# zicodasilva/cheetah_pose_estimation

Measured on AMD Instinct MI355X. Metric: frames/sec residual+Jacobian eval + full-traj solves/sec, 200-frame 6-cam seq, higher is better.
Workload: dtype f64; 1 GPU; cfg2: synthetic 200-frame x 6-cam x 25-marker sequences, phantom skeleton, const-accel model; frames=200, cams=6, markers=25, sequences_per_gpu=2048, parallelism=shard1 (independent sequences, no collective)

## Files before the change

cheetah_pose_estimation_amd/csrc/cpe_api.hip:

```cpp
#include <hip/hip_runtime.h>

#include <cmath>
#include <cstdio>
#include <cstdlib>
#include <cstring>
#include <functional>
#include <string>
#include <vector>
#include <algorithm>
#include <type_traits>

#include "cpe_kernels.hip"

static thread_local std::string g_err;
static cpe_status fail(cpe_status s, const std::string& m) { g_err = m; return s; }
#define HIPCHK(x)                                                                                         \
    do {                                                                                                  \
        hipError_t e_ = (x);                                                                              \
        if (e_ != hipSuccess) return fail(CPE_HIP_ERROR, std::string(#x) + ": " + hipGetErrorString(e_)); \
    } while (0)

struct cpe_handle {
    int device = 0;
    int n_cu = 256;
    hipStream_t stream = nullptr;
    DevModel hm;
    DevModel* dm = nullptr;
    std::vector<DevModel> models;
    cpe_options opts;
    size_t ws_frames = 0; int ws_B = 0;
    std::vector<void**> ws_bufs;
    double *qbuf = nullptr, *gbuf = nullptr, *Bbuf = nullptr, *costbuf = nullptr, *Lbuf = nullptr, *zbuf = nullptr,
           *gtbuf = nullptr, *dgbuf = nullptr, *cmax = nullptr, *mu = nullptr, *gambuf = nullptr;
    SeqState* st = nullptr;
    int* flag = nullptr;
    int* act = nullptr;
    int2* rseq = nullptr;
    int* n_act = nullptr;
    int* poll_host = nullptr;
    hipEvent_t poll_ev[2] = {nullptr, nullptr};
    hipEvent_t order_ev = nullptr;
    bool prof = false;
    double prof_ms[CPE_PROFILE_SLOTS] = {0};
    int64_t prof_n[CPE_PROFILE_SLOTS] = {0};
    std::vector<std::pair<int, std::pair<hipEvent_t, hipEvent_t>>> prof_spans;
    cpe_eom_options* eom = nullptr;
    cpe_dyn_options* dyn = nullptr;
    DevPriors* pri = nullptr;
    int gmm_k = 0, gmm_dim = 0, lr_window = 0;
    double* Hlr = nullptr;
    DevKin* dk = nullptr; DevKin hk;
    std::vector<DevKin> hks;
    size_t kws_frames = 0;
    std::vector<void**> kws_bufs;
    double *kmut = nullptr;
    double *kmus = nullptr;
    double *fbuf = nullptr, *kmu = nullptr, *Jbuf = nullptr, *Abuf = nullptr, *pieces = nullptr, *gTb = nullptr, *dstat = nullptr, *slackb = nullptr,
           *Tbuf = nullptr, *gk = nullptr, *Bk = nullptr, *Hk = nullptr;
    int* pmeta = nullptr;
    DevTrack* dtrack = nullptr; std::vector<DevTrack> htrack;
    double* xtgt = nullptr; size_t xtgt_frames = 0;
    double* covG = nullptr; size_t covG_n = 0;
    int pb = 3;
};

struct DevBuf {
    double* p = nullptr;
    ~DevBuf() { if (p) (void)hipFree(p); }
    hipError_t alloc(size_t n) { return hipMalloc(&p, sizeof(double) * (n ? n : 1)); }
};

template <class T>
static hipError_t ws_alloc(std::vector<void**>& rec, T*& p, size_t n) {
    rec.push_back(reinterpret_cast<void**>(&p));
    return hipMalloc(&p, sizeof(T) * n);
}
static void ws_free(std::vector<void**>& rec) {
    for (void** p : rec) { (void)hipFree(*p); *p = nullptr; }
    rec.clear();
}

static double host_rho0(double a, double b, double c) {
    auto sg = [](double t) { return 1.0 / (1.0 + std::exp(t)); };
    const double sa = sg(a), sb = sg(b), sc = sg(c);
    const double cb = c - b, w = c / cb;
    return (sa - sb) * (-0.5 * a * a) + (sb - sc) * (a * b - 0.5 * a * a + 0.5 * a * cb * (1.0 - w * w)) +
           sc * (a * b - 0.5 * a * a + 0.5 * a * cb);
}

static cpe_status build_model(const cpe_skeleton* s, const cpe_camera* cams, int C, const cpe_options* o, DevModel& m) {
    memset(&m, 0, sizeof(m));
    if (s->n_links < 1 || s->n_links > CPE_MAX_LINKS || s->n_markers < 1 || s->n_markers > CPE_MAX_MARKERS ||
        s->n_joints < 0 || s->n_joints > CPE_MAX_JOINTS || s->n_bounds < 0 || s->n_bounds > CPE_MAX_BOUNDS ||
        C < 1 || C > CPE_MAX_CAMS)
        return fail(CPE_BAD_ARG, "skeleton / camera counts out of range");
    const int nl = s->n_links, nq = 3 + 3 * nl, L = s->n_markers;
    m.nl = nl; m.L = L; m.C = C; m.nq = nq; m.nj = s->n_joints; m.nb = s->n_bounds;
    m.h = o->h; m.ih2 = 1.0 / (o->h * o->h);
    m.loss_a = o->loss_a; m.loss_b = o->loss_b; m.loss_c = o->loss_c;
    m.bound_penalty = o->bound_penalty; m.curvature = o->curvature;
    m.rho0 = host_rho0(o->loss_a, o->loss_b, o->loss_c);
    if (!(o->h > 0)) return fail(CPE_BAD_ARG, "options.h must be > 0");
    double mt = 0;
    for (int i = 0; i < nl; i++) {
        if (s->parent[i] >= i) return fail(CPE_BAD_ARG, "links must be ordered parents first");
        m.parent[i] = s->parent[i];
        for (int d = 0; d < 3; d++) { m.attach[i][d] = s->attach[i][d]; m.com[i][d] = s->com[i][d]; }
        m.mass[i] = s->mass[i]; mt += s->mass[i];
    }
    m.inv_total_mass = mt > 0 ? 1.0 / mt : 0.0;
    for (int c = 0; c < C; c++) m.cam[c] = cams[c];

    for (int p = 0; p < nq; p++) { m.u_of_q[p] = -1; m.dep_of_q[p] = -1; }
    int ndep = 0;
    std::vector<int> joint_of_child(nl, -1);
    for (int j = 0; j < s->n_joints; j++) {
        const int p = s->joint_parent[j], c = s->joint_child[j], k = s->joint_kind[j];
        if (p < 0 || p >= nl || c <= p || c >= nl || joint_of_child[c] >= 0) return fail(CPE_BAD_ARG, "bad joint");
        m.joint_parent[j] = p; m.joint_child[j] = c; m.joint_kind[j] = k;
        joint_of_child[c] = j;
        m.joint_dep0[j] = ndep;
        m.dep_joint[ndep] = j;
        m.dep_of_q[3 + 3 * c] = ndep++;
        if (k == CPE_JOINT_REVOLUTE_Y) { m.dep_joint[ndep] = j; m.dep_of_q[3 + 3 * c + 2] = ndep++; }
        else if (k != CPE_JOINT_HOOKE_YZ) return fail(CPE_BAD_ARG, "unknown joint kind");
        if (ndep > CPE_MAX_DEP) return fail(CPE_BAD_ARG, "too many dependent angles");
    }
    m.ndep = ndep;
    int nu = 0;
    for (int p = 0; p < nq; p++)
        if (m.dep_of_q[p] < 0) { if (nu >= CPE_NX) return fail(CPE_BAD_ARG, "more than 28 independent dofs"); m.indep[nu] = p; m.u_of_q[p] = nu++; }
    m.nu = nu;
    if (nu != CPE_NX) return fail(CPE_BAD_ARG, "the solver is built for exactly 28 independent dofs");
    for (int p = 0; p < nq; p++)
        if (m.dep_of_q[p] >= 0 && s->motion_w[p] != 0.0) return fail(CPE_BAD_ARG, "motion weight on a dependent angle");
    for (int k = 0; k < nu; k++) {
        const int p = m.indep[k];
        m.motion_w_u[k] = s->motion_w[p];
        m.rel_sign_u[k] = s->rel_ref[p] < 0 ? 1.0 : s->rel_sign[p];
        m.rel_ref_u[k] = s->rel_ref[p] < 0 ? -1 : m.u_of_q[s->rel_ref[p]];
        if (s->rel_ref[p] >= 0 && m.rel_ref_u[k] < 0) return fail(CPE_BAD_ARG, "relative angle references a dependent dof");
    }
// ... 21 lines not shown
            m.joint_body[j] = p;
            m.srow[r] = m.n_srow++;
            int n = 0;
            auto add = [&](int col, int kind, int ang, int chain) -> bool {
                for (int e = 0; e < n; e++)
                    if (m.scol[r][e] == col) { if (chain >= 0) m.hk_chain[r][e] = (int16_t)chain; else { m.hk_kind[r][e] = (int8_t)kind; m.hk_ang[r][e] = (int8_t)ang; } return true; }
                if (n >= CPE_MAX_SCOL) return false;
                m.scol[r][n] = col; m.hk_kind[r][n] = (int8_t)kind; m.hk_ang[r][n] = (int8_t)ang; m.hk_chain[r][n] = (int16_t)chain; n++;
                return true;
            };
            if (m.u_of_q[3 + 3 * c + 1] < 0 || m.u_of_q[3 + 3 * c + 2] < 0) return fail(CPE_BAD_ARG, "theta/psi of a hooke child must be independent");
            bool ok = add(m.u_of_q[3 + 3 * c + 1], 0, 1, -1) && add(m.u_of_q[3 + 3 * c + 2], 0, 2, -1);
            m.dep_level[r] = 0;
            for (int a = 0; a < 3 && ok; a++) {
                const int pq = 3 + 3 * p + a;
                if (m.u_of_q[pq] >= 0) ok = add(m.u_of_q[pq], 1, a, -1);
                else {
                    if (a != 0) return fail(CPE_BAD_ARG, "hooke parent with dependent theta/psi is not supported");
                    const int pr = m.dep_of_q[pq];
                    if (m.dep_level[pr] != 0 || m.joint_kind[m.dep_joint[pr]] != CPE_JOINT_HOOKE_YZ)
                        return fail(CPE_BAD_ARG, "hooke chains deeper than two are not supported");
                    m.dep_level[r] = 1;
                    for (int e = 0; e < m.scol_n[pr] && ok; e++) ok = add(m.scol[pr][e], 2, 0, m.srow[pr] * CPE_MAX_SCOL + e);
                }
            }
            if (!ok) return fail(CPE_BAD_ARG, "too many columns in a hooke row");
            m.scol_n[r] = n;
        }
    }
    std::vector<int> rev_of_link(nl, -1);
    m.nrev = 0;
    for (int p = 0; p < nq; p++) m.euler_rev[p] = -1;
    for (int k = 0; k < nu; k++) { m.rev_of_u[k] = -1; m.ucoord_src[k] = m.indep[k]; m.bodyang_j[k] = -1; m.bodyang_legs_n[k] = 0; }
    for (int j = 0; j < s->n_joints; j++)
        if (m.joint_kind[j] == CPE_JOINT_REVOLUTE_Y) {
            const int r = m.nrev++, c = m.joint_child[j], Bk = m.joint_body[j];
            rev_of_link[c] = r;
            m.rev_child[r] = c; m.rev_body[r] = Bk; m.rev_u[r] = m.u_of_q[3 + 3 * c + 1];
            m.rev_of_u[m.rev_u[r]] = r; m.euler_rev[3 + 3 * c + 1] = r;
            for (int a = 0; a < 3; a++) {
                const int kb = m.u_of_q[3 + 3 * Bk + a];
                m.rev_body_u[r][a] = kb; m.bodyang_j[kb] = a;
                m.bodyang_legs[kb][m.bodyang_legs_n[kb]++] = r;
            }
        }
    m.ns = nq + m.nrev;
    for (int k = 0; k < nu; k++) {
        const int r = m.rev_of_u[k];
        m.ucost[k] = r < 0 ? m.indep[k] : ((3 + 3 * m.rev_body[r] + 1) | (nq + r + 1) << 8);
    }
    if (m.nrev > LM_MAX_REV) return fail(CPE_BAD_ARG, "more than 12 leg links");
    for (int k = 0; k < nu; k++) if (m.bodyang_legs_n[k] > LM_MAX_LEGS) return fail(CPE_BAD_ARG, "more than 6 leg links on one body");
    for (int r = 0; r < m.nrev; r++) m.ucoord_src[m.rev_u[r]] = nq + r;
    m.n_trunk = 0;
    for (int i = 0; i < nl; i++) { m.trunk_slot[i] = -1; if (rev_of_link[i] < 0) { m.trunk_slot[i] = m.n_trunk; m.trunk_link[m.n_trunk++] = i; } }
    int S = 0, mct = 0, ss = 0, sv = 0;
    for (int l = 0; l < L; l++) {
        int chain[CPE_MAX_LINKS], n = 0, k = s->marker_link[l];
        if (k < 0 || k >= nl) return fail(CPE_BAD_ARG, "bad marker link");
        while (k >= 0) { chain[n++] = k; k = s->parent[k]; }
        if (n > CPE_MAX_CHAIN) return fail(CPE_BAD_ARG, "marker chain too long");
        m.chain_len[l] = n;
        for (int i = 0; i < n; i++) {
            const int link = chain[n - 1 - i];
            m.chain_link[l][i] = link;
            const double* v = i == n - 1 ? s->marker_off[l] : s->attach[chain[n - 2 - i]];
            for (int d = 0; d < 3; d++) m.chain_vec[l][i][d] = v[d];
        }
        m.slot_off[l] = S;
        if (S + 3 + 3 * n > CPE_MAX_SLOTS) return fail(CPE_BAD_ARG, "too many Jacobian slots");
        for (int d = 0; d < 3; d++) { m.slot_marker[S] = l; m.slot_dof[S] = d; m.slot_cpos[S] = -1; m.slot_ang[S] = 0; S++; }
        for (int i = 0; i < n; i++)
            for (int a = 0; a < 3; a++) { m.slot_marker[S] = l; m.slot_dof[S] = 3 + 3 * m.chain_link[l][i] + a; m.slot_cpos[S] = i; m.slot_ang[S] = a; S++; }
        int nc = 0;
        auto col_index = [&](int col) -> int {
            for (int e = 0; e < nc; e++) if (m.mcol[l][e] == col) return e;
            if (nc >= CPE_MAX_MCOL) return -1;
            m.mcol[l][nc] = col; m.term_n[l][nc] = 0; return nc++;
        };
        auto add_term = [&](int col, int slot, int sidx) -> bool {
            const int e = col_index(col);
            if (e < 0 || m.term_n[l][e] >= CPE_MAX_TERMS) return false;
            m.term_slot[l][e][m.term_n[l][e]] = (int16_t)slot; m.term_s[l][e][m.term_n[l][e]] = (int16_t)sidx; m.term_n[l][e]++;
            return true;
        };
        auto new_slot = [&](int moff, int vdyn, const double* v) -> int {
            if (ss >= CPE_MAX_SLOTS) return -1;
            m.ss_moff[ss] = moff; m.ss_vdyn[ss] = vdyn;
            for (int d = 0; d < 3; d++) m.ss_vec[ss][d] = v ? v[d] : 0.0;
            return ss++;
        };
        bool ok = true;
        const double ex[3][3] = {{1, 0, 0}, {0, 1, 0}, {0, 0, 1}};
        for (int d = 0; d < 3 && ok; d++) { const int sl = new_slot(-1, -1, ex[d]); ok = sl >= 0 && add_term(m.u_of_q[d], sl, -1); }
        int n_trunk_chain = 0;
        while (n_trunk_chain < n && rev_of_link[m.chain_link[l][n_trunk_chain]] < 0) n_trunk_chain++;
        m.pc_len[l] = n_trunk_chain; m.pw_id[l] = -1; m.pw_body[l] = 0;
        for (int i = 0; i < n_trunk_chain && ok; i++) {
            const int link = m.chain_link[l][i];
            m.pc_link[l][i] = link;
            for (int d = 0; d < 3; d++) m.pc_vec[l][i][d] = m.chain_vec[l][i][d];
            for (int a = 0; a < 3 && ok; a++) {
                const int sl = new_slot(9 * (4 * m.trunk_slot[link] + 1 + a), -1, m.chain_vec[l][i]);
                const int p = 3 + 3 * link + a;
                if (sl < 0) { ok = false; break; }
                if (m.u_of_q[p] >= 0) ok = add_term(m.u_of_q[p], sl, -1);
// ... 86 lines not shown
                const int a = m.mcol[l][i];
                if (m.gg_cnt[a] >= CPE_MAX_GG) return fail(CPE_BAD_ARG, "gradient gather list too long");
                m.gg_code[m.gg_cnt[a]++][a] = (uint16_t)((m.mcol_off[l] + i) | (l << 8));
            }
    }
    {
        m.hk_n = 0;
        for (int r = 0; r < m.ndep; r++) {
            const int j = m.dep_joint[r];
            if (m.joint_kind[j] != CPE_JOINT_HOOKE_YZ || m.srow[r] < 0) continue;
            for (int jc = 0; jc < m.scol_n[r]; jc++) {
                if (m.hk_n >= 64) return fail(CPE_BAD_ARG, "more than 64 entries in the hooke rows of S");
                const int ps = m.trunk_slot[m.joint_parent[j]], cs = m.trunk_slot[m.joint_child[j]];
                if (ps < 0 || cs < 0 || ps >= 64 || cs >= 64) return fail(CPE_BAD_ARG, "hooke joint between leg links");
                m.hk_w[m.hk_n][0] = ps | (cs << 6) | ((m.hk_kind[r][jc] & 3) << 12) | ((m.hk_ang[r][jc] & 3) << 14) | ((m.dep_level[r] & 1) << 16);
                m.hk_w[m.hk_n][1] = (m.hk_chain[r][jc] + 1) | ((m.srow[r] * CPE_MAX_SCOL + jc) << 16);
                m.hk_n++;
            }
        }
        m.hj_n = 0;
        for (int j = 0; j < s->n_joints; j++)
            if (m.joint_kind[j] == CPE_JOINT_HOOKE_YZ) {
                if (m.hj_n >= 64) return fail(CPE_BAD_ARG, "more than 64 hooke joints");
                m.fn_lane[m.hj_n++][0] = m.joint_parent[j] | (m.joint_child[j] << 8) | ((m.dep_of_q[3 + 3 * m.joint_parent[j]] >= 0 ? 1 : 0) << 16);
            }
        for (int t = 0; t < 4 * m.n_trunk && t < 64; t++) m.fn_lane[t][1] = m.trunk_link[t >> 2];
        for (int r = 0; r < m.nrev; r++) m.fn_lane[r][2] = m.rev_body[r] | (m.rev_child[r] << 8) | (m.trunk_slot[m.rev_body[r]] << 16);
        for (int t = 0; t < m.sv_n; t++) m.fn_lane[t][3] = m.sv_kind[t] | (m.sv_cnt[t] << 2) | (m.sv_rev[t][0] << 4) | (m.sv_rev[t][1] << 10) | (m.sv_rev[t][2] << 16);
        for (int l = 0; l < L; l++) {
            for (int i = 0; i < m.pc_len[l]; i++) m.pc_off[l][i] = 36 * m.trunk_slot[m.pc_link[l][i]];
            m.pw_off[l] = m.pw_id[l] >= 0 ? 36 * m.trunk_slot[m.pw_body[l]] : 0;
        }
    }
    for (int bnd = 0; bnd < s->n_bounds; bnd++) {
        const int a = s->bound_a[bnd], bb = s->bound_b[bnd];
        if (a < 0 || a >= nq || bb >= nq || m.u_of_q[a] < 0 || (bb >= 0 && m.u_of_q[bb] < 0))
            return fail(CPE_BAD_ARG, "bounds must act on independent dofs");
        m.bound_ua[bnd] = m.u_of_q[a]; m.bound_ub[bnd] = bb < 0 ? -1 : m.u_of_q[bb];
        m.bound_lo[bnd] = s->bound_lo[bnd]; m.bound_up[bnd] = s->bound_up[bnd];
        const int ca = m.ucost[m.u_of_q[a]], cb = bb < 0 ? 0 : m.ucost[m.u_of_q[bb]];
        m.bnd_q[bnd] = (ca & 255) | (bb < 0 ? 0 : ((cb & 255) + 1) << 8) | ((ca >> 8) & 255) << 16 | (bb < 0 ? 0 : ((cb >> 8) & 255)) << 24;
    }
    return CPE_OK;
}

#define FRAME_NORMAL(plain) ((plain) ? k_frame_normal<true> : k_frame_normal<false>)
#define FRAME_NORMAL_RAGGED(plain) ((plain) ? k_frame_normal<true, true> : k_frame_normal<false, true>)
static size_t lds_fk(const DevModel& m) { return sizeof(double) * (m.nq + 6 * m.nl + 36 * m.nl + 3 * m.L + 23 * m.C); }
static size_t lds_normal(const DevModel& m, int gmm_k = 0, int gmm_dim = 0, bool shutter = false) {
    const bool plain = gmm_k == 0 && !shutter;
    size_t ov = CPE_MAX_SCOL * m.n_srow, hg = plain ? m.nu : m.nu * m.nu + m.nu;
    size_t camov = 6 * m.nl + 2 * m.nrev + 36 * m.n_trunk;
    if (camov < (size_t)22 * m.C) camov = (size_t)22 * m.C;
    size_t n = m.ns + camov + 3 * m.L + 3 * m.sv_n + GAM_STRIDE * m.nrev + (ov > hg ? ov : hg) +
               9 * m.L + 3 * m.mc_total;
    if (gmm_k > 0) n += CPE_NX + gmm_k * gmm_dim + CPE_MAX_GMM + CPE_NX;
    if (shutter) n += 15 * m.C + 6 * m.L + 6;
    return sizeof(double) * n;
}
static size_t lds_fk_all(const cpe_handle* h) {
    size_t n = lds_fk(h->hm);
    for (const DevModel& m : h->models) n = std::max(n, lds_fk(m));
    return n;
}
static size_t lds_normal_all(const cpe_handle* h) {
    size_t n = lds_normal(h->hm, h->gmm_k, h->gmm_dim);
    for (const DevModel& m : h->models) n = std::max(n, lds_normal(m, h->gmm_k, h->gmm_dim));
    return n;
}
#define FRAME_TRACKED(gmm) ((gmm) ? k_frame_tracked<true> : k_frame_tracked<false>)
#define FRAME_TRACKED_RAGGED(gmm) ((gmm) ? k_frame_tracked<true, true> : k_frame_tracked<false, true>)
static size_t lds_tracked(const DevModel& m, int gmm_k, int gmm_dim) {
    size_t n = m.ns + 6 * m.nl + 2 * m.nrev + 36 * m.n_trunk + GAM_STRIDE * m.nrev + m.nu + m.nu * m.nu + m.nu;
    if (gmm_k > 0) n += CPE_NX + gmm_k * gmm_dim + CPE_MAX_GMM + CPE_NX;
    return sizeof(double) * n;
}
static size_t lds_tracked_all(const cpe_handle* h) {
    size_t n = lds_tracked(h->hm, h->gmm_k, h->gmm_dim);
    for (const DevModel& m : h->models) n = std::max(n, lds_tracked(m, h->gmm_k, h->gmm_dim));
    return n;
}
static int n_models(const cpe_handle* h) { return h->models.empty() ? 1 : (int)h->models.size(); }
static int cams_max(const cpe_handle* h) {
    int c = h->hm.C;
    for (const DevModel& m : h->models) c = std::max(c, m.C);
    return c;
}

extern "C" {

const char* cpe_last_error(void) { return g_err.c_str(); }

void cpe_default_options(cpe_options* o) {
    o->h = 1.0 / 120.0; o->loss_a = 3.0; o->loss_b = 10.0; o->loss_c = 20.0; o->cost_scale = 1e-3;
    o->bound_penalty = 1e4; o->bound_tol = 1e-6; o->lambda0 = 1e-4; o->tol_step = 1e-8; o->tol_cost = 1e-9; o->max_iter = 200;
    o->curvature = 0; o->max_outer = 8; o->_pad = 0;
}

void cpe_destroy(cpe_handle* h);
static cpe_status create_impl(cpe_handle* h, const cpe_skeleton* skel, const cpe_camera* cams, int32_t n_cams, const cpe_options* opts,
                              const cpe_priors* priors, bool use_pri, const std::vector<DevModel>* models = nullptr) {
    const int device = h->device;
    if (models) { h->models = *models; h->hm = h->models[0]; }
    else if (cpe_status s = build_model(skel, cams, n_cams, opts, h->hm); s != CPE_OK) return s;
    HIPCHK(hipSetDevice(device));
    {
        hipDeviceProp_t prop;
        HIPCHK(hipGetDeviceProperties(&prop, device));
        h->n_cu = prop.multiProcessorCount > 0 ? prop.multiProcessorCount : 256;
        const void* ks[] = {(const void*)&k_resjac<true, 4, 3, 2>, (const void*)&k_resjac<false, 4, 3, 2>,
                            (const void*)&k_resjac<true, 4, 4, 2>, (const void*)&k_resjac<false, 4, 4, 2>,
                            (const void*)&k_dyn_eval<>, (const void*)&k_dyn_assemble<>, (const void*)&k_dyn_schur<>, (const void*)&k_dyn_jac<>,
                            (const void*)&k_dyn_eval<true>, (const void*)&k_dyn_assemble<true>, (const void*)&k_dyn_schur<true>, (const void*)&k_dyn_jac<true>};
        for (const void* k : ks) {
            hipFuncAttributes fa;
            HIPCHK(hipFuncGetAttributes(&fa, k));
            HIPCHK(hipFuncSetAttribute(k, hipFuncAttributeMaxDynamicSharedMemorySize, 160 * 1024 - (int)fa.sharedSizeBytes));
        }
    }
    HIPCHK(hipStreamCreateWithFlags(&h->stream, hipStreamNonBlocking));
    HIPCHK(hipEventCreateWithFlags(&h->order_ev, hipEventDisableTiming));
    for (int i = 0; i < 2; i++) HIPCHK(hipEventCreateWithFlags(&h->poll_ev[i], hipEventDisableTiming));
    HIPCHK(hipHostMalloc(reinterpret_cast<void**>(&h->poll_host), 2 * sizeof(int), hipHostMallocDefault));
    HIPCHK(hipMalloc(&h->n_act, sizeof(int)));
    HIPCHK(hipMalloc(&h->dm, sizeof(DevModel) * n_models(h)));
    HIPCHK(hipMemcpy(h->dm, h->models.empty() ? &h->hm : h->models.data(), sizeof(DevModel) * n_models(h), hipMemcpyHostToDevice));
// ... 374 lines not shown
    if (!h) return fail(CPE_BAD_ARG, "null argument");
    size_t F;
    if (cpe_status s = frames(B, N, &F); s != CPE_OK) return s;
    if (F == 0) return CPE_OK;
    if (!positions || !uv) return fail(CPE_BAD_ARG, "null argument");
    HIPCHK(hipSetDevice(h->device));
    hipLaunchKernelGGL(k_reproject, dim3((unsigned)F), dim3(WAVE), 0, h->stream, h->dm, positions, uv);
    HIPCHK(hipGetLastError());
    return CPE_OK;
}

cpe_status cpe_triangulate(cpe_handle* h, int32_t n, const int32_t* cam_a, const int32_t* cam_b, const double* uv_a, const double* uv_b,
                           double depth, double* xyz) {
    if (!h) return fail(CPE_BAD_ARG, "null argument");
    if (n < 0) return fail(CPE_BAD_ARG, "negative size");
    if (n == 0) return CPE_OK;
    if (!cam_a || !cam_b || !uv_a || !uv_b || !xyz) return fail(CPE_BAD_ARG, "null argument");
    HIPCHK(hipSetDevice(h->device));
    std::vector<int32_t> ia(n), ib(n);
    HIPCHK(hipMemcpyAsync(ia.data(), cam_a, sizeof(int32_t) * n, hipMemcpyDeviceToHost, h->stream));
    HIPCHK(hipMemcpyAsync(ib.data(), cam_b, sizeof(int32_t) * n, hipMemcpyDeviceToHost, h->stream));
    HIPCHK(hipStreamSynchronize(h->stream));
    for (int i = 0; i < n; i++)
        if (ia[i] < 0 || ia[i] >= h->hm.C || ib[i] >= h->hm.C) return fail(CPE_BAD_ARG, "camera index out of range");
    hipLaunchKernelGGL(k_triangulate, dim3((unsigned)((n + 255) / 256)), dim3(256), 0, h->stream, h->dm, n, cam_a, cam_b, uv_a, uv_b, depth, xyz);
    HIPCHK(hipGetLastError());
    return CPE_OK;
}

cpe_status cpe_tensorise_dlc(cpe_handle* h, int32_t N, int32_t n_slots, int32_t slot, const double* table, int32_t rows, int32_t parts,
                             int32_t first_row, const int32_t* part_of_marker, const double* inv_sigma, double thresh, double* meas, double* weight) {
    if (!h) return fail(CPE_BAD_ARG, "null argument");
    if (N < 0 || rows < 0 || parts <= 0) return fail(CPE_BAD_ARG, "bad size");
    if (n_slots <= 0 || slot < 0 || slot >= n_slots) return fail(CPE_BAD_ARG, "camera slot out of range");
    if (N == 0) return CPE_OK;
    if (!part_of_marker || !inv_sigma || !meas || !weight || (!table && rows > 0)) return fail(CPE_BAD_ARG, "null argument");
    HIPCHK(hipSetDevice(h->device));
    const long total = (long)N * h->hm.L;
    hipLaunchKernelGGL(k_tensorise_dlc, dim3((unsigned)((total + 255) / 256)), dim3(256), 0, h->stream, N, h->hm.L, n_slots, slot, table, rows, parts,
                       first_row, part_of_marker, inv_sigma, thresh, meas, weight);
    HIPCHK(hipGetLastError());
    return CPE_OK;
}

static size_t n_mu(const DevModel& m, size_t F) { return F * (size_t)(m.nb > 0 ? m.nb : 1) * 2; }

static cpe_status ensure_ws(cpe_handle* h, int B, int N) {
    const size_t F = (size_t)B * N;
    if (F <= h->ws_frames && B <= h->ws_B) return CPE_OK;
    free_ws(h);
    const int nu = h->hm.nu;
    auto& w = h->ws_bufs;
    HIPCHK(ws_alloc(w, h->qbuf, 2 * F * h->hm.ns));
    HIPCHK(ws_alloc(w, h->gambuf, 2 * F * (size_t)(GAM_STRIDE * (h->hm.nrev > 0 ? h->hm.nrev : 1))));
    HIPCHK(ws_alloc(w, h->gbuf, 2 * F * nu));
    HIPCHK(ws_alloc(w, h->Bbuf, 2 * F * nu * nu));
    HIPCHK(ws_alloc(w, h->costbuf, 2 * F * COST_STRIDE));
    HIPCHK(ws_alloc(w, h->mu, n_mu(h->hm, F)));
    HIPCHK(ws_alloc(w, h->Lbuf, F * (h->pb + 1) * nu * nu + (size_t)B * lm_spill_doubles(h->pb)));
    HIPCHK(ws_alloc(w, h->zbuf, F * nu));
    HIPCHK(ws_alloc(w, h->gtbuf, F * nu));
    HIPCHK(ws_alloc(w, h->dgbuf, F * nu));
    HIPCHK(ws_alloc(w, h->cmax, F));
    HIPCHK(ws_alloc(w, h->st, B));
    HIPCHK(ws_alloc(w, h->act, B));
    HIPCHK(ws_alloc(w, h->rseq, B));
    if (h->lr_window > 0) HIPCHK(ws_alloc(w, h->Hlr, 2 * F * h->pb * nu * nu));
    h->ws_frames = F; h->ws_B = B;
    return CPE_OK;
}

static cpe_status state_reset(cpe_handle* h, int B, int N, const double* q, const RaggedArgs* rg = nullptr) {
    const size_t F = (size_t)B * N;
    if (rg) hipLaunchKernelGGL(k_state_init<true>, dim3((unsigned)F), dim3(WAVE), 0, h->stream, h->dm, q, h->qbuf, *rg);
    else hipLaunchKernelGGL(k_state_init<>, dim3((unsigned)F), dim3(WAVE), 0, h->stream, h->dm, q, h->qbuf);
    HIPCHK(hipMemsetAsync(h->st, 0, sizeof(SeqState) * B, h->stream));
    HIPCHK(hipMemsetAsync(h->mu, 0, sizeof(double) * n_mu(h->hm, F), h->stream));
    return CPE_OK;
}

cpe_status cpe_eval_normal(cpe_handle* h, int32_t B, int32_t N, const double* q, const double* meas, const double* weight,
                           double* g, double* Bm, double* cost, double* gam, double* q_out) {
    if (!h || !q || !meas || !weight || !g || !Bm || !cost) return fail(CPE_BAD_ARG, "null argument");
    size_t F;
    if (cpe_status s = frames(B, N, &F); s != CPE_OK) return s;
    if (F == 0) return CPE_OK;
    HIPCHK(hipSetDevice(h->device));
    cpe_status s = ensure_ws(h, B, N);
    if (s != CPE_OK) return s;
    if ((s = state_reset(h, B, N, q)) != CPE_OK) return s;
    const DevModel& m = h->hm;
    hipLaunchKernelGGL(FRAME_NORMAL(h->gmm_k == 0), dim3((unsigned)F), dim3(WAVE), lds_normal(m, h->gmm_k, h->gmm_dim), h->stream, h->dm, h->st, N, 1, F, h->qbuf, meas, weight,
                       h->gbuf, h->Bbuf, h->costbuf, h->mu, h->gambuf, h->pri, nullptr, nullptr, ShutterArgs{nullptr, nullptr, nullptr}, RaggedArgs{});
    HIPCHK(hipMemcpyAsync(g, h->gbuf, sizeof(double) * F * m.nu, hipMemcpyDeviceToDevice, h->stream));
    HIPCHK(hipMemcpyAsync(Bm, h->Bbuf, sizeof(double) * F * m.nu * m.nu, hipMemcpyDeviceToDevice, h->stream));
    hipLaunchKernelGGL(k_gather_normal, dim3((unsigned)F), dim3(128), 0, h->stream, h->dm, F, h->qbuf, h->costbuf, h->gambuf, cost, gam, q_out);
    HIPCHK(hipGetLastError());
    return CPE_OK;
}

static LmParams lm_params(const cpe_handle* h, int B, int N) {
    LmParams prm;
    prm.tol_step = h->opts.tol_step; prm.tol_cost = h->opts.tol_cost; prm.lambda0 = h->opts.lambda0; prm.B = B; prm.N = N;
    prm.bound_tol = h->opts.bound_tol; prm.max_outer = h->opts.max_outer; prm.max_iter = h->opts.max_iter;
    return prm;
}

using LmIterate = std::function<void(int first, const int* act, const int* n_act, int slots)>;

static cpe_status lm_drive(cpe_handle* h, int B, const LmIterate& iterate) {
    iterate(1, nullptr, nullptr, B);
    HIPCHK(hipGetLastError());
    const int window = std::min(B, h->n_cu * (h->pb == 3 ? 2 : 1));
    constexpr int POLL = 4;
    const long per_seq = (long)h->opts.max_iter + 2L * (h->opts.max_outer > 0 ? h->opts.max_outer : 0) + POLL;
    const long max_rounds = ((long)(B + window - 1) / window + 1) * per_seq;
    bool pending[2] = {false, false};
    int slot = 0;
    for (long it = 0; it < max_rounds; it += POLL) {
        for (int k = 0; k < POLL; k++) {
            prof_begin(h, 3);
            hipLaunchKernelGGL(k_build_act, dim3(1), dim3(256), 0, h->stream, h->st, B, window, h->act, h->n_act);
            prof_end(h);
            iterate(0, h->act, h->n_act, window);
        }
        HIPCHK(hipGetLastError());
        HIPCHK(hipMemcpyAsync(h->poll_host + slot, h->n_act, sizeof(int), hipMemcpyDeviceToHost, h->stream));
        HIPCHK(hipEventRecord(h->poll_ev[slot], h->stream));
        pending[slot] = true;
        const int prev = 1 - slot;
        if (pending[prev]) {
            HIPCHK(hipEventSynchronize(h->poll_ev[prev]));
            pending[prev] = false;
            if (h->poll_host[prev] == 0) break;
        }
        slot = prev;
    }
    return CPE_OK;
}

__global__ void k_reset_status(SeqState* __restrict__ st, int B) {
    const int b = blockIdx.x * blockDim.x + threadIdx.x;
    if (b < B) { st[b].status = 0; st[b].al_pending = 0; }
}

extern "C++" template <class Fn>
static void with_pb(int pb, Fn&& f) {
    switch (pb) {
    case 3: f(std::integral_constant<int, 3>{}); break;
    case 4: f(std::integral_constant<int, 4>{}); break;
    case 5: f(std::integral_constant<int, 5>{}); break;
    default: f(std::integral_constant<int, 6>{}); break;
    }
}

static void lm_iterate(cpe_handle* h, const LmParams& prm, int N, size_t Fw, size_t ldsn, const double* meas, const double* weight, ShutterArgs sh,
                       const RaggedArgs* rg, int first, const int* act, const int* n_act, int slots, bool back = true) {
    const bool lr = h->lr_window > 0;
    const unsigned gf = (unsigned)((size_t)slots * N);
    const double* hiu = lr ? reinterpret_cast<const double*>(reinterpret_cast<const char*>(h->pri) + offsetof(DevPriors, lr_HIu)) + CPE_NX * CPE_NX : nullptr;
    if (rg) {
        prof_begin(h, 0);
        hipLaunchKernelGGL(FRAME_NORMAL_RAGGED(h->gmm_k == 0), dim3(gf), dim3(WAVE), ldsn, h->stream, h->dm, h->st, N, first, Fw, h->qbuf, meas, weight,
                           h->gbuf, h->Bbuf, h->costbuf, h->mu, h->gambuf, h->pri, act, n_act, ShutterArgs{nullptr, nullptr, nullptr}, *rg);
        prof_end(h);
        if (lr) {
            prof_begin(h, 1);
            hipLaunchKernelGGL(k_lr_band<true>, dim3(gf), dim3(WAVE), 0, h->stream, h->dm, h->st, N, first, Fw, h->qbuf, h->gambuf, h->pri, h->pb, h->gbuf,
                               h->Bbuf, h->Hlr, h->costbuf, act, n_act, *rg);
            prof_end(h);
        }
        prof_begin(h, 2);
        with_pb(h->pb, [&](auto pbc) {
            hipLaunchKernelGGL((k_lm_step<decltype(pbc)::value, 0, true>), dim3(slots), dim3(LM_THREADS), 0, h->stream, h->dm, h->st, prm, first, h->qbuf,
                               h->gbuf, h->Bbuf, h->costbuf, h->Lbuf, h->zbuf, h->gtbuf, h->gambuf, h->Hlr, act, n_act, 2, nullptr, h->dgbuf, hiu, h->lr_window, *rg);
        });
        prof_end(h);
        if (!back) return;
        prof_begin(h, 7);
        with_pb(h->pb, [&](auto pbc) {
            hipLaunchKernelGGL((k_lm_back<decltype(pbc)::value, true>), dim3(slots), dim3(2 * WAVE), 0, h->stream, h->dm, h->st, prm, h->qbuf, h->Lbuf,
                               h->zbuf, h->gtbuf, h->dgbuf, act, n_act, *rg);
        });
        prof_end(h);
        return;
    }
    prof_begin(h, 0);
    hipLaunchKernelGGL(FRAME_NORMAL(h->gmm_k == 0 && sh.tau == nullptr), dim3(gf), dim3(WAVE), ldsn, h->stream, h->dm, h->st, N, first, Fw, h->qbuf, meas, weight, h->gbuf, h->Bbuf,
                       h->costbuf, h->mu, h->gambuf, h->pri, act, n_act, sh, RaggedArgs{});
    prof_end(h);
    if (lr) {
        prof_begin(h, 1);
        hipLaunchKernelGGL(k_lr_band<>, dim3(gf), dim3(WAVE), 0, h->stream, h->dm, h->st, N, first, Fw, h->qbuf, h->gambuf, h->pri, h->pb, h->gbuf, h->Bbuf,
                           h->Hlr, h->costbuf, act, n_act);
        prof_end(h);
    }
    prof_begin(h, 2);
    with_pb(h->pb, [&](auto pbc) {
        hipLaunchKernelGGL((k_lm_step<decltype(pbc)::value, 0>), dim3(slots), dim3(LM_THREADS), 0, h->stream, h->dm, h->st, prm, first, h->qbuf, h->gbuf,
                           h->Bbuf, h->costbuf, h->Lbuf, h->zbuf, h->gtbuf, h->gambuf, h->Hlr, act, n_act, 2, sh.gx, h->dgbuf, hiu, h->lr_window);
    });
    prof_end(h);
    if (!back) return;
    prof_begin(h, 7);
    with_pb(h->pb, [&](auto pbc) {
        hipLaunchKernelGGL((k_lm_back<decltype(pbc)::value>), dim3(slots), dim3(2 * WAVE), 0, h->stream, h->dm, h->st, prm, h->qbuf, h->Lbuf, h->zbuf,
                           h->gtbuf, h->dgbuf, act, n_act);
    });
    prof_end(h);
}

static cpe_status lm_run(cpe_handle* h, int B, int N, const double* q_init, const double* meas, const double* weight, ShutterArgs sh,
                         const RaggedArgs* rg = nullptr) {
    const DevModel& m = h->hm;
    const size_t Fw = (size_t)B * N;
    if (q_init) {
        const cpe_status s = state_reset(h, B, N, q_init, rg);
        if (s != CPE_OK) return s;
    } else hipLaunchKernelGGL(k_reset_status, dim3((B + 255) / 256), dim3(256), 0, h->stream, h->st, B);
    const LmParams prm = lm_params(h, B, N);
    const size_t ldsn = rg ? lds_normal_all(h) : lds_normal(m, h->gmm_k, h->gmm_dim, sh.tau != nullptr);
    return lm_drive(h, B, [&](int first, const int* act, const int* n_act, int slots) {
        lm_iterate(h, prm, N, Fw, ldsn, meas, weight, sh, rg, first, act, n_act, slots);
    });
}

static cpe_status lm_readback(cpe_handle* h, int B, int N, const double* meas, double* q, double* dq, double* ddq, double* positions, double* meas_err,
                              const double* tau, const std::function<void()>& more, std::vector<SeqState>& hs, std::vector<double>& hc,
                              const RaggedArgs* rg = nullptr) {
    const size_t F = (size_t)B * N;
    HIPCHK(hipMemsetAsync(h->cmax, 0, sizeof(double) * B, h->stream));
    if (rg) hipLaunchKernelGGL(k_finalize<true>, dim3((unsigned)F), dim3(WAVE), lds_fk_all(h), h->stream, h->dm, h->st, N, F, h->qbuf, meas, q, dq, ddq,
                               positions, meas_err, reinterpret_cast<unsigned long long*>(h->cmax), nullptr, *rg);
    else hipLaunchKernelGGL(k_finalize<>, dim3((unsigned)F), dim3(WAVE), lds_fk(h->hm), h->stream, h->dm, h->st, N, F, h->qbuf, meas, q, dq, ddq, positions, meas_err,
                            reinterpret_cast<unsigned long long*>(h->cmax), tau);
    if (more) more();
    HIPCHK(hipGetLastError());
    hs.resize(B);
    hc.resize(B);
    HIPCHK(hipMemcpyAsync(hs.data(), h->st, sizeof(SeqState) * B, hipMemcpyDeviceToHost, h->stream));
    HIPCHK(hipMemcpyAsync(hc.data(), h->cmax, sizeof(double) * B, hipMemcpyDeviceToHost, h->stream));
    HIPCHK(hipStreamSynchronize(h->stream));
    prof_collect(h);
    return CPE_OK;
}

static void kinematic_costs(const SeqState& S, double scale, cpe_stats& o) {
    o.cost_meas = S.terms[0]; o.cost_model = S.terms[1]; o.cost_pose = S.terms[3]; o.cost_motion = S.terms[4];
    o.cost = scale * (S.terms[0] + S.terms[1] + S.terms[3] + S.terms[4]);
}
static void kinetic_costs(const SeqState& S, double scale, cpe_stats& o) {
    o.cost_meas = S.terms[0]; o.cost_model = S.terms[4]; o.cost_pose = S.terms[3]; o.cost_motion = 0.0;
    o.cost = scale * (S.terms[0] + S.terms[3] + S.terms[4]);
// ... 322 lines not shown
    HIPCHK(ws_alloc(w, h->Jbuf, F * KIN_JSTRIDE));
    HIPCHK(ws_alloc(w, h->Abuf, F * CPE_MAX_NQ * KIN_LS));
    HIPCHK(ws_alloc(w, h->pieces, 2 * F * KIN_PIECE));
    HIPCHK(ws_alloc(w, h->pmeta, 2 * F * (KIN_LS + 1)));
    HIPCHK(ws_alloc(w, h->gTb, 2 * (F + 2) * KIN_NC3));
    HIPCHK(ws_alloc(w, h->dstat, 2 * F * KIN_STAT));
    HIPCHK(ws_alloc(w, h->slackb, 2 * F * CPE_MAX_NQ));
    HIPCHK(ws_alloc(w, h->Tbuf, (F + 2) * 6 * BB));
    HIPCHK(ws_alloc(w, h->gk, F * CPE_NX));
    HIPCHK(ws_alloc(w, h->Bk, F * BB));
    HIPCHK(ws_alloc(w, h->Hk, F * 3 * BB));
    h->kws_frames = F;
    return CPE_OK;
}

static cpe_status kin_state_reset(cpe_handle* h, size_t F, bool torque_box) {
    HIPCHK(hipMemsetAsync(h->fbuf, 0, sizeof(double) * 2 * F * KIN_LS, h->stream));
    HIPCHK(hipMemsetAsync(h->kmu, 0, sizeof(double) * F * 4 * KIN_MU, h->stream));
    HIPCHK(hipMemsetAsync(h->kmus, 0, sizeof(double) * F * 2 * CPE_MAX_NQ, h->stream));
    if (torque_box) HIPCHK(hipMemsetAsync(h->kmut, 0, sizeof(double) * F * 2 * CPE_MAX_MOTORS, h->stream));
    return CPE_OK;
}

extern "C++" {

template <bool RAGGED = false>
static void launch_dyn_eval(cpe_handle* h, int N, int first, size_t Fw, const int32_t* stance, const int* act, const int* n_act, int slots, RaggedArgs rg = RaggedArgs{}) {
    const unsigned gf = (unsigned)((size_t)slots * N);
    prof_begin(h, 5);
    hipLaunchKernelGGL(k_dyn_eval<RAGGED>, dim3(gf), dim3(KIN_THREADS), lds_kin_eval(), h->stream, h->dm, h->dk, h->st, N, first, Fw, h->qbuf, stance, h->fbuf, h->kmu,
                       h->costbuf, h->Jbuf, h->Abuf, h->pieces, h->pmeta, h->dstat, h->slackb, act, n_act, rg);
    prof_end(h);
}
template <bool RAGGED = false>
static void launch_dyn_pieces(cpe_handle* h, int N, int first, size_t Fw, const int* act, const int* n_act, int slots, RaggedArgs rg = RaggedArgs{}) {
    const unsigned gf = (unsigned)((size_t)slots * N);
    prof_begin(h, 10);
    hipLaunchKernelGGL(k_dyn_jac<RAGGED>, dim3(gf), dim3(KJ_THREADS), sizeof(double) * KJ_DOUBLES, h->stream, h->dm, h->dk, h->st, N, first, Fw, h->qbuf, h->fbuf, h->Jbuf,
                       act, n_act, rg);
    prof_end(h);
    prof_begin(h, 8);
    hipLaunchKernelGGL(k_dyn_assemble<RAGGED>, dim3(gf), dim3(KIN_THREADS), lds_kin_assemble(), h->stream, h->dm, h->dk, h->st, N, first, Fw, h->Jbuf, h->Abuf, h->pieces,
                       h->pmeta, h->gTb, act, n_act, rg);
    prof_end(h);
}

template <bool RAGGED>
static void kin_iterate(cpe_handle* h, const LmParams& prm, int N, size_t Fw, size_t ldsn, const double* meas, const double* weight, const int32_t* stance,
                        const double* xt, RaggedArgs rg, int first, const int* act, const int* n_act, int slots) {
    const unsigned gf = (unsigned)((size_t)slots * N);
    const bool plain = h->gmm_k == 0;
    prof_begin(h, 0);
    if (xt) hipLaunchKernelGGL(RAGGED ? FRAME_TRACKED_RAGGED(!plain) : FRAME_TRACKED(!plain), dim3(gf), dim3(WAVE), ldsn, h->stream, h->dm, h->dtrack, h->st, N, first, Fw,
                               h->qbuf, xt, h->gbuf, h->Bbuf, h->costbuf, h->mu, h->gambuf, h->pri, act, n_act, rg);
    else hipLaunchKernelGGL(RAGGED ? FRAME_NORMAL_RAGGED(plain) : FRAME_NORMAL(plain), dim3(gf), dim3(WAVE), ldsn, h->stream, h->dm, h->st, N, first, Fw, h->qbuf, meas,
                            weight, h->gbuf, h->Bbuf, h->costbuf, h->mu, h->gambuf, h->pri, act, n_act, ShutterArgs{nullptr, nullptr, nullptr}, rg);
    prof_end(h);
    launch_dyn_eval<RAGGED>(h, N, first, Fw, stance, act, n_act, slots, rg);
    prof_begin(h, 2);
    hipLaunchKernelGGL((k_lm_step<3, 1, RAGGED>), dim3(slots), dim3(LM_THREADS), 0, h->stream, h->dm, h->st, prm, first, h->qbuf, h->gbuf, h->Bbuf, h->costbuf,
                       h->Lbuf, h->zbuf, h->gtbuf, h->gambuf, nullptr, act, n_act, 2, nullptr, h->dgbuf, nullptr, 0, rg);
    prof_end(h);
    launch_dyn_pieces<RAGGED>(h, N, 0, Fw, act, n_act, slots, rg);
    prof_begin(h, 9);
    hipLaunchKernelGGL(k_dyn_schur<RAGGED>, dim3(gf), dim3(KIN_THREADS), lds_kin_schur(), h->stream, h->dk, h->st, N, Fw, h->pieces, h->pmeta, h->fbuf, h->kmu, stance,
                       h->Tbuf, act, n_act, rg);
    prof_end(h);
    prof_begin(h, 6);
    hipLaunchKernelGGL(k_dyn_gather<RAGGED>, dim3(gf), dim3(KIN_THREADS), 0, h->stream, h->st, N, Fw, h->gbuf, h->Bbuf, h->Tbuf, h->gTb, h->gk, h->Bk, h->Hk, act,
                       n_act, rg);
    prof_end(h);
    prof_begin(h, 2);
    hipLaunchKernelGGL((k_lm_step<3, 2, RAGGED>), dim3(slots), dim3(LM_THREADS), 0, h->stream, h->dm, h->st, prm, first, h->qbuf, h->gk, h->Bk, h->costbuf,
                       h->Lbuf, h->zbuf, h->gtbuf, h->gambuf, h->Hk, act, n_act, 1, nullptr, h->dgbuf, nullptr, 0, rg);
    prof_end(h);
    prof_begin(h, 7);
    hipLaunchKernelGGL((k_lm_back<3, RAGGED>), dim3(slots), dim3(2 * WAVE), 0, h->stream, h->dm, h->st, prm, h->qbuf, h->Lbuf, h->zbuf, h->gtbuf, h->dgbuf, act, n_act, rg);
    prof_end(h);
}

}

void cpe_default_track_weights(double w[CPE_NX]) {
    static const double t[CPE_NX] = {10, 10, 10, 5, 5, 5, 0, 5, 5, 0, 2, 2, 5, 5, 5, 5, 5, 2, 1, 5, 2, 1, 5, 2, 5, 2, 1, 1};
    for (int k = 0; k < CPE_NX; k++) w[k] = t[k];
}

static cpe_status build_track(cpe_handle* h, const double* w, int rows) {
    for (int i = 0; i < rows * CPE_NX; i++)
        if (!std::isfinite(w[i]) || w[i] < 0.0)
            return fail(CPE_BAD_ARG, "track_w: weights must be finite and non-negative (row " + std::to_string(i / CPE_NX) + ", entry " + std::to_string(i % CPE_NX) + ")");
    const int nmod = n_models(h);
    h->htrack.assign((size_t)nmod, DevTrack{});
    for (int k = 0; k < nmod; k++) {
        const DevModel& m = h->models.empty() ? h->hm : h->models[(size_t)k];
        const double* wk = w + (size_t)std::min(k, rows - 1) * CPE_NX;
        const int nu = m.nu;
        double X[CPE_NX][CPE_NX] = {};
        for (int i = 0; i < nu; i++)
            for (int side = 0; side < 2; side++) {
                const int kk = side == 0 ? i : m.rel_ref_u[i];
                if (kk < 0) continue;
                const double sgn = side == 0 ? m.rel_sign_u[i] : -m.rel_sign_u[i];
                X[i][kk] += sgn;
                const int r = m.rev_of_u[kk];
                if (r >= 0) X[i][m.rev_body_u[r][1]] += sgn;
            }
        DevTrack& T = h->htrack[(size_t)k];
        for (int i = 0; i < nu; i++) T.w[i] = wk[i];
        for (int i = 0; i < nu; i++)
            for (int j = 0; j < nu; j++) {
                T.Xt[j][i] = X[i][j];
                double a = 0.0;
                for (int p = 0; p < nu; p++) a += X[p][i] * wk[p] * X[p][j];
                T.H[i * nu + j] = 2.0 * a;
            }
    }
    if (!h->dtrack) HIPCHK(hipMalloc(&h->dtrack, sizeof(DevTrack) * nmod));
    HIPCHK(hipMemcpyAsync(h->dtrack, h->htrack.data(), sizeof(DevTrack) * nmod, hipMemcpyHostToDevice, h->stream));
    return CPE_OK;
}

static cpe_status check_target(const double* hq, int B, int N, int nq, const int32_t* lens) {
    for (int b = 0; b < B; b++)
        for (size_t i = 0; i < (size_t)(lens ? lens[b] : N) * nq; i++)
            if (!std::isfinite(hq[(size_t)b * N * nq + i]))
                return fail(CPE_BAD_ARG, "q_target: non-finite entry (sequence " + std::to_string(b) + ", frame " + std::to_string(i / nq) + ")");
// ... 135 lines not shown
    return solve_kinetic_impl(h, opt, B, N, nullptr, nullptr, q_init, meas, weight, stance, nullptr, tau_box, nullptr, q, dq, ddq, positions, meas_err, tau, lambda, grf, slack, stats, kstats);
}

cpe_status cpe_solve_kinetic_ragged(cpe_handle* h, const cpe_kinetic_options* opts, int32_t B, int32_t N_max, const int32_t* model, const int32_t* n_frames,
                                    const double* q_init, const double* meas, const double* weight, const int32_t* stance, const double* grf_fixed,
                                    const double* tau_box, const double* grf_box, double* q, double* dq, double* ddq, double* positions, double* meas_err,
                                    double* tau, double* lambda, double* grf, double* slack, cpe_stats* stats, cpe_kinetic_stats* kstats) {
    if (!h || !opts || !model || !n_frames) return fail(CPE_BAD_ARG, "null argument");
    if ((grf_fixed != nullptr) + (tau_box != nullptr) + (grf_box != nullptr) > 1)
        return fail(CPE_BAD_ARG, "cpe_solve_kinetic_ragged: at most one of grf_fixed, tau_box, grf_box");
    return solve_kinetic_impl(h, opts, B, N_max, model, n_frames, q_init, meas, weight, stance, grf_fixed, tau_box, grf_box, q, dq, ddq, positions, meas_err,
                              tau, lambda, grf, slack, stats, kstats);
}

cpe_status cpe_solve_kinetic_tracked(cpe_handle* h, const cpe_kinetic_options* opt, const double* track_w, int32_t B, int32_t N, const double* q_init,
                                     const double* q_target, const double* meas, const double* weight, const int32_t* stance, const double* grf_fixed,
                                     const double* tau_box, const double* grf_box, double* q, double* dq, double* ddq, double* positions, double* meas_err,
                                     double* tau, double* lambda, double* grf, double* slack, cpe_stats* stats, cpe_kinetic_stats* kstats) {
    if ((grf_fixed != nullptr) + (tau_box != nullptr) + (grf_box != nullptr) > 1)
        return fail(CPE_BAD_ARG, "cpe_solve_kinetic_tracked: at most one of grf_fixed, tau_box, grf_box");
    const TrackIn tr{track_w, 1, q_target, false};
    return solve_kinetic_impl(h, opt, B, N, nullptr, nullptr, q_init, meas, weight, stance, grf_fixed, tau_box, grf_box, q, dq, ddq, positions, meas_err,
                              tau, lambda, grf, slack, stats, kstats, &tr);
}

cpe_status cpe_solve_kinetic_tracked_ragged(cpe_handle* h, const cpe_kinetic_options* opts, const double* track_w, int32_t B, int32_t N_max,
                                            const int32_t* model, const int32_t* n_frames, const double* q_init, const double* q_target, const double* meas,
                                            const double* weight, const int32_t* stance, const double* grf_fixed, const double* tau_box,
                                            const double* grf_box, double* q, double* dq, double* ddq, double* positions, double* meas_err, double* tau,
                                            double* lambda, double* grf, double* slack, cpe_stats* stats, cpe_kinetic_stats* kstats) {
    if (!h || !opts || !model || !n_frames) return fail(CPE_BAD_ARG, "null argument");
    if ((grf_fixed != nullptr) + (tau_box != nullptr) + (grf_box != nullptr) > 1)
        return fail(CPE_BAD_ARG, "cpe_solve_kinetic_tracked_ragged: at most one of grf_fixed, tau_box, grf_box");
    const TrackIn tr{track_w, n_models(h), q_target, false};
    return solve_kinetic_impl(h, opts, B, N_max, model, n_frames, q_init, meas, weight, stance, grf_fixed, tau_box, grf_box, q, dq, ddq, positions, meas_err,
                              tau, lambda, grf, slack, stats, kstats, &tr);
}

cpe_status cpe_eval_normal_tracked(cpe_handle* h, const double* track_w, int32_t B, int32_t N, const double* q, const double* q_target, double* g,
                                   double* Bm, double* cost, double* gam, double* q_out) {
    if (!h || !q || !g || !Bm || !cost) return fail(CPE_BAD_ARG, "null argument");
    if (!track_w) return fail(CPE_BAD_ARG, "track_w is null");
    if (!q_target) return fail(CPE_BAD_ARG, "q_target is null");
    size_t F;
    if (cpe_status s = frames(B, N, &F); s != CPE_OK) return s;
    if (F == 0) return CPE_OK;
    HIPCHK(hipSetDevice(h->device));
    cpe_status s = ensure_ws(h, B, N);
    if (s != CPE_OK) return s;
    if ((s = build_track(h, track_w, 1)) != CPE_OK || (s = track_target(h, B, N, q_target, nullptr, nullptr, false)) != CPE_OK) return s;
    if ((s = state_reset(h, B, N, q)) != CPE_OK) return s;
    const DevModel& m = h->hm;
    hipLaunchKernelGGL(FRAME_TRACKED(h->gmm_k > 0), dim3((unsigned)F), dim3(WAVE), lds_tracked(m, h->gmm_k, h->gmm_dim), h->stream, h->dm, h->dtrack, h->st, N, 1, F,
                       h->qbuf, h->xtgt, h->gbuf, h->Bbuf, h->costbuf, h->mu, h->gambuf, h->pri, nullptr, nullptr, RaggedArgs{});
    HIPCHK(hipMemcpyAsync(g, h->gbuf, sizeof(double) * F * m.nu, hipMemcpyDeviceToDevice, h->stream));
    HIPCHK(hipMemcpyAsync(Bm, h->Bbuf, sizeof(double) * F * m.nu * m.nu, hipMemcpyDeviceToDevice, h->stream));
    hipLaunchKernelGGL(k_gather_normal, dim3((unsigned)F), dim3(128), 0, h->stream, h->dm, F, h->qbuf, h->costbuf, h->gambuf, cost, gam, q_out);
    HIPCHK(hipGetLastError());
    return CPE_OK;
}

cpe_status cpe_eval_kinetic_nodes(cpe_handle* h, const cpe_kinetic_options* opt, int32_t B, int32_t N, const double* q, const double* meas, const double* weight,
                                  const int32_t* stance, double* f, double* stat, double* g, double* Huu, double* Hfu, double* Hff, int32_t* meta) {
    return cpe_eval_kinetic_system(h, opt, B, N, q, meas, weight, stance, nullptr, nullptr, nullptr, f, stat, g, Huu, Hfu, Hff, meta, nullptr, nullptr, nullptr);
}

cpe_status cpe_eval_kinetic_system(cpe_handle* h, const cpe_kinetic_options* opt, int32_t B, int32_t N, const double* q, const double* meas, const double* weight,
                                   const int32_t* stance, const double* grf_fixed, const double* tau_box, const double* grf_box, double* f, double* stat,
                                   double* g, double* Huu, double* Hfu, double* Hff, int32_t* meta, double* gk, double* Bk, double* Hk) {
    if (!h || !opt || !q || !meas || !weight || !stance) return fail(CPE_BAD_ARG, "null argument");
    if ((grf_fixed != nullptr) + (tau_box != nullptr) + (grf_box != nullptr) > 1)
        return fail(CPE_BAD_ARG, "cpe_eval_kinetic_system: at most one of grf_fixed, tau_box, grf_box");
    size_t F;
    if (cpe_status s = frames(B, N, &F); s != CPE_OK) return s;
    if (F == 0) return CPE_OK;
    if (h->pb != 3) return fail(CPE_BAD_ARG, "the physics-based model runs on the half-bandwidth-3 solver");
    HIPCHK(hipSetDevice(h->device));
    cpe_status s = ensure_ws(h, B, N);
    if (s != CPE_OK) return s;
    if ((s = ensure_kws(h, B, N)) != CPE_OK) return s;
    if ((s = build_kin(h, opt, grf_fixed, tau_box, grf_box)) != CPE_OK) return s;
    if ((s = state_reset(h, B, N, q)) != CPE_OK || (s = kin_state_reset(h, F, tau_box != nullptr)) != CPE_OK) return s;
    HIPCHK(hipMemsetAsync(h->pieces, 0, sizeof(double) * F * KIN_PIECE, h->stream));
    HIPCHK(hipMemsetAsync(h->gTb, 0, sizeof(double) * F * KIN_NC3, h->stream));
    HIPCHK(hipMemsetAsync(h->dstat, 0, sizeof(double) * F * KIN_STAT, h->stream));
    const bool band = gk || Bk || Hk;
    std::vector<SeqState> hs;
    if (band) {
        hs.assign((size_t)B, SeqState{});
        for (SeqState& S : hs) S.lambda = h->opts.lambda0;
        HIPCHK(hipMemcpyAsync(h->st, hs.data(), sizeof(SeqState) * B, hipMemcpyHostToDevice, h->stream));
    }
    const DevModel& m = h->hm;
    hipLaunchKernelGGL(FRAME_NORMAL(h->gmm_k == 0), dim3((unsigned)F), dim3(WAVE), lds_normal(m, h->gmm_k, h->gmm_dim), h->stream, h->dm, h->st, N, 1, F, h->qbuf, meas, weight,
                       h->gbuf, h->Bbuf, h->costbuf, h->mu, h->gambuf, h->pri, nullptr, nullptr, ShutterArgs{nullptr, nullptr, nullptr}, RaggedArgs{});
    launch_dyn_eval<>(h, N, 1, F, stance, nullptr, nullptr, B);
    launch_dyn_pieces<>(h, N, 1, F, nullptr, nullptr, B);
    if (band) {
        hipLaunchKernelGGL(k_dyn_schur<>, dim3((unsigned)F), dim3(KIN_THREADS), lds_kin_schur(), h->stream, h->dk, h->st, N, F, h->pieces, h->pmeta, h->fbuf, h->kmu,
                           stance, h->Tbuf, nullptr, nullptr, RaggedArgs{});
        hipLaunchKernelGGL(k_dyn_gather<>, dim3((unsigned)F), dim3(KIN_THREADS), 0, h->stream, h->st, N, F, h->gbuf, h->Bbuf, h->Tbuf, h->gTb, h->gk, h->Bk, h->Hk,
                           nullptr, nullptr, RaggedArgs{});
    }
    HIPCHK(hipGetLastError());
    if (f) HIPCHK(hipMemcpyAsync(f, h->fbuf, sizeof(double) * F * KIN_LS, hipMemcpyDeviceToDevice, h->stream));
    if (stat) HIPCHK(hipMemcpyAsync(stat, h->dstat, sizeof(double) * F * KIN_STAT, hipMemcpyDeviceToDevice, h->stream));
    if (g) HIPCHK(hipMemcpyAsync(g, h->gTb, sizeof(double) * F * KIN_NC3, hipMemcpyDeviceToDevice, h->stream));
    if (meta) HIPCHK(hipMemcpyAsync(meta, h->pmeta, sizeof(int) * F * (KIN_LS + 1), hipMemcpyDeviceToDevice, h->stream));
    const size_t w = sizeof(double), BB = (size_t)CPE_NX * CPE_NX;
    if (Huu) HIPCHK(hipMemcpy2DAsync(Huu, w * KIN_NC3 * KIN_NC3, h->pieces, w * KIN_PIECE, w * KIN_NC3 * KIN_NC3, F, hipMemcpyDeviceToDevice, h->stream));
    if (Hfu) HIPCHK(hipMemcpy2DAsync(Hfu, w * KIN_LS * KIN_NC3, h->pieces + KIN_NC3 * KIN_NC3, w * KIN_PIECE, w * KIN_LS * KIN_NC3, F, hipMemcpyDeviceToDevice, h->stream));
    if (Hff) HIPCHK(hipMemcpy2DAsync(Hff, w * KIN_LS * KIN_LS, h->pieces + KIN_NC3 * KIN_NC3 + KIN_LS * KIN_NC3, w * KIN_PIECE, w * KIN_LS * KIN_LS, F, hipMemcpyDeviceToDevice, h->stream));
    if (gk) HIPCHK(hipMemcpyAsync(gk, h->gk, w * F * CPE_NX, hipMemcpyDeviceToDevice, h->stream));
    if (Bk) HIPCHK(hipMemcpyAsync(Bk, h->Bk, w * F * BB, hipMemcpyDeviceToDevice, h->stream));
    if (Hk) HIPCHK(hipMemcpy2DAsync(Hk, w * 2 * BB, h->Hk, w * 3 * BB, w * 2 * BB, F, hipMemcpyDeviceToDevice, h->stream));
    if (band) HIPCHK(hipStreamSynchronize(h->stream));
    return CPE_OK;
}

cpe_status cpe_eval_lm_step(cpe_handle* h, const cpe_kinetic_options* kopt, int32_t B, int32_t N, const double* q, const double* meas,
                            const double* weight, const int32_t* stance, double lam, double* g, double* dg, double* L, double* delta, double* state,
                            double* seq) {
    if (!h || !q || !meas || !weight || !seq) return fail(CPE_BAD_ARG, "null argument");
    if ((kopt == nullptr) != (stance == nullptr)) return fail(CPE_BAD_ARG, "cpe_eval_lm_step: stance is given with the kinetic options, and only then");
    if (!(lam > 0.0) || !std::isfinite(lam)) return fail(CPE_BAD_ARG, "cpe_eval_lm_step: the damping must be positive and finite");
    size_t F;
    if (cpe_status s = frames(B, N, &F); s != CPE_OK) return s;
    if (F == 0) return CPE_OK;
    if (kopt && h->pb != 3) return fail(CPE_BAD_ARG, "the physics-based model runs on the half-bandwidth-3 solver");
    HIPCHK(hipSetDevice(h->device));
    cpe_status s = ensure_ws(h, B, N);
    if (s != CPE_OK) return s;
    if (kopt) {
        if ((s = ensure_kws(h, B, N)) != CPE_OK) return s;
        if ((s = build_kin(h, kopt)) != CPE_OK) return s;
    }
    if ((s = state_reset(h, B, N, q)) != CPE_OK) return s;
    if (kopt && (s = kin_state_reset(h, F, false)) != CPE_OK) return s;
    const DevModel& m = h->hm;
    const int ns = m.ns, RING = h->pb + 1;
    const size_t BB = (size_t)CPE_NX * CPE_NX, w = sizeof(double), LC = (size_t)RING * BB;
    HIPCHK(hipMemsetAsync(h->gtbuf, 0, w * F * CPE_NX, h->stream));
    HIPCHK(hipMemsetAsync(h->dgbuf, 0, w * F * CPE_NX, h->stream));
    HIPCHK(hipMemsetAsync(h->zbuf, 0, w * F * CPE_NX, h->stream));
    HIPCHK(hipMemsetAsync(h->Lbuf, 0, w * F * LC, h->stream));
    HIPCHK(hipMemcpyAsync(h->qbuf + F * ns, h->qbuf, w * F * ns, hipMemcpyDeviceToDevice, h->stream));
    LmParams prm = lm_params(h, B, N);
    prm.lambda0 = lam;
// ... 445 lines not shown
```

cheetah_pose_estimation_amd/csrc/cpe_model.h:

```cpp
#pragma once
#include <stdint.h>

#include "../../include/cpe.h"

#define CPE_MAX_CHAIN 6
#define CPE_MAX_TL 512
#define CPE_MAX_SLOTS 320
#define CPE_MAX_MCOL 12
#define CPE_MAX_TERMS 8
#define CPE_MAX_HG 56
#define CPE_MAX_GG 32
#define CPE_MAX_DEP 32
#define CPE_MAX_SCOL 8
#define CPE_MAX_SDYN 48

struct DevModel {
    int32_t nl, L, C, nq, nu, S, nj, nb, ndep, curvature;
    double h, ih2, loss_a, loss_b, loss_c, bound_penalty, rho0;

    int32_t parent[CPE_MAX_LINKS];
    double attach[CPE_MAX_LINKS][3];
    double com[CPE_MAX_LINKS][3];
    double mass[CPE_MAX_LINKS];
    double inv_total_mass;

    int32_t chain_len[CPE_MAX_MARKERS];
    int32_t chain_link[CPE_MAX_MARKERS][CPE_MAX_CHAIN];
    double chain_vec[CPE_MAX_MARKERS][CPE_MAX_CHAIN][3];

    int32_t slot_off[CPE_MAX_MARKERS + 1];
    int32_t slot_marker[CPE_MAX_SLOTS];
    int32_t slot_dof[CPE_MAX_SLOTS];
    int32_t slot_cpos[CPE_MAX_SLOTS];
    int32_t slot_ang[CPE_MAX_SLOTS];

    cpe_camera cam[CPE_MAX_CAMS];

    int32_t joint_parent[CPE_MAX_JOINTS], joint_child[CPE_MAX_JOINTS], joint_kind[CPE_MAX_JOINTS];
    int32_t joint_body[CPE_MAX_JOINTS];
    int32_t joint_dep0[CPE_MAX_JOINTS];

    int32_t indep[CPE_NX];
    int32_t ucost[CPE_NX];
    int32_t u_of_q[CPE_MAX_NQ];
    int32_t dep_of_q[CPE_MAX_NQ];
    double motion_w_u[CPE_NX];
    double rel_sign_u[CPE_NX];
    int32_t rel_ref_u[CPE_NX];

    int32_t bound_ua[CPE_MAX_BOUNDS], bound_ub[CPE_MAX_BOUNDS];
    double bound_lo[CPE_MAX_BOUNDS], bound_up[CPE_MAX_BOUNDS];

    int32_t scol_n[CPE_MAX_DEP];
    int32_t scol[CPE_MAX_DEP][CPE_MAX_SCOL];

    int32_t mcol_n[CPE_MAX_MARKERS];
    int32_t mcol[CPE_MAX_MARKERS][CPE_MAX_MCOL];
    int32_t mcol_off[CPE_MAX_MARKERS + 1];
    int32_t term_n[CPE_MAX_MARKERS][CPE_MAX_MCOL];
    alignas(16) int16_t term_slot[CPE_MAX_MARKERS][CPE_MAX_MCOL][CPE_MAX_TERMS];
    alignas(16) int16_t term_s[CPE_MAX_MARKERS][CPE_MAX_MCOL][CPE_MAX_TERMS];
    int32_t mc_total;
    int32_t hg_cnt[64], hg_max;
    uint32_t hg_code[CPE_MAX_HG][64];
    int32_t gg_cnt[CPE_NX];
    uint16_t gg_code[CPE_MAX_GG][CPE_NX];
    int32_t tl_n;
    struct alignas(16) { int32_t w0, moff; double v[3]; } tl[CPE_MAX_TL];
    uint32_t h_covered[(CPE_NX * CPE_NX + 31) / 32];
    int16_t mc_marker[CPE_MAX_MARKERS * CPE_MAX_MCOL];
    int16_t mc_j[CPE_MAX_MARKERS * CPE_MAX_MCOL];

    int8_t hk_kind[CPE_MAX_DEP][CPE_MAX_SCOL];
    int8_t hk_ang[CPE_MAX_DEP][CPE_MAX_SCOL];
    int16_t hk_chain[CPE_MAX_DEP][CPE_MAX_SCOL];
    int32_t dep_joint[CPE_MAX_DEP];
    int32_t dep_level[CPE_MAX_DEP];
    int32_t srow[CPE_MAX_DEP], n_srow;

    int32_t nrev, ns, n_trunk, ss_n, sv_n;
    int32_t rev_child[CPE_MAX_JOINTS], rev_body[CPE_MAX_JOINTS], rev_u[CPE_MAX_JOINTS];
    int32_t rev_body_u[CPE_MAX_JOINTS][3];
    int32_t rev_of_u[CPE_NX];
    int32_t ucoord_src[CPE_NX];
    int32_t euler_rev[CPE_MAX_NQ];
    int32_t bodyang_j[CPE_NX];
    int32_t bodyang_legs_n[CPE_NX];
    int32_t bodyang_legs[CPE_NX][CPE_MAX_JOINTS];
    int32_t trunk_link[CPE_MAX_LINKS];
    int32_t trunk_slot[CPE_MAX_LINKS];
    int32_t sv_kind[CPE_MAX_SDYN], sv_cnt[CPE_MAX_SDYN], sv_rev[CPE_MAX_SDYN][3];
    double sv_vec[CPE_MAX_SDYN][3][3];
    int32_t pc_len[CPE_MAX_MARKERS], pc_link[CPE_MAX_MARKERS][CPE_MAX_CHAIN], pw_id[CPE_MAX_MARKERS], pw_body[CPE_MAX_MARKERS];
    double pc_vec[CPE_MAX_MARKERS][CPE_MAX_CHAIN][3];
    int32_t hj_n;
    alignas(16) int32_t fn_lane[64][4];
    int32_t hk_n, hk_w[64][2];
    int32_t pc_off[CPE_MAX_MARKERS][CPE_MAX_CHAIN], pw_off[CPE_MAX_MARKERS];
    int32_t bnd_q[CPE_MAX_BOUNDS];
    int32_t ss_moff[CPE_MAX_SLOTS], ss_vdyn[CPE_MAX_SLOTS];
    double ss_vec[CPE_MAX_SLOTS][3];
};

struct DevPriors {
    cpe_priors p;
    double lr_PK[CPE_MAX_WINDOW + 1][CPE_MAX_WINDOW + 1][CPE_NX * CPE_NX];
    double lr_HI[CPE_MAX_WINDOW + 1][CPE_NX * CPE_NX];
    int32_t lr_nf, _pad_nf;
    uint8_t lr_feat[CPE_MAX_WINDOW * CPE_NX];
    double lr_coefT[CPE_MAX_WINDOW * CPE_NX][CPE_NX];
    double Xc[CPE_NX][CPE_NX];
    double lr_PKu[CPE_MAX_WINDOW + 1][CPE_MAX_WINDOW + 1][CPE_NX * CPE_NX];
    double lr_HIu[CPE_MAX_WINDOW + 1][CPE_NX * CPE_NX];
    double gmm_PT[CPE_MAX_GMM][CPE_NX][CPE_NX];
    double gmm_Q[CPE_MAX_GMM][CPE_NX * CPE_NX];
};

struct SeqState {
    int32_t cur;
    int32_t status;
    int32_t iters;
    int32_t rejects;
    int32_t outer;
    int32_t al_pending;
    int32_t back_pending;
    int32_t fresh;
    double lambda, nu, cost_cur, pred, maxstep, maxviol;
    double terms[5];
};
```

cheetah_pose_estimation_amd/csrc/cpe_solver.hip.inc:

```

#define NU CPE_NX
#ifdef CPE_LM_STAMPS
__device__ unsigned long long g_lm_stamps[32];
__device__ unsigned long long g_fn_stamps[16];
#ifdef CPE_JAC_STAMPS
#define FSTAMP(i) do { (void)tf_last; } while (0)
#else
#define FSTAMP(i) do { if (blockIdx.x == 0 && threadIdx.x == 0) { const unsigned long long t_ = __builtin_amdgcn_s_memtime(); g_fn_stamps[i] += t_ - tf_last; tf_last = t_; } } while (0)
#endif
#define STAMP(i) do { if (blockIdx.x == 0 && threadIdx.x == 0) { const unsigned long long t_ = __builtin_amdgcn_s_memtime(); g_lm_stamps[i] += t_ - t_last; t_last = t_; } } while (0)
#define USTAMP(i) do { if (blockIdx.x == 0 && threadIdx.x == WAVE) { const unsigned long long t_ = __builtin_amdgcn_s_memtime(); g_lm_stamps[i] += t_ - tu_last; tu_last = t_; } } while (0)
#define BSTAMP(i) do { if (blockIdx.x == 0 && lane == 0) { const unsigned long long t_ = __builtin_amdgcn_s_memtime(); g_lm_stamps[16 + (i)] += t_ - tb_last; tb_last = t_; } } while (0)
#define RSTAMP(i) do { if (blockIdx.x == 0 && threadIdx.x == WAVE && g_tu) { const unsigned long long t_ = __builtin_amdgcn_s_memtime(); g_lm_stamps[i] += t_ - *g_tu; *g_tu = t_; } } while (0)
#else
#define RSTAMP(i) do { } while (0)
#define USTAMP(i) do { } while (0)
#define BSTAMP(i) do { } while (0)
#define STAMP(i) do { } while (0)
#define FSTAMP(i) do { } while (0)
#endif
#define LDB 29
#define BLK (NU * LDB)
#define LM_THREADS 256
#define LM_DIAG_FLOOR(N) ((N) < 4 ? 0.1 : 1e-12)
#define LM_NU0 8.0
#define LM_MAX_REV 12
#define LM_MAX_LEGS 6
#define LM_MAX_TERMS 256
#define LM_MAX_GROUP 7

struct LmParams {
    double tol_step, tol_cost, lambda0, bound_tol;
    int32_t B, N, max_outer, max_iter;
};
struct RaggedArgs { const int2* seq; int nmax; int cstride; };

#define COST_STRIDE 8

#define GAM_STRIDE 4

__device__ __forceinline__ double cost_coord(const DevModel* __restrict__ M, const double* __restrict__ state, int k) {
    const int w = M->ucost[k];
    return state[w & 255] + ((w >> 8) ? state[(w >> 8) - 1] : 0.0);
}

__device__ __forceinline__ void leg_euler(const double* RB, const double* scB, double sa, double ca, double psi_ref,
                                          double* euler, double* gam) {
    const double r00 = RB[0] * ca - RB[2] * sa, r10 = RB[3] * ca - RB[5] * sa, r20 = RB[6] * ca - RB[8] * sa;
    const double r21 = RB[7], r22 = RB[6] * sa + RB[8] * ca;
    double sth = -r20; sth = fmin(1.0, fmax(-1.0, sth));
    const double th = asin(sth), phi = atan2(r21, r22);
    double psi = atan2(r10, r00);
    psi += 6.283185307179586476925286766559 * rint((psi_ref - psi) / 6.283185307179586476925286766559);
    euler[0] = phi; euler[1] = th; euler[2] = psi;
    const double cth = sqrt(fmax(0.0, 1.0 - sth * sth));
    const double icth = cth > 1e-300 ? 1.0 / cth : 0.0;
    const double sphic = r21 * icth, cphic = r22 * icth;
    const double sfB = scB[0], cfB = scB[1], stB = scB[2], ctB = scB[3];
    gam[0] = cphic;
    gam[1] = -sphic * sa;
    gam[2] = cphic * cfB + sphic * ca * sfB;
    gam[3] = cphic * sfB * ctB - sphic * (ca * cfB * ctB - sa * stB);
}

template <bool RAGGED = false>
__global__ __launch_bounds__(WAVE) void k_state_init(const DevModel* __restrict__ M, const double* __restrict__ q, double* __restrict__ state,
                                                    RaggedArgs rg = RaggedArgs{}) {
    const int lane = threadIdx.x;
    const size_t f = blockIdx.x;
    if constexpr (RAGGED) {
        const int2 rs = rg.seq[f / (unsigned)rg.nmax];
        if ((int)(f % (unsigned)rg.nmax) >= rs.y) return;
        M += rs.x;
    }
    const int nq = M->nq, ns = M->ns;
    if (lane < nq) state[f * ns + lane] = q[f * nq + lane];
    if (lane < M->nrev) {
        const double* qb = q + f * nq + 3 + 3 * M->rev_body[lane];
        const double* qc = q + f * nq + 3 + 3 * M->rev_child[lane];
        double scb[6], scc[6], RB[9], RC[9];
        for (int a = 0; a < 3; a++) { sincos(qb[a], &scb[2 * a], &scb[2 * a + 1]); sincos(qc[a], &scc[2 * a], &scc[2 * a + 1]); }
        rot_kind(scb, 0, RB); rot_kind(scc, 0, RC);
        const double m00 = RB[0] * RC[0] + RB[3] * RC[3] + RB[6] * RC[6], m02 = RB[0] * RC[2] + RB[3] * RC[5] + RB[6] * RC[8];
        state[f * ns + nq + lane] = atan2(m02, m00);
    }
}

struct ShutterArgs { const double* tau; double* gx; double* rcb; };
template <bool PLAIN, bool RAGGED = false>
__global__ __launch_bounds__(WAVE) void k_frame_normal(const DevModel* __restrict__ M, const SeqState* __restrict__ st,
                                                       int N, int which, size_t n_frames,
                                                       double* __restrict__ qbuf, const double* __restrict__ meas,
                                                       const double* __restrict__ weight, double* __restrict__ gbuf,
                                                       double* __restrict__ Bbuf, double* __restrict__ costbuf,
                                                       double* __restrict__ mu, double* __restrict__ gambuf,
                                                       const DevPriors* __restrict__ pri, const int* __restrict__ act ,
                                                       const int* __restrict__ n_act ,
                                                       ShutterArgs sh = ShutterArgs{nullptr, nullptr, nullptr},
                                                       RaggedArgs rg = RaggedArgs{} ) {
    extern __shared__ double smem[];
    const int lane = threadIdx.x;
    if (n_act && (int)(blockIdx.x / (unsigned)N) >= *n_act) return;
    const int b = act ? act[blockIdx.x / (unsigned)N] : (int)(blockIdx.x / (unsigned)N);
    if constexpr (RAGGED) {
        const int2 rs = rg.seq[b];
        if ((int)(blockIdx.x % (unsigned)N) >= rs.y) return;
        M += rs.x;
    }
    const size_t f = (size_t)b * N + blockIdx.x % (unsigned)N;
    const SeqState S = st[b];
    if (S.status != 0) return;
    const int pend = S.al_pending;
    const int buf = (which || pend) ? S.cur : 1 - S.cur;

    const int nq = M->nq, nl = M->nl, L = M->L, C = M->C, nu = M->nu, ndep = M->ndep, mct = M->mc_total;
    const int nrev = M->nrev, ns = M->ns, ssn = M->ss_n, svn = M->sv_n;
    double* sq = smem;
    double* sal = sq + nq;
    double* ssc = sal + nrev;
    double* ssa = ssc + 6 * nl;
    double* sR = ssa + 2 * nrev;
    const int n_camov = 6 * nl + 2 * nrev + 36 * M->n_trunk;
    double* spos = ssc + (n_camov > CAMW * C ? n_camov : CAMW * C);
    double* scam = ssc;
    double* sdyn = spos + 3 * L;
    double* sgam = sdyn + 3 * svn;
    double* sSv = sgam + GAM_STRIDE * nrev;
    const int n_ov = CPE_MAX_SCOL * M->n_srow, n_hg = PLAIN ? nu : nu * nu + nu;
    double* sMv = sSv + (n_ov > n_hg ? n_ov : n_hg);
    double* sDp = sMv + 9 * L;
    double* sH = sSv;
    double* sg = PLAIN ? sSv : sH + nu * nu;
    (void)ssn;

#ifdef CPE_LM_STAMPS
    unsigned long long tf_last = __builtin_amdgcn_s_memtime();
#endif
    const int4 fw = *reinterpret_cast<const int4*>(M->fn_lane[lane]);
    const int svl = lane < CPE_MAX_SDYN ? lane : 0;
    double svv[3][3];
#pragma unroll
    for (int i = 0; i < 3; i++) { svv[i][0] = M->sv_vec[svl][i][0]; svv[i][1] = M->sv_vec[svl][i][1]; svv[i][2] = M->sv_vec[svl][i][2]; }
    const int hj_n = M->hj_n;
    __builtin_amdgcn_s_setprio(2);
    const int hk_n = M->hk_n;
    const int2 hkw = *reinterpret_cast<const int2*>(M->hk_w[lane]);
    double* stf = qbuf + (size_t)buf * n_frames * ns + f * ns;
    for (int t = lane; t < ns; t += WAVE) sq[t] = stf[t];
    for (int t = lane; t < 9 * L; t += WAVE) sMv[t] = 0.0;
    wave_lds_sync();
    wave_sincos(M, sq, ssc, lane);
    if (lane < nrev) { double s_, c_; sincos(sal[lane], &s_, &c_); ssa[2 * lane] = s_; ssa[2 * lane + 1] = c_; }
    wave_lds_sync();
    for (int level = 0; level < 2; level++) {
        if (lane < hj_n && ((fw.x >> 16) & 1) == level) {
            const int p = fw.x & 255, c = (fw.x >> 8) & 255;
            double a[3];
            rot_ycol(ssc + 6 * p, a);
            const double st = ssc[6 * c + 2], ct = ssc[6 * c + 3], sp = ssc[6 * c + 4], cp = ssc[6 * c + 5];
            const double num = a[0] * st * cp + a[1] * st * sp + a[2] * ct;
            const double den = a[1] * cp - a[0] * sp;
            const double hyp = sqrt(num * num + den * den);
            sq[3 + 3 * c] = atan2(num, den);
            ssc[6 * c] = num / hyp; ssc[6 * c + 1] = den / hyp;
        }
        wave_lds_sync();
    }
    if (lane < 4 * M->n_trunk) rot_kind(ssc + 6 * fw.y, lane & 3, sR + 9 * lane);
    for (int t = WAVE + lane; t < 4 * M->n_trunk; t += WAVE) rot_kind(ssc + 6 * M->trunk_link[t >> 2], t & 3, sR + 9 * t);
    wave_lds_sync();
    if (lane < nrev) {
        const int Bk = fw.z & 255, c = (fw.z >> 8) & 255;
        double e[3];
        double gtrue[GAM_STRIDE];
        leg_euler(sR + 36 * (fw.z >> 16), ssc + 6 * Bk, ssa[2 * lane], ssa[2 * lane + 1], sq[3 + 3 * Bk + 2], e, gtrue);
        sq[3 + 3 * c] = e[0]; sq[3 + 3 * c + 1] = e[1]; sq[3 + 3 * c + 2] = e[2];
        sgam[GAM_STRIDE * lane] = 1.0; sgam[GAM_STRIDE * lane + 1] = 0.0; sgam[GAM_STRIDE * lane + 2] = 1.0; sgam[GAM_STRIDE * lane + 3] = 0.0;
    }
    if (lane < svn) {
        double d0 = 0.0, d1 = 0.0, d2 = 0.0;
        if ((fw.w & 3) == 0) {
            const int cnt = (fw.w >> 2) & 3;
#pragma unroll
            for (int i = 0; i < 3; i++) {
                const int r = (fw.w >> (4 + 6 * i)) & 63;
                const double sa = ssa[2 * r], ca = ssa[2 * r + 1];
                if (i < cnt) { d0 += ca * svv[i][0] + sa * svv[i][2]; d1 += svv[i][1]; d2 += -sa * svv[i][0] + ca * svv[i][2]; }
            }
        } else {
            const int r = (fw.w >> 4) & 63;
            const double sa = ssa[2 * r], ca = ssa[2 * r + 1];
            d0 = -sa * svv[0][0] + ca * svv[0][2]; d2 = -ca * svv[0][0] - sa * svv[0][2];
        }
        sdyn[3 * lane] = d0; sdyn[3 * lane + 1] = d1; sdyn[3 * lane + 2] = d2;
    }
    wave_lds_sync();
    if (lane < nq) stf[lane] = sq[lane];
    if (lane < GAM_STRIDE * nrev) gambuf[((size_t)buf * n_frames + f) * (GAM_STRIDE * nrev) + lane] = sgam[lane];

    const int lm_ = lane < L ? lane : 0;
    int pco[CPE_MAX_CHAIN]; double pcv[CPE_MAX_CHAIN][3];
#pragma unroll
    for (int k = 0; k < CPE_MAX_CHAIN; k++) { pco[k] = M->pc_off[lm_][k]; pcv[k][0] = M->pc_vec[lm_][k][0]; pcv[k][1] = M->pc_vec[lm_][k][1]; pcv[k][2] = M->pc_vec[lm_][k][2]; }
    const int pwid = M->pw_id[lm_], pwo = M->pw_off[lm_];
    FSTAMP(0);
    for (int level = 0; level < 2; level++) {
        if (lane < hk_n && ((hkw.x >> 16) & 1) == level) {
            const double* Rp = sR + 36 * (hkw.x & 63); const double* Rc = sR + 36 * ((hkw.x >> 6) & 63);
            const double y0 = Rp[1], y1 = Rp[4], y2 = Rp[7];
            const double z0 = Rc[2], z1 = Rc[5], z2 = Rc[8];
            const double* Dcphi = Rc + 9;
            const double gphi = y0 * Dcphi[2] + y1 * Dcphi[5] + y2 * Dcphi[8];
            const int kind = (hkw.x >> 12) & 3, ang = (hkw.x >> 14) & 3;
            double direct = 0.0;
            if (kind == 0) { const double* D = Rc + 9 * (1 + ang); direct = y0 * D[2] + y1 * D[5] + y2 * D[8]; }
            else if (kind == 1) { const double* D = Rp + 9 * (1 + ang); direct = D[1] * z0 + D[4] * z1 + D[7] * z2; }
            double val = -direct / gphi;
            const int ch = (hkw.y & 0xFFFF) - 1;
            if (ch >= 0) {
                const double* Dpphi = Rp + 9;
                const double t0 = -(Dpphi[1] * z0 + Dpphi[4] * z1 + Dpphi[7] * z2) / gphi;
                val += t0 * sSv[ch];
            }
            sSv[hkw.y >> 16] = val;
        }
        wave_lds_sync();
    }

    FSTAMP(1);
    if (lane < L) {
        double p0 = sq[0], p1 = sq[1], p2 = sq[2];
#pragma unroll
        for (int k = 0; k < CPE_MAX_CHAIN; k++) {
            const double* R = sR + pco[k];
            const double v0 = pcv[k][0], v1 = pcv[k][1], v2 = pcv[k][2];
            p0 += R[0] * v0 + R[1] * v1 + R[2] * v2; p1 += R[3] * v0 + R[4] * v1 + R[5] * v2; p2 += R[6] * v0 + R[7] * v1 + R[8] * v2;
        }
        const int wid = pwid;
        if (wid >= 0) {
            const double* R = sR + pwo;
            const double v0 = sdyn[3 * wid], v1 = sdyn[3 * wid + 1], v2 = sdyn[3 * wid + 2];
            p0 += R[0] * v0 + R[1] * v1 + R[2] * v2; p1 += R[3] * v0 + R[4] * v1 + R[5] * v2; p2 += R[6] * v0 + R[7] * v1 + R[8] * v2;
        }
        spos[3 * lane] = p0; spos[3 * lane + 1] = p1; spos[3 * lane + 2] = p2;
    }
    FSTAMP(2);
    constexpr int PAIR_PF = 3;
    const size_t pair0 = f * (size_t)((RAGGED ? rg.cstride : C) * L);
    const int n_pairs = C * L;
    const int pt0 = lane < n_pairs ? lane : n_pairs - 1, pt1 = WAVE + lane < n_pairs ? WAVE + lane : n_pairs - 1,
              pt2 = 2 * WAVE + lane < n_pairs ? 2 * WAVE + lane : n_pairs - 1;
// ... 150 lines not shown
            sg[lane] = ga;
        }
    }
    wave_lds_sync();
    if (sh.tau) {
        if (shut) {
            for (int t = lane; t < mct; t += WAVE) {
                const int l = M->mc_marker[t], j = M->mcol[l][M->mc_j[t]];
                const double* m1 = sM1 + 6 * l; const double* d = sDp + 3 * t;
                const double y0 = m1[0] * d[0] + m1[1] * d[1] + m1[2] * d[2], y1 = m1[1] * d[0] + m1[3] * d[1] + m1[4] * d[2], y2 = m1[2] * d[0] + m1[4] * d[1] + m1[5] * d[2];
                atomicAdd(sH + 0 * nu + j, y0); atomicAdd(sH + 1 * nu + j, y1); atomicAdd(sH + 2 * nu + j, y2);
                atomicAdd(sH + j * nu + 0, y0); atomicAdd(sH + j * nu + 1, y1); atomicAdd(sH + j * nu + 2, y2);
            }
            if (lane < 9) { const int r = lane / 3, cc = lane - 3 * r; const int e = r <= cc ? (r == 0 ? cc : (r == 1 ? 2 + cc : 5)) : (cc == 0 ? r : (cc == 1 ? 2 + r : 5)); atomicAdd(sH + r * nu + cc, sM2[e]); }
            if (lane < 3) { double a = 0.0; for (int c = 0; c < C; c++) a += sCo[3 * c] * sRc[3 * c + lane]; atomicAdd(sg + lane, a); }
        }
        const size_t fo2 = (size_t)buf * n_frames + f;
        if (lane < 6) {
            double a = 0.0;
            if (shut) for (int c = 0; c < C; c++) a += sCo[3 * c + 1 + lane / 3] * sRc[3 * c + lane % 3];
            sh.gx[fo2 * 6 + lane] = a;
        }
        for (int t = lane; t < 9 * C; t += WAVE) { const int c = t / 9, e = t - 9 * c; sh.rcb[(fo2 * C + c) * 9 + e] = e < 3 ? sRc[3 * c + e] : sMc[6 * c + e - 3]; }
        wave_lds_sync();
    }

    FSTAMP(5);
    double fb = 0.0, vm = 0.0;
    if (lane < nbnd) {
        const double kp = M->bound_penalty;
        const double v = sq[bq & 255] + (((bq >> 16) & 255) ? sq[((bq >> 16) & 255) - 1] : 0.0)
                         - (((bq >> 8) & 255) ? sq[((bq >> 8) & 255) - 1] + (((bq >> 24) & 255) ? sq[((bq >> 24) & 255) - 1] : 0.0) : 0.0);
        double* mp = mu + (f * (size_t)nbnd + lane) * 2;
        double mu_up = pf_mu.x, mu_lo = pf_mu.y;
        const double du = v - b_up, dlo = b_lo - v;
        if (pend) {
            mu_up = fmax(0.0, mu_up + kp * du); mu_lo = fmax(0.0, mu_lo + kp * dlo);
            mp[0] = mu_up; mp[1] = mu_lo;
        }
        vm = fmax(0.0, fmax(du, dlo));
        const double pu = fmax(0.0, mu_up + kp * du), pl = fmax(0.0, mu_lo + kp * dlo);
        fb = (pu * pu - mu_up * mu_up + pl * pl - mu_lo * mu_lo) / (2.0 * kp);
        if (pu > 0.0 || pl > 0.0) {
            const double gv = pu - pl, hv = kp * ((pu > 0.0 ? 1.0 : 0.0) + (pl > 0.0 ? 1.0 : 0.0));
            const int ka = M->bound_ua[lane], kb = M->bound_ub[lane];
            int col[8]; double val[8]; int nz = 0;
            for (int side = 0; side < 2; side++) {
                const int k = side == 0 ? ka : kb;
                if (k < 0) continue;
                const double sgn = side == 0 ? 1.0 : -1.0;
                const int r = M->rev_of_u[k];
                if (r < 0) { col[nz] = k; val[nz++] = sgn; }
                else {
                    col[nz] = k; val[nz++] = sgn * sgam[GAM_STRIDE * r];
                    for (int a = 0; a < 3; a++) { col[nz] = M->rev_body_u[r][a]; val[nz++] = sgn * sgam[GAM_STRIDE * r + 1 + a]; }
                }
            }
            if (PLAIN) __builtin_amdgcn_s_waitcnt(0x0F70);
            for (int i = 0; i < nz; i++) {
                atomicAdd(sg + col[i], gv * val[i]);
                for (int j = 0; j < nz; j++) atomicAdd((PLAIN ? Bo : sH) + col[i] * nu + col[j], hv * val[i] * val[j]);
            }
        }
    }
    fb = wave_sum(fb);
    vm = wave_max(vm);
    wave_lds_sync();

    FSTAMP(6);
    double fpz = 0.0;
    if (pri && pri->p.gmm_k > 0) {
        const int K = pri->p.gmm_k, D = pri->p.gmm_dim, off = nu - D;
        double* sxv = sDp + 3 * mct;
        double* sv = sxv + CPE_NX;
        double* slp = sv + K * D;
        double* sgr = slp + CPE_MAX_GMM;
        if (lane < D) {
            const int k = off + lane, r = M->rel_ref_u[k];
            sxv[lane] = M->rel_sign_u[k] * (cost_coord(M, sq, k) - (r >= 0 ? cost_coord(M, sq, r) : 0.0));
        }
        wave_lds_sync();
        constexpr int CH = 8;
        for (int t = lane; t < K * D; t += WAVE) {
            const int k = t / D, i = t - k * D;
            double a = 0.0;
            for (int j0 = 0; j0 < D; j0 += CH) {
                double pq[CH], mq[CH];
#pragma unroll
                for (int u = 0; u < CH; u++) { const int j = j0 + u < D ? j0 + u : D - 1; pq[u] = pri->gmm_PT[k][j][i]; mq[u] = pri->p.gmm_mu[k][j]; }
#pragma unroll
                for (int u = 0; u < CH; u++) if (j0 + u < D) a += pq[u] * (sxv[j0 + u] - mq[u]);
            }
            sv[t] = a;
        }
        wave_lds_sync();
        if (lane < K) {
            double qf = 0.0;
            for (int i0 = 0; i0 < D; i0 += CH) {
                double mq[CH];
#pragma unroll
                for (int u = 0; u < CH; u++) mq[u] = pri->p.gmm_mu[lane][i0 + u < D ? i0 + u : D - 1];
#pragma unroll
                for (int u = 0; u < CH; u++) if (i0 + u < D) qf += sv[lane * D + i0 + u] * (sxv[i0 + u] - mq[u]);
            }
            slp[lane] = pri->p.gmm_logw[lane] - 0.5 * qf;
        }
        wave_lds_sync();
        double mx = -1e300, sum = 0.0;
        for (int k = 0; k < K; k++) mx = fmax(mx, slp[k]);
        for (int k = 0; k < K; k++) sum += exp(slp[k] - mx);
        const double dens = sum * exp(mx) + 1e-12;
        fpz = -log(dens);
        double resp[CPE_MAX_GMM];
#pragma unroll
        for (int k = 0; k < CPE_MAX_GMM; k++) resp[k] = k < K ? exp(slp[k]) / dens : 0.0;
        if (lane < D) {
            double a = 0.0;
#pragma unroll
            for (int k = 0; k < CPE_MAX_GMM; k++) if (k < K) a += resp[k] * sv[k * D + lane];
            sgr[lane] = a;
        }
        wave_lds_sync();
        if (lane < nu) {
            double a = 0.0;
            for (int i0 = 0; i0 < D; i0 += CH) {
                double xq[CH];
#pragma unroll
                for (int u = 0; u < CH; u++) xq[u] = pri->Xc[off + (i0 + u < D ? i0 + u : D - 1)][lane];
#pragma unroll
                for (int u = 0; u < CH; u++) if (i0 + u < D) a += xq[u] * sgr[i0 + u];
            }
            sg[lane] += a;
        }
        for (int t0 = lane; t0 < nu * nu; t0 += 2 * WAVE) {
            const int t1 = t0 + WAVE;
            const bool h1 = t1 < nu * nu;
            const int t1c = h1 ? t1 : t0;
            double q0[CPE_MAX_GMM], q1[CPE_MAX_GMM];
#pragma unroll
            for (int k = 0; k < CPE_MAX_GMM; k++) { const int kc = k < K ? k : K - 1; q0[k] = pri->gmm_Q[kc][t0]; q1[k] = pri->gmm_Q[kc][t1c]; }
            double a0 = 0.0, a1 = 0.0;
#pragma unroll
            for (int k = 0; k < CPE_MAX_GMM; k++) { a0 += resp[k] * q0[k]; a1 += resp[k] * q1[k]; }
            sH[t0] += a0;
            if (h1) sH[t1] += a1;
        }
        wave_lds_sync();
    }

    FSTAMP(7);
    if (!PLAIN) for (int t = lane; t < nu * nu; t += WAVE) Bo[t] = sH[t];
    if (lane < nu) gbuf[fo * nu + lane] = sg[lane];
    if (lane == 0) {
        double* cb = costbuf + fo * COST_STRIDE;
        cb[0] = fc; cb[1] = fb; cb[2] = fpz; cb[3] = 0.0; cb[4] = vm; cb[5] = 0.0;
    }
    FSTAMP(8);
}

template <bool RAGGED = false>
__global__ __launch_bounds__(WAVE) void k_lr_band(const DevModel* __restrict__ M, const SeqState* __restrict__ st, int N, int which,
                                                  size_t n_frames, const double* __restrict__ qbuf, const double* __restrict__ gambuf,
                                                  const DevPriors* __restrict__ pri, int nk, double* __restrict__ gbuf, double* __restrict__ Bbuf,
                                                  double* __restrict__ Hlr, double* __restrict__ costbuf, const int* __restrict__ act,
                                                  const int* __restrict__ n_act, RaggedArgs rg = RaggedArgs{}) {
    if (n_act && (int)(blockIdx.x / (unsigned)N) >= *n_act) return;
    __shared__ double sx[(2 * CPE_MAX_WINDOW + 1) * CPE_NX];
    __shared__ double ssl[(CPE_MAX_WINDOW + 1) * CPE_NX];
    __shared__ double sgx[CPE_NX];
    __shared__ double sgu[CPE_NX];
    const int lane = threadIdx.x;
    const int b = act ? act[blockIdx.x / (unsigned)N] : (int)(blockIdx.x / (unsigned)N), a = (int)(blockIdx.x % (unsigned)N);
    const size_t f = (size_t)b * N + a;
    int NL = N;
    if constexpr (RAGGED) {
        const int2 rs = rg.seq[b];
        if (a >= rs.y) return;
        M += rs.x; NL = rs.y;
    }
    const SeqState S = st[b];
    if (S.status != 0) return;
    const int buf = (which || S.al_pending) ? S.cur : 1 - S.cur;
    const int nu = M->nu, ns = M->ns, W = pri->p.lr_window;
    const double* qs = qbuf + ((size_t)buf * n_frames + (size_t)b * N) * ns;
    (void)gambuf;
    const size_t fo = (size_t)buf * n_frames + f;

    for (int t = lane; t < (2 * W + 1) * nu; t += WAVE) {
        const int d = t / nu, k = t - d * nu, n = a - W + d;
        double v = 0.0;
        if (n >= 0 && n < NL) {
            const double* qn = qs + (size_t)n * ns;
            const int r = M->rel_ref_u[k];
            v = M->rel_sign_u[k] * (cost_coord(M, qn, k) - (r >= 0 ? cost_coord(M, qn, r) : 0.0));
        }
        sx[t] = v;
    }
    wave_lds_sync();
    double fl = 0.0;
    for (int t = lane; t < (W + 1) * nu; t += WAVE) {
        const int d = t / nu, p = t - d * nu, n = a + d;
        double sl = 0.0;
        if (n >= W && n < NL) {
            sl = sx[(d + W) * nu + p] - pri->p.lr_b[p];
            const double* xs = sx + d * nu;
            for (int e = 0; e < pri->lr_nf; e++) { const int ft = pri->lr_feat[e]; sl -= pri->lr_coefT[ft][p] * xs[ft]; }
        }
        const double w = pri->p.lr_w[p];
        if (d == 0) fl += w * sl * sl;
        ssl[t] = 2.0 * w * sl;
    }
    fl = wave_sum(fl);
    wave_lds_sync();
    if (lane < nu) {
        double gacc = ssl[lane];
        for (int d = 1; d <= W; d++) {
            const int tt = W - d;
            const double* sn = ssl + d * nu;
            for (int p = 0; p < nu; p++) gacc -= pri->p.lr_coef[p][tt * nu + lane] * sn[p];
        }
        sgx[lane] = gacc;
    }
    wave_lds_sync();
    if (lane < nu) { double gacc = 0.0; for (int r = 0; r < nu; r++) gacc += pri->Xc[r][lane] * sgx[r]; sgu[lane] = gacc; }
    wave_lds_sync();
    if (lane < nu) gbuf[fo * nu + lane] += sgu[lane];
    const bool row_interior = a >= W && a <= NL - W;
    for (int k = 0; k <= nk && k <= a; k++) {
        if (k > 0 && row_interior) break;
        const int ta_lo = k > a - NL + 1 + W ? k : a - NL + 1 + W, ta_hi = W < a ? W : a;
        const bool interior = ta_lo == k && ta_hi == W;
        for (int t = lane; t < nu * nu; t += WAVE) {
            double v = 0.0;
            if (interior) v = pri->lr_HIu[k][t];
            else for (int ta = ta_lo; ta <= ta_hi; ta++) v += pri->lr_PKu[ta][ta - k][t];
            if (k == 0) Bbuf[fo * (nu * nu) + t] += v;
            else Hlr[(fo * nk + (k - 1)) * (nu * nu) + t] = v;
        }
// ... 5 lines not shown
    __shared__ int wcnt[4];
    __shared__ int base;
    const int tid = threadIdx.x, lane = tid & 63, wave = __builtin_amdgcn_readfirstlane(tid >> 6);
#ifdef CPE_LM_STAMPS
    unsigned long long* g_tu = nullptr;
#endif
    if (tid == 0) base = 0;
    __syncthreads();
    for (int b0 = 0; b0 < B; b0 += 256) {
        const int b = b0 + tid;
        const bool run = b < B && st[b].status == 0;
        const unsigned long long m = __ballot(run);
        if (lane == 0) wcnt[wave] = __popcll(m);
        __syncthreads();
        int off = base;
        for (int w = 0; w < wave; w++) off += wcnt[w];
        const int idx = off + __popcll(m & ((1ull << lane) - 1ull));
        if (run && idx < window) act[idx] = b;
        __syncthreads();
        if (tid == 0) base += wcnt[0] + wcnt[1] + wcnt[2] + wcnt[3];
        __syncthreads();
        if (base >= window) break;
    }
    if (tid == 0) *n_act = base < window ? base : window;
}

__global__ __launch_bounds__(WAVE) void k_shutter_step(const DevModel* __restrict__ M, const SeqState* __restrict__ st, int N, size_t n_frames,
                                                       const double* __restrict__ qbuf, const double* __restrict__ rcb,
                                                       const double* __restrict__ tau, double* __restrict__ step ) {
    const int b = blockIdx.x, lane = threadIdx.x, C = M->C, ns = M->ns;
    const int cur = st[b].cur;
    const double* qs = qbuf + ((size_t)cur * n_frames + (size_t)b * N) * ns;
    const double ih = 1.0 / M->h;
    if (lane == 0) step[(size_t)b * C] = 0.0;
    for (int c = 1; c < C; c++) {
        const double ta = tau[(size_t)b * C + c];
        double g = 0.0, hh = 0.0;
        for (int n = 2 + lane; n < N; n += WAVE) {
            const double* r = rcb + (((size_t)cur * n_frames + (size_t)b * N + n) * C + c) * 9;
            double t3[3];
            for (int d = 0; d < 3; d++) {
                const double x0 = qs[(size_t)n * ns + d], x1 = qs[(size_t)(n - 1) * ns + d], x2 = qs[(size_t)(n - 2) * ns + d];
                t3[d] = (x0 - x1) * ih + 2.0 * ta * (x0 - 2.0 * x1 + x2) * ih * ih;
            }
            g += t3[0] * r[0] + t3[1] * r[1] + t3[2] * r[2];
            hh += t3[0] * (r[3] * t3[0] + r[4] * t3[1] + r[5] * t3[2]) + t3[1] * (r[4] * t3[0] + r[6] * t3[1] + r[7] * t3[2]) + t3[2] * (r[5] * t3[0] + r[7] * t3[1] + r[8] * t3[2]);
        }
        g = wave_sum(g); hh = wave_sum(hh);
        if (lane == 0) step[(size_t)b * C + c] = hh > 0.0 ? -g / hh : 0.0;
    }
}

__global__ void k_gather_normal(const DevModel* __restrict__ M, size_t F, const double* __restrict__ qbuf, const double* __restrict__ costbuf,
                                const double* __restrict__ gambuf, double* __restrict__ cost, double* __restrict__ gam, double* __restrict__ q_out) {
    const size_t f = blockIdx.x;
    const int t = threadIdx.x, nq = M->nq, ns = M->ns, GS = GAM_STRIDE * M->nrev;
    if (t < 3) cost[3 * f + t] = costbuf[f * COST_STRIDE + t];
    if (gam && t < GS) gam[f * GS + t] = gambuf[f * GS + t];
    if (q_out && t < nq) q_out[f * nq + t] = qbuf[f * ns + t];
}

__device__ __forceinline__ double readlane_f64(double v, int l) {
    int lo = __double2loint(v), hi = __double2hiint(v);
    lo = __builtin_amdgcn_readlane(lo, l);
    hi = __builtin_amdgcn_readlane(hi, l);
    return __hiloint2double(hi, lo);
}

__device__ __forceinline__ double motion_T(int i, int k, int N) {
    const double c[4] = {-1.0, 3.0, -3.0, 1.0};
    double s = 0.0;
#pragma unroll
    for (int t = 0; t < 4; t++)
        if (t >= k && t <= i && t >= i + 4 - N) s += c[t] * c[t - k];
    return s;
}

template <int RING>
__device__ __forceinline__ int blk_slot(int r, int c) {
    const int ri = r % RING, ci = c % RING;
    if (ri == ci) return ri;
    const int lo = ri < ci ? ri : ci, hi = ri < ci ? ci : ri;
    return RING + lo * RING - lo * (lo + 1) / 2 + (hi - lo - 1);
}

__device__ __forceinline__ double rsqrt_f64(double x) {
    double y = __builtin_amdgcn_rsq(x);
    y = y * (1.5 - 0.5 * x * y * y);
    y = y * (1.5 - 0.5 * x * y * y);
    return y;
}

__device__ __forceinline__ double rcp_f64(double x) {
    double y = __builtin_amdgcn_rcp(x);
    y = y * fma(-x, y, 2.0);
    y = y * fma(-x, y, 2.0);
    return y;
}

__device__ __forceinline__ bool wave_factor_panel(const double* src, double* dst , bool store_lower_only,
                                                  double* colbuf , double* invd_out , int lane,
                                                  int ident = -1 ) {
    static_assert(NU % 4 == 0, "groups of four columns");
    double a[NU];
#pragma unroll
    for (int j = 0; j < NU; j++) a[j] = src[j];
    if (ident >= 0) {
#pragma unroll
        for (int j = 0; j < NU; j++) a[j] = j == ident ? 1.0 : 0.0;
    }
    bool ok = true;
// ... 55 lines not shown
}
__device__ __forceinline__ void mfma_frag_cols(const double* blk, int col0, int lane, double (&f)[7]) {
    const double* p = blk + (lane >> 4) * LDB + col0 + (lane & 15);
#pragma unroll
    for (int s = 0; s < 7; s++) f[s] = p[4 * s * LDB];
}

#define LM_LDS_BLOCKS 21
__host__ __device__ constexpr size_t lm_spill_doubles(int pb) {
    return (pb + 1) * (pb + 2) / 2 <= LM_LDS_BLOCKS ? 0 : (size_t)((pb + 1) * (pb + 2) / 2 - LM_LDS_BLOCKS) * BLK + 4 * LDB;
}
template <int RING>
__device__ __forceinline__ double* win_blk(double* W, double* Wg, int slot) {
    constexpr int NLDS = RING * (RING + 1) / 2 < LM_LDS_BLOCKS ? RING * (RING + 1) / 2 : LM_LDS_BLOCKS;
    if constexpr (RING * (RING + 1) / 2 <= LM_LDS_BLOCKS) { (void)Wg; return W + slot * BLK; }
    else return slot < NLDS ? W + slot * BLK : Wg + (slot - NLDS) * BLK;
}

template <int RING, int CNT>
__device__ __forceinline__ void p2_tiles(double* W, int n, int i, int tr, int g0, const double (&xa)[7], int lane, double* Wg = nullptr) {
    constexpr int SPLIT = CNT <= 2 ? 2 : 1;
    double xb[CNT][7];
    d4_t acc[CNT][SPLIT];
#pragma unroll
    for (int q = 0; q < CNT; q++) {
        const int idx = g0 + q;
        mfma_frag_rows(win_blk<RING>(W, Wg, blk_slot<RING>(n + 1 + idx / 2, n)), 16 * (idx & 1), lane, xb[q]);
#pragma unroll
        for (int h = 0; h < SPLIT; h++) acc[q][h] = d4_t{0.0, 0.0, 0.0, 0.0};
    }
#pragma unroll
    for (int s2 = 0; s2 < 7; s2++)
#pragma unroll
        for (int q = 0; q < CNT; q++) acc[q][s2 % SPLIT] = __builtin_amdgcn_mfma_f64_16x16x4f64(xa[s2], xb[q][s2], acc[q][s2 % SPLIT], 0, 0, 0);
#pragma unroll
    for (int q = 0; q < CNT; q++) {
        const int idx = g0 + q, j = 1 + idx / 2, col = 16 * (idx & 1) + (lane & 15);
        double* Cd = win_blk<RING>(W, Wg, blk_slot<RING>(n + i, n + j));
#pragma unroll
        for (int r = 0; r < 4; r++) {
            const int row = 16 * tr + (lane >> 4) + 4 * r;
            const double v = SPLIT == 2 ? acc[q][0][r] + acc[q][SPLIT - 1][r] : acc[q][0][r];
            if (row < NU && col < NU) Cd[row * LDB + col] -= v;
        }
    }
}

template <int PB, int MODE = 0, bool RAGGED = false>
__global__ __launch_bounds__(LM_THREADS, PB == 3 ? 2 : 1) void k_lm_step(const DevModel* __restrict__ M, SeqState* __restrict__ st,
                                                        LmParams prm, int first, double* __restrict__ qbuf,
                                                        const double* __restrict__ gbuf, const double* __restrict__ Bbuf,
                                                        const double* __restrict__ costbuf, double* __restrict__ Lbuf,
                                                        double* __restrict__ zbuf, double* __restrict__ gtbuf,
                                                        const double* __restrict__ gambuf, const double* __restrict__ Hlr,
                                                        const int* __restrict__ act ,
                                                        const int* __restrict__ n_act , int hb = 2,
                                                        const double* __restrict__ gxbuf = nullptr ,
                                                        double* __restrict__ dgbuf = nullptr ,
                                                        const double* __restrict__ HIu = nullptr ,
                                                        int lrW = 0 , RaggedArgs rg = RaggedArgs{}) {
    if (n_act && (int)blockIdx.x >= *n_act) return;
    constexpr int RING = PB + 1;
    constexpr int NBLK = RING * (RING + 1) / 2;
    constexpr int NRH = 2 * PB;
    constexpr int NLDS = NBLK < LM_LDS_BLOCKS ? NBLK : LM_LDS_BLOCKS, NSPILL = NBLK - NLDS;
    static_assert(PB >= 3 && PB <= 6, "the tile deal of P2 below is written for PB = 3..6");
    __shared__ double W[NLDS * BLK];
    __shared__ __attribute__((aligned(16))) double colbuf[NU * 4];
    __shared__ double dummy_row[NU + 4];
    __shared__ double Tm[BLK + 4 * LDB];
    __shared__ double smw[NU];
    __shared__ int sindep[NU];
    constexpr int RG = RING + 1;
    __shared__ double gamw[RG * LM_MAX_REV * GAM_STRIDE];
    __shared__ double marr[2 * NU];
    __shared__ double sgc[2 * NU];
    __shared__ int s_cnt[4];
    __shared__ int mterm[LM_MAX_TERMS + LM_MAX_GROUP];
    __shared__ int srev_of_u[NU], sja[NU], srev_u[LM_MAX_REV], srbu[LM_MAX_REV * 3], slegs_n[NU], slegs[NU * LM_MAX_LEGS];
    __shared__ int scoord_of_state[CPE_MAX_NQ + CPE_MAX_JOINTS];
    __shared__ double rw[RING * NU];
    __shared__ double invd[NU];
    __shared__ double red[16];
    __shared__ int s_int[4];
    __shared__ double s_dbl[4];

    const int tid = threadIdx.x, lane = tid & 63, wave = __builtin_amdgcn_readfirstlane(tid >> 6);
#ifdef CPE_LM_STAMPS
    unsigned long long* g_tu = nullptr;
#endif
    const int b = act ? act[blockIdx.x] : (int)blockIdx.x, NS = prm.N;
    int N = NS;
    if constexpr (RAGGED) { const int2 rs = rg.seq[b]; M += rs.x; N = rs.y; }
    const int nq = M->ns;
    const int nrev = M->nrev, GS = GAM_STRIDE * nrev;
    const size_t n_frames = (size_t)prm.B * NS;
    SeqState S = st[b];
    if (S.status != 0) return;
#ifdef CPE_LM_STAMPS
    unsigned long long t_last = __builtin_amdgcn_s_memtime();
#endif

    if (MODE == 2) { if (S.al_pending) return; }
    if (MODE != 2) {
        const int mode = first ? 1 : (S.al_pending ? 2 : 0);
        const int eb = mode ? S.cur : 1 - S.cur;
        const double* cb = costbuf + ((size_t)eb * n_frames + (size_t)b * NS) * COST_STRIDE;
        const double* qe = qbuf + (size_t)eb * n_frames * nq + (size_t)b * NS * nq;
        double acc[6] = {0, 0, 0, 0, 0, 0};
        double vmax = 0.0;
        for (int n = tid; n < N; n += LM_THREADS) {
            const double* c = cb + (size_t)n * COST_STRIDE;
            acc[0] += c[0]; acc[2] += c[1]; acc[3] += c[2]; acc[4] += c[3]; acc[5] += c[5]; vmax = fmax(vmax, c[4]);
        }
        for (int t = tid; t < N * NU; t += LM_THREADS) {
            const int n = t / NU, k = t - n * NU;
            const double wk = M->motion_w_u[k];
            if (n >= 3 && wk != 0.0) {
                const double* qf = qe + (size_t)n * nq;
                const double e = (cost_coord(M, qf, k) - 3.0 * cost_coord(M, qf - nq, k) + 3.0 * cost_coord(M, qf - 2 * nq, k) - cost_coord(M, qf - 3 * nq, k)) * M->ih2;
                acc[1] += wk * e * e;
            }
        }
        double tot[6];
        for (int v = 0; v < 6; v++) {
            double x = wave_sum(acc[v]);
            __syncthreads();
            if (lane == 0) red[wave] = x;
            __syncthreads();
            tot[v] = red[0] + red[1] + red[2] + red[3];
        }
        vmax = wave_max(vmax);
        __syncthreads();
        if (lane == 0) red[wave] = vmax;
        __syncthreads();
        vmax = fmax(fmax(red[0], red[1]), fmax(red[2], red[3]));
        if (tid == 0) {
            double total = tot[0] + tot[1] + tot[2] + tot[3] + tot[5];
            if (tot[4] > 0.0 || !isfinite(total)) total = INFINITY;
            bool inner_done = false;
            if (mode == 1) {
                S.cost_cur = total; S.lambda = prm.lambda0; S.nu = LM_NU0; S.iters = 0; S.rejects = 0; S.outer = 0; S.al_pending = 0; S.fresh = 1;
                S.maxviol = vmax;
                S.terms[0] = tot[0]; S.terms[1] = tot[1]; S.terms[2] = tot[2]; S.terms[3] = tot[3]; S.terms[4] = tot[5];
                if (!isfinite(total)) S.status = 2;
            } else if (mode == 2) {
                S.cost_cur = total; S.maxviol = vmax; S.al_pending = 0; S.nu = LM_NU0; S.fresh = 1;
                if (S.lambda > 1e-3) S.lambda = 1e-3;
                S.terms[0] = tot[0]; S.terms[1] = tot[1]; S.terms[2] = tot[2]; S.terms[3] = tot[3]; S.terms[4] = tot[5];
            } else {
                S.iters++;
                const double act = S.cost_cur - total;
                const double gain = S.pred > 0.0 ? act / S.pred : -1.0;
                if (isfinite(total) && act > 0.0 && gain > 1e-4) {
                    const double rel = act / (fabs(S.cost_cur) + 1e-30);
                    S.cur = 1 - S.cur; S.cost_cur = total; S.maxviol = vmax; S.fresh = 1;
                    S.terms[0] = tot[0]; S.terms[1] = tot[1]; S.terms[2] = tot[2]; S.terms[3] = tot[3]; S.terms[4] = tot[5];
                    const double t3 = 2.0 * gain - 1.0, fl = 1.0 - t3 * t3 * t3;
                    S.lambda *= fl > 1.0 / 3.0 ? fl : 1.0 / 3.0; S.nu = LM_NU0;
                    if (S.lambda < 1e-12) S.lambda = 1e-12;
                    if (S.maxstep < prm.tol_step || rel < prm.tol_cost) inner_done = true;
                } else {
                    S.lambda *= S.nu; S.nu *= 2.0; S.rejects++; S.fresh = 0;
                    if (S.maxstep < prm.tol_step * 1e-2 || S.lambda > 1e14) inner_done = true;
                }
            }
            if (inner_done) {
                if (S.maxviol > prm.bound_tol && S.outer < prm.max_outer) { S.outer++; S.al_pending = 1; }
                else S.status = 1;
            }
            if (S.status == 0 && !S.al_pending && S.iters >= prm.max_iter) S.status = 3;
            st[b] = S;
            s_int[0] = S.cur; s_int[1] = S.status; s_int[3] = S.al_pending; s_dbl[0] = S.lambda;
        }
        __syncthreads();
        S.cur = s_int[0]; S.status = s_int[1]; S.lambda = s_dbl[0];
        if (S.status != 0 || s_int[3]) return;
    }
    if (MODE == 1) return;

    STAMP(0);
    const int cur = S.cur;
    const double lam = S.lambda;
    const double* qc = qbuf + (size_t)cur * n_frames * nq + (size_t)b * NS * nq;
    const size_t hcur = hb == 2 ? (size_t)cur * n_frames : 0;
    const double* gc = gbuf + (hcur + (size_t)b * NS) * NU;
    const double* Bc = Bbuf + (hcur + (size_t)b * NS) * (NU * NU);
    double* Lb = Lbuf + (size_t)b * NS * RING * (NU * NU);
    double* Wg = nullptr;
    if constexpr (NSPILL > 0) Wg = Lbuf + n_frames * RING * (NU * NU) + (size_t)b * lm_spill_doubles(PB);
    double* zb = zbuf + (size_t)b * NS * NU;
    double* gtb = gtbuf + (size_t)b * NS * NU;
    double* dgb = dgbuf + (size_t)b * NS * NU;
    const double mscale = 2.0 * M->ih2 * M->ih2;

    if (tid < NU) {
        smw[tid] = mscale * M->motion_w_u[tid]; sindep[tid] = M->ucost[tid];
        srev_of_u[tid] = M->rev_of_u[tid]; sja[tid] = M->bodyang_j[tid]; slegs_n[tid] = M->bodyang_legs_n[tid];
        for (int i = 0; i < M->bodyang_legs_n[tid]; i++) slegs[tid * LM_MAX_LEGS + i] = M->bodyang_legs[tid][i];
    }
    if (tid < nrev) { srev_u[tid] = M->rev_u[tid]; for (int a = 0; a < 3; a++) srbu[3 * tid + a] = M->rev_body_u[tid][a]; }
    for (int t = tid; t < nq; t += LM_THREADS) scoord_of_state[t] = -1;
    __syncthreads();
    if (tid < NU) scoord_of_state[M->ucoord_src[tid]] = tid;
    const double* gamc = gambuf + ((size_t)cur * n_frames + (size_t)b * NS) * GS;
    const double* Hlc = Hlr ? Hlr + (hcur + (size_t)b * NS) * PB * (NU * NU) : nullptr;
    __syncthreads();

    auto mot = [&](int i, int j, const double* Ga, const double* Gb) -> double {
        const int ri = srev_of_u[i], rj = srev_of_u[j];
        if (ri >= 0 && rj >= 0) return ri == rj ? Ga[GAM_STRIDE * ri] * smw[i] * Gb[GAM_STRIDE * ri] : 0.0;
        if (ri >= 0) { const int jb = sja[j]; return (jb >= 0 && srbu[3 * ri + jb] == j) ? Ga[GAM_STRIDE * ri] * smw[i] * Gb[GAM_STRIDE * ri + 1 + jb] : 0.0; }
        if (rj >= 0) { const int ja = sja[i]; return (ja >= 0 && srbu[3 * rj + ja] == i) ? Ga[GAM_STRIDE * rj + 1 + ja] * smw[j] * Gb[GAM_STRIDE * rj] : 0.0; }
        double v = i == j ? smw[i] : 0.0;
        const int ja = sja[i], jb = sja[j];
        if (ja >= 0 && jb >= 0)
            for (int e = 0; e < slegs_n[i]; e++) {
                const int r = slegs[i * LM_MAX_LEGS + e];
                if (srbu[3 * r + jb] == j) v += Ga[GAM_STRIDE * r + 1 + ja] * smw[srev_u[r]] * Gb[GAM_STRIDE * r + 1 + jb];
            }
        return v;
    };

    constexpr int UT = LM_THREADS - WAVE, NPB = (NU * NU + UT - 1) / UT;
    const int ut = tid - WAVE;
    double pb[NPB], pbh = 0.0;
    int hcnt = 0, ht = 0;

    auto lds_release = [&]() {
        if constexpr (NSPILL > 0) __builtin_amdgcn_fence(__ATOMIC_RELEASE, "workgroup");
        else __builtin_amdgcn_fence(__ATOMIC_RELEASE, "workgroup", "local");
    };
    auto wait_ge = [&](int idx, int target) {
        while (__atomic_load_n(&s_cnt[idx], __ATOMIC_RELAXED) < target) __builtin_amdgcn_s_sleep(1);
        if constexpr (NSPILL > 0) __builtin_amdgcn_fence(__ATOMIC_ACQUIRE, "workgroup");
        else __builtin_amdgcn_fence(__ATOMIC_ACQUIRE, "workgroup", "local");
    };
    int sync_epoch = 0;
    auto sync3 = [&]() {
        lds_release();
        if (lane == 0) atomicAdd(&s_cnt[3], 1);
        sync_epoch += 3;
        wait_ge(3, sync_epoch);
    };
    if (tid == 0) { s_int[0] = 0; s_int[1] = 0; }
    __syncthreads();
    constexpr int HEAVY_MAX = (LM_MAX_TERMS + LM_MAX_GROUP) / 8;
    int* elist = reinterpret_cast<int*>(W);
    if (tid == 0) { s_int[1] = 0; s_int[3] = 0; }
    __syncthreads();
#pragma unroll
    for (int j = 0; j < NPB; j++) {
        const int t = ut + UT * j;
        if (ut >= 0 && t < NU * NU) {
            const int a = t / NU, c = t - a * NU;
            const int ri = srev_of_u[a], rj = srev_of_u[c];
            int codes[LM_MAX_GROUP], cnt = 0;
            auto emit = [&](int oa, int ob, int wi) { if (cnt < LM_MAX_GROUP) codes[cnt++] = (oa << 10) | (ob << 16) | (wi << 22); };
            if (ri >= 0 && rj >= 0) { if (ri == rj) emit(GAM_STRIDE * ri, GAM_STRIDE * ri, a); }
            else if (ri >= 0) { const int jb = sja[c]; if (jb >= 0 && srbu[3 * ri + jb] == c) emit(GAM_STRIDE * ri, GAM_STRIDE * ri + 1 + jb, a); }
            else if (rj >= 0) { const int ja = sja[a]; if (ja >= 0 && srbu[3 * rj + ja] == a) emit(GAM_STRIDE * rj + 1 + ja, GAM_STRIDE * rj, c); }
            else {
                if (a == c) emit(63, 63, a);
                const int ja = sja[a], jb = sja[c];
                if (ja >= 0 && jb >= 0)
                    for (int e = 0; e < slegs_n[a]; e++) {
                        const int r = slegs[a * LM_MAX_LEGS + e];
                        if (srbu[3 * r + jb] == c) emit(GAM_STRIDE * r + 1 + ja, GAM_STRIDE * r + 1 + jb, srev_u[r]);
                    }
            }
            const int where = (a * LDB + c) | (a == c ? 1 << 30 : 0);
            if (cnt == 0) elist[NU * NU - 1 - atomicAdd(&s_int[3], 1)] = where;
            else if (cnt == 1) elist[atomicAdd(&s_int[1], 1)] = where | codes[0] | (1 << 28);
            else {
                const int h = atomicAdd(&s_int[0], 1);
                if (h < HEAVY_MAX) {
                    for (int g = 0; g < LM_MAX_GROUP; g++) mterm[8 * h + g] = g < cnt ? codes[g] : 0;
                    mterm[8 * h + 7] = (cnt << 16) | t;
                }
            }
        }
    }
    __syncthreads();
    const int n_term = s_int[1], n_plain = s_int[3];
    (void)n_plain;
    const int npa = (n_term + UT - 1) / UT;
    int my_code[NPB];
    auto elem_of = [&](int code) -> int { const int off = code & 1023; return (off / LDB) * NU + off % LDB; };
#pragma unroll
    for (int j = 0; j < NPB; j++) {
        const int i = ut + UT * j;
        int code = 1 << 31;
        if (ut >= 0) {
            if (i < n_term) code = elist[i];
            else if (i - n_term < n_plain) code = elist[NU * NU - 1 - (i - n_term)];
        }
        my_code[j] = code;
    }
    auto fetch_B = [&](int m) {
#pragma unroll
        for (int j = 0; j < NPB; j++) if (my_code[j] >= 0) pb[j] = Bc[(size_t)m * (NU * NU) + elem_of(my_code[j])];
        if (hcnt > 0) pbh = Bc[(size_t)m * (NU * NU) + ht];
    };
    __syncthreads();
    const int n_heavy = s_int[0];
    const bool list_ok = n_heavy <= HEAVY_MAX && n_heavy <= WAVE;
    const int hsel = ut - WAVE, gsel = ut - 2 * WAVE;
    int hcode[LM_MAX_GROUP];
#pragma unroll
    for (int g = 0; g < LM_MAX_GROUP; g++) hcode[g] = 0;
    if (list_ok && hsel >= 0 && hsel < n_heavy) {
#pragma unroll
        for (int g = 0; g < LM_MAX_GROUP; g++) hcode[g] = mterm[8 * hsel + g];
        hcnt = mterm[8 * hsel + 7] >> 16; ht = mterm[8 * hsel + 7] & 0xffff;
    }
    int gl[LM_MAX_LEGS], gl_n = 0, gl_own = -1;
#pragma unroll
    for (int e = 0; e < LM_MAX_LEGS; e++) gl[e] = 0;
    if (gsel >= 0 && gsel < NU) {
        const int r = srev_of_u[gsel];
        if (r >= 0) gl_own = GAM_STRIDE * r;
        else {
            const int ja = sja[gsel];
            if (ja >= 0) {
                gl_n = slegs_n[gsel];
#pragma unroll
                for (int e = 0; e < LM_MAX_LEGS; e++)
                    if (e < gl_n) { const int rr = slegs[gsel * LM_MAX_LEGS + e]; gl[e] = (GAM_STRIDE * rr + 1 + ja) | (srev_u[rr] << 8); }
            }
        }
    }
    double st_gam = 0.0, st_tu = 0.0, st_gv = 0.0;
    auto stage_load = [&](int m) {
        st_gam = lane < GS ? gamc[(size_t)m * GS + lane] : 0.0;
        if (lane < NU) {
            const int p = sindep[lane] & 255, p2 = (sindep[lane] >> 8) - 1;
            double tu = 0.0;
#pragma unroll
            for (int j = -3; j <= 3; j++) {
                const int mj = m + j;
                if (mj < 0 || mj >= N) continue;
                const double T = j <= 0 ? motion_T(m, -j, N) : motion_T(mj, j, N);
                tu += T * (qc[(size_t)mj * nq + p] + (p2 >= 0 ? qc[(size_t)mj * nq + p2] : 0.0));
            }
            st_tu = tu;
            double gv = gc[(size_t)m * NU + lane];
            if (gxbuf && lane < 3) {
                const double* gxc = gxbuf + ((size_t)cur * n_frames + (size_t)b * NS) * 6;
                if (m + 1 < N) gv += gxc[(size_t)(m + 1) * 6 + lane];
                if (m + 2 < N) gv += gxc[(size_t)(m + 2) * 6 + 3 + lane];
            }
            st_gv = gv;
        }
    };
    auto stage_store = [&](int m) {
        if (lane < GS) gamw[(m % RG) * GS + lane] = st_gam;
        if (lane < NU) { marr[(m & 1) * NU + lane] = smw[lane] * st_tu; sgc[(m & 1) * NU + lane] = st_gv; }
    };
    auto store_row = [&](int m) {
        const double* Gm = gamw + (m % RG) * GS;
        double Tk[4];
        int base[PB + 1];
#pragma unroll
        for (int k = 0; k <= 3; k++) Tk[k] = m - k >= 0 ? motion_T(m, k, N) : 0.0;
#pragma unroll
        for (int k = 0; k <= PB; k++) base[k] = blk_slot<RING>(m, m - k >= 0 ? m - k : m) * BLK;
        const double* Gk[4];
#pragma unroll
        for (int k = 0; k <= 3; k++) Gk[k] = gamw + ((m - k >= 0 ? m - k : m) % RG) * GS;
        const bool prior = Hlc != nullptr;
        const double* Hrow = prior ? ((HIu && m >= lrW && m <= N - lrW) ? HIu : Hlc + (size_t)m * PB * (NU * NU)) : nullptr;
        auto wput = [&](int bo, int off, double v) {
            if constexpr (NSPILL == 0) W[bo + off] = v;
            else { if (bo < NLDS * BLK) W[bo + off] = v; else Wg[bo - NLDS * BLK + off] = v; }
        };
        auto put = [&](int t, int where, double bval, const double (&acc)[4]) {
            const int off = where & 1023;
            double v = bval + Tk[0] * acc[0];
            if (where & (1 << 30)) { dgb[(size_t)m * NU + off / (LDB + 1)] = v; v += lam * fmax(v, LM_DIAG_FLOOR(N)); }
            W[base[0] + off] = v;
            if (prior) {
#pragma unroll
                for (int k = 1; k <= PB; k++)
                    if (m - k >= 0) wput(base[k], off, Hrow[(k - 1) * (NU * NU) + t] + (k <= 3 ? Tk[k] * acc[k] : 0.0));
            } else {
#pragma unroll
                for (int k = 1; k <= PB; k++)
                    if (m - k >= 0) wput(base[k], off, k <= 3 ? Tk[k] * acc[k] : 0.0);
            }
        };
#pragma unroll
        for (int j = 0; j < NPB; j++) {
            int code = my_code[j];
            asm volatile("" : "+v"(code));
            if (code >= 0) {
                const int t = prior ? elem_of(code) : 0;
                if (j < npa) {
                    const int oa = (code >> 10) & 63, ob = (code >> 16) & 63, wi = (code >> 22) & 31;
                    const int oac = oa == 63 ? 0 : oa, obc = ob == 63 ? 0 : ob;
                    const double sw = smw[wi], ga = Gm[oac];
                    double gb[4];
#pragma unroll
                    for (int k = 0; k <= 3; k++) gb[k] = Gk[k][obc];
                    const double wa = (code & (1 << 28)) ? sw * (oa == 63 ? 1.0 : ga) : 0.0;
                    double acc[4];
#pragma unroll
                    for (int k = 0; k <= 3; k++) acc[k] = wa * (ob == 63 ? 1.0 : gb[k]);
                    put(t, code, pb[j], acc);
                } else {
                    const double acc[4] = {0.0, 0.0, 0.0, 0.0};
                    put(t, code, pb[j], acc);
                }
            }
        }
        RSTAMP(14);
        if (hcnt > 0) {
            double sw[LM_MAX_GROUP], ga[LM_MAX_GROUP], gb[LM_MAX_GROUP][4];
            int hc[LM_MAX_GROUP];
#pragma unroll
            for (int g = 0; g < LM_MAX_GROUP; g++) { hc[g] = hcode[g]; asm volatile("" : "+v"(hc[g])); }
#pragma unroll
            for (int g = 0; g < LM_MAX_GROUP; g++) {
                const int oa = (hc[g] >> 10) & 63, ob = (hc[g] >> 16) & 63, wi = (hc[g] >> 22) & 31;
                sw[g] = smw[wi]; ga[g] = Gm[oa == 63 ? 0 : oa];
#pragma unroll
                for (int k = 0; k <= 3; k++) gb[g][k] = Gk[k][ob == 63 ? 0 : ob];
            }
            double acc[4] = {0.0, 0.0, 0.0, 0.0};
#pragma unroll
            for (int g = 0; g < LM_MAX_GROUP; g++) {
                const int oa = (hc[g] >> 10) & 63, ob = (hc[g] >> 16) & 63;
                const bool on = g < hcnt;
                const double wa = on ? sw[g] * (oa == 63 ? 1.0 : ga[g]) : 0.0;
#pragma unroll
                for (int k = 0; k <= 3; k++) acc[k] += wa * (ob == 63 || !on ? 1.0 : gb[g][k]);
            }
            const int a = ht / NU, c = ht - a * NU;
            put(ht, (a * LDB + c) | (a == c ? 1 << 30 : 0), pbh, acc);
        }
        RSTAMP(15);
        if (gsel >= 0 && gsel < NU) {
            const double* mar = marr + (m & 1) * NU;
            const double own = mar[gsel], gown = Gm[gl_own >= 0 ? gl_own : 0];
            double lg[LM_MAX_LEGS], lm[LM_MAX_LEGS];
#pragma unroll
            for (int e = 0; e < LM_MAX_LEGS; e++) { lg[e] = Gm[gl[e] & 255]; lm[e] = mar[gl[e] >> 8]; }
            double gm = gl_own >= 0 ? gown * own : own;
#pragma unroll
            for (int e = 0; e < LM_MAX_LEGS; e++) gm += e < gl_n ? lg[e] * lm[e] : 0.0;
            const double gt = sgc[(m & 1) * NU + gsel] + gm;
            gtb[(size_t)m * NU + gsel] = gt;
            rw[(m % RING) * NU + gsel] = -gt;
        }
    };

    if (tid < 4) s_cnt[tid] = 0;
    if (tid == 0) s_int[2] = list_ok ? 0 : 1;
    for (int t = tid; t < BLK + 4 * LDB; t += LM_THREADS) Tm[t] = 0.0;
    __syncthreads();
    STAMP(1);

    if (s_int[2]) {
    } else if (wave == 0) {
        __builtin_amdgcn_s_setprio(3);
        for (int m = 0; m < RING && m < N; m++) {
            if (m >= 2) wait_ge(3, 3 * (m - 1));
            stage_load(m); stage_store(m);
            lds_release();
            if (lane == 0) __atomic_store_n(&s_cnt[1], m + 1, __ATOMIC_RELAXED);
        }
        const int rows0 = N < RING ? N : RING;
        wait_ge(3, 3 * rows0);
        for (int n = 0; n < N; n++) {
            double* D00 = W + blk_slot<RING>(n, n) * BLK;
            if (n + RING < N) stage_load(n + RING);
            if (n >= 1) {
                wait_ge(3, 3 * (rows0 + 3 * (n - 1) + 1));
                STAMP(3);
                const double* X1 = win_blk<RING>(W, Wg, blk_slot<RING>(n, n - 1));
                if (lane < NU) {
                    const double* Li = X1 + lane * LDB;
                    const double* z = rw + ((n - 1) % RING) * NU;
                    double acc0 = 0.0, acc1 = 0.0;
#pragma unroll
                    for (int k = 0; k < NU; k += 2) { acc0 = fma(Li[k], z[k], acc0); acc1 = fma(Li[k + 1], z[k + 1], acc1); }
                    rw[(n % RING) * NU + lane] -= acc0 + acc1;
                }
                double xa[7];
                mfma_frag_rows(X1, 0, lane, xa);
                p2_tiles<RING, 1>(W, n - 1, 1, 0, 0, xa, lane, Wg);
                mfma_frag_rows(X1, 16, lane, xa);
                p2_tiles<RING, 2>(W, n - 1, 1, 1, 0, xa, lane, Wg);
                lds_release();
                if (lane == 0) __atomic_store_n(&s_cnt[2], n, __ATOMIC_RELAXED);
            }
            STAMP(6);
            const double* src;
            double* dst;
            int ident = -1;
            if (lane < NU) { src = D00 + lane * LDB; dst = D00 + lane * LDB; }
            else if (lane < 2 * NU) { ident = lane - NU; src = dummy_row; dst = Tm + ident * LDB; }
            else if (lane == 2 * NU) { src = rw + (n % RING) * NU; dst = rw + (n % RING) * NU; }
            else { src = dummy_row; dst = dummy_row; }
            const bool ok = wave_factor_panel(src, dst, lane < NU, colbuf, invd, lane, ident);
            if (!ok && lane == 0) s_int[2] = 1;
            lds_release();
            if (lane == 0) __atomic_store_n(&s_cnt[0], n + 1, __ATOMIC_RELAXED);
            STAMP(2);
            if (!ok) break;
            if (n + RING < N) {
                stage_store(n + RING);
                lds_release();
                if (lane == 0) __atomic_store_n(&s_cnt[1], n + RING + 1, __ATOMIC_RELAXED);
            }
            STAMP(1);
        }
// ... 701 lines not shown
```

cheetah_pose_estimation_amd/csrc/cpe_tracked.hip.inc:

```

struct DevTrack {
    double w[CPE_NX];
    double Xt[CPE_NX][CPE_NX];
    double H[CPE_NX * CPE_NX];
};

template <bool RAGGED = false>
__global__ __launch_bounds__(WAVE) void k_track_target(const DevModel* __restrict__ M, const double* __restrict__ q, double* __restrict__ xt,
                                                      RaggedArgs rg = RaggedArgs{}) {
    __shared__ double ss[CPE_MAX_NQ + LM_MAX_REV];
    const int lane = threadIdx.x;
    const size_t f = blockIdx.x;
    if constexpr (RAGGED) {
        const int2 rs = rg.seq[f / (unsigned)rg.nmax];
        if ((int)(f % (unsigned)rg.nmax) >= rs.y) return;
        M += rs.x;
    }
    const int nq = M->nq;
    if (lane < nq) ss[lane] = q[f * nq + lane];
    if (lane < M->nrev) {
        const double* qb = q + f * nq + 3 + 3 * M->rev_body[lane];
        const double* qc = q + f * nq + 3 + 3 * M->rev_child[lane];
        double scb[6], scc[6], RB[9], RC[9];
        for (int a = 0; a < 3; a++) { sincos(qb[a], &scb[2 * a], &scb[2 * a + 1]); sincos(qc[a], &scc[2 * a], &scc[2 * a + 1]); }
        rot_kind(scb, 0, RB); rot_kind(scc, 0, RC);
        const double m00 = RB[0] * RC[0] + RB[3] * RC[3] + RB[6] * RC[6], m02 = RB[0] * RC[2] + RB[3] * RC[5] + RB[6] * RC[8];
        ss[nq + lane] = atan2(m02, m00);
    }
    wave_lds_sync();
    if (lane < M->nu) {
        const int r = M->rel_ref_u[lane];
        xt[f * CPE_NX + lane] = M->rel_sign_u[lane] * (cost_coord(M, ss, lane) - (r >= 0 ? cost_coord(M, ss, r) : 0.0));
    }
}

template <bool GMM, bool RAGGED = false>
__global__ __launch_bounds__(WAVE) void k_frame_tracked(const DevModel* __restrict__ M, const DevTrack* __restrict__ T, const SeqState* __restrict__ st,
                                                        int N, int which, size_t n_frames, double* __restrict__ qbuf, const double* __restrict__ xt,
                                                        double* __restrict__ gbuf, double* __restrict__ Bbuf, double* __restrict__ costbuf,
                                                        double* __restrict__ mu, double* __restrict__ gambuf, const DevPriors* __restrict__ pri,
                                                        const int* __restrict__ act, const int* __restrict__ n_act, RaggedArgs rg = RaggedArgs{}) {
    extern __shared__ double smem[];
    const int lane = threadIdx.x;
    if (n_act && (int)(blockIdx.x / (unsigned)N) >= *n_act) return;
    const int b = act ? act[blockIdx.x / (unsigned)N] : (int)(blockIdx.x / (unsigned)N);
    if constexpr (RAGGED) {
        const int2 rs = rg.seq[b];
        if ((int)(blockIdx.x % (unsigned)N) >= rs.y) return;
        M += rs.x; T += rs.x;
    }
    const size_t f = (size_t)b * N + blockIdx.x % (unsigned)N;
    const SeqState S = st[b];
    if (S.status != 0) return;
    const int pend = S.al_pending;
    const int buf = (which || pend) ? S.cur : 1 - S.cur;

    const int nq = M->nq, nl = M->nl, nu = M->nu, nrev = M->nrev, ns = M->ns;
    double* sq = smem;
    double* sal = sq + nq;
    double* ssc = sq + ns;
    double* ssa = ssc + 6 * nl;
    double* sR = ssa + 2 * nrev;
    double* sgam = sR + 36 * M->n_trunk;
    double* sres = sgam + GAM_STRIDE * nrev;
    double* sH = sres + nu;
    double* sg = sH + nu * nu;
    const int4 fw = *reinterpret_cast<const int4*>(M->fn_lane[lane]);
    double* stf = qbuf + (size_t)buf * n_frames * ns + f * ns;
    for (int t = lane; t < ns; t += WAVE) sq[t] = stf[t];
    const double xtg = lane < nu ? xt[f * CPE_NX + lane] : 0.0;
    const int nbnd = M->nb;
    double2 pf_mu = make_double2(0.0, 0.0);
    if (nbnd > 0) pf_mu = reinterpret_cast<const double2*>(mu)[f * (size_t)nbnd + (lane < nbnd ? lane : nbnd - 1)];
    wave_lds_sync();
    wave_sincos(M, sq, ssc, lane);
    if (lane < nrev) { double s_, c_; sincos(sal[lane], &s_, &c_); ssa[2 * lane] = s_; ssa[2 * lane + 1] = c_; }
    wave_lds_sync();
    for (int level = 0; level < 2; level++) {
        if (lane < M->hj_n && ((fw.x >> 16) & 1) == level) {
            const int p = fw.x & 255, c = (fw.x >> 8) & 255;
            double a[3];
            rot_ycol(ssc + 6 * p, a);
            const double st_ = ssc[6 * c + 2], ct = ssc[6 * c + 3], sp = ssc[6 * c + 4], cp = ssc[6 * c + 5];
            const double num = a[0] * st_ * cp + a[1] * st_ * sp + a[2] * ct;
            const double den = a[1] * cp - a[0] * sp;
            const double hyp = sqrt(num * num + den * den);
            sq[3 + 3 * c] = atan2(num, den);
            ssc[6 * c] = num / hyp; ssc[6 * c + 1] = den / hyp;
        }
        wave_lds_sync();
    }
    if (lane < 4 * M->n_trunk) rot_kind(ssc + 6 * fw.y, lane & 3, sR + 9 * lane);
    for (int t = WAVE + lane; t < 4 * M->n_trunk; t += WAVE) rot_kind(ssc + 6 * M->trunk_link[t >> 2], t & 3, sR + 9 * t);
    wave_lds_sync();
    if (lane < nrev) {
        const int Bk = fw.z & 255, c = (fw.z >> 8) & 255;
        double e[3], gtrue[GAM_STRIDE];
        leg_euler(sR + 36 * (fw.z >> 16), ssc + 6 * Bk, ssa[2 * lane], ssa[2 * lane + 1], sq[3 + 3 * Bk + 2], e, gtrue);
        sq[3 + 3 * c] = e[0]; sq[3 + 3 * c + 1] = e[1]; sq[3 + 3 * c + 2] = e[2];
        sgam[GAM_STRIDE * lane] = 1.0; sgam[GAM_STRIDE * lane + 1] = 0.0; sgam[GAM_STRIDE * lane + 2] = 1.0; sgam[GAM_STRIDE * lane + 3] = 0.0;
    }
    double ft = 0.0;
    if (lane < nu) {
        const int r = M->rel_ref_u[lane];
        const double d = M->rel_sign_u[lane] * (cost_coord(M, sq, lane) - (r >= 0 ? cost_coord(M, sq, r) : 0.0)) - xtg;
        const double w = T->w[lane];
        ft = w * d * d;
        sres[lane] = 2.0 * w * d;
    }
    for (int t = lane; t < nu * nu; t += WAVE) sH[t] = T->H[t];
    wave_lds_sync();
    if (lane < nq) stf[lane] = sq[lane];
    if (lane < GAM_STRIDE * nrev) gambuf[((size_t)buf * n_frames + f) * (GAM_STRIDE * nrev) + lane] = sgam[lane];
    if (lane < nu) {
        double a = 0.0;
        for (int k = 0; k < nu; k++) a += T->Xt[lane][k] * sres[k];
        sg[lane] = a;
    }
    ft = wave_sum(ft);
    wave_lds_sync();

    double fb = 0.0, vm = 0.0;
    if (lane < nbnd) {
        const int bq = M->bnd_q[lane];
        const double b_lo = M->bound_lo[lane], b_up = M->bound_up[lane];
        const double kp = M->bound_penalty;
        const double v = sq[bq & 255] + (((bq >> 16) & 255) ? sq[((bq >> 16) & 255) - 1] : 0.0)
                         - (((bq >> 8) & 255) ? sq[((bq >> 8) & 255) - 1] + (((bq >> 24) & 255) ? sq[((bq >> 24) & 255) - 1] : 0.0) : 0.0);
        double* mp = mu + (f * (size_t)nbnd + lane) * 2;
        double mu_up = pf_mu.x, mu_lo = pf_mu.y;
        const double du = v - b_up, dlo = b_lo - v;
        if (pend) {
            mu_up = fmax(0.0, mu_up + kp * du); mu_lo = fmax(0.0, mu_lo + kp * dlo);
            mp[0] = mu_up; mp[1] = mu_lo;
        }
        vm = fmax(0.0, fmax(du, dlo));
        const double pu = fmax(0.0, mu_up + kp * du), pl = fmax(0.0, mu_lo + kp * dlo);
        fb = (pu * pu - mu_up * mu_up + pl * pl - mu_lo * mu_lo) / (2.0 * kp);
        if (pu > 0.0 || pl > 0.0) {
            const double gv = pu - pl, hv = kp * ((pu > 0.0 ? 1.0 : 0.0) + (pl > 0.0 ? 1.0 : 0.0));
            const int ka = M->bound_ua[lane], kb = M->bound_ub[lane];
            int col[8]; double val[8]; int nz = 0;
            for (int side = 0; side < 2; side++) {
                const int k = side == 0 ? ka : kb;
                if (k < 0) continue;
                const double sgn = side == 0 ? 1.0 : -1.0;
                const int r = M->rev_of_u[k];
                if (r < 0) { col[nz] = k; val[nz++] = sgn; }
                else {
                    col[nz] = k; val[nz++] = sgn * sgam[GAM_STRIDE * r];
                    for (int a = 0; a < 3; a++) { col[nz] = M->rev_body_u[r][a]; val[nz++] = sgn * sgam[GAM_STRIDE * r + 1 + a]; }
                }
            }
            for (int i = 0; i < nz; i++) {
                atomicAdd(sg + col[i], gv * val[i]);
                for (int j = 0; j < nz; j++) atomicAdd(sH + col[i] * nu + col[j], hv * val[i] * val[j]);
            }
        }
    }
    fb = wave_sum(fb);
    vm = wave_max(vm);
    wave_lds_sync();

    double fpz = 0.0;
    if constexpr (GMM) {
        const int K = pri->p.gmm_k, D = pri->p.gmm_dim, off = nu - D;
        double* sxv = sg + nu;
        double* sv = sxv + CPE_NX;
        double* slp = sv + K * D;
        double* sgr = slp + CPE_MAX_GMM;
        if (lane < D) {
            const int k = off + lane, r = M->rel_ref_u[k];
            sxv[lane] = M->rel_sign_u[k] * (cost_coord(M, sq, k) - (r >= 0 ? cost_coord(M, sq, r) : 0.0));
        }
        wave_lds_sync();
        constexpr int CH = 8;
        for (int t = lane; t < K * D; t += WAVE) {
            const int k = t / D, i = t - k * D;
            double a = 0.0;
            for (int j0 = 0; j0 < D; j0 += CH) {
                double pq[CH], mq[CH];
#pragma unroll
                for (int u = 0; u < CH; u++) { const int j = j0 + u < D ? j0 + u : D - 1; pq[u] = pri->gmm_PT[k][j][i]; mq[u] = pri->p.gmm_mu[k][j]; }
#pragma unroll
                for (int u = 0; u < CH; u++) if (j0 + u < D) a += pq[u] * (sxv[j0 + u] - mq[u]);
            }
            sv[t] = a;
        }
        wave_lds_sync();
        if (lane < K) {
            double qf = 0.0;
            for (int i0 = 0; i0 < D; i0 += CH) {
                double mq[CH];
#pragma unroll
                for (int u = 0; u < CH; u++) mq[u] = pri->p.gmm_mu[lane][i0 + u < D ? i0 + u : D - 1];
#pragma unroll
                for (int u = 0; u < CH; u++) if (i0 + u < D) qf += sv[lane * D + i0 + u] * (sxv[i0 + u] - mq[u]);
            }
            slp[lane] = pri->p.gmm_logw[lane] - 0.5 * qf;
        }
        wave_lds_sync();
        double mx = -1e300, sum = 0.0;
        for (int k = 0; k < K; k++) mx = fmax(mx, slp[k]);
        for (int k = 0; k < K; k++) sum += exp(slp[k] - mx);
// ... 49 lines not shown
```

Before: 148.7 million frames/s.

## Precompute constant motion-cost Hessian on host and drop per-frame gamma buffers

```diff
diff --git a/cheetah_pose_estimation_amd/csrc/cpe_api.hip b/cheetah_pose_estimation_amd/csrc/cpe_api.hip
--- a/cheetah_pose_estimation_amd/csrc/cpe_api.hip
+++ b/cheetah_pose_estimation_amd/csrc/cpe_api.hip
@@ -31,7 +31,7 @@
     size_t ws_frames = 0; int ws_B = 0;
     std::vector<void**> ws_bufs;
     double *qbuf = nullptr, *gbuf = nullptr, *Bbuf = nullptr, *costbuf = nullptr, *Lbuf = nullptr, *zbuf = nullptr,
-           *gtbuf = nullptr, *dgbuf = nullptr, *cmax = nullptr, *mu = nullptr, *gambuf = nullptr;
+           *gtbuf = nullptr, *dgbuf = nullptr, *cmax = nullptr, *mu = nullptr;
     SeqState* st = nullptr;
     int* flag = nullptr;
     int* act = nullptr;
@@ -88,6 +88,46 @@
            sc * (a * b - 0.5 * a * a + 0.5 * a * cb);
 }
 
+static void build_motion_constants(DevModel& m) {
+    const int nu = m.nu;
+    double w[CPE_NX];
+    const double mscale = 2.0 * m.ih2 * m.ih2;
+    for (int k = 0; k < nu; k++) w[k] = mscale * m.motion_w_u[k];
+    for (int a = 0; a < nu; a++)
+        for (int c = 0; c < nu; c++) {
+            double term[1 + CPE_MAX_BODY_LEGS];
+            int cnt = 0;
+            auto emit = [&](double ga, double gb, int wi) { const double wa = w[wi] * ga; term[cnt++] = wa * gb; };
+            const int ri = m.rev_of_u[a], rj = m.rev_of_u[c];
+            if (ri >= 0 && rj >= 0) { if (ri == rj) emit(cpe_cost_gamma(0), cpe_cost_gamma(0), a); }
+            else if (ri >= 0) { const int jb = m.bodyang_j[c]; if (jb >= 0 && m.rev_body_u[ri][jb] == c) emit(cpe_cost_gamma(0), cpe_cost_gamma(1 + jb), a); }
+            else if (rj >= 0) { const int ja = m.bodyang_j[a]; if (ja >= 0 && m.rev_body_u[rj][ja] == a) emit(cpe_cost_gamma(1 + ja), cpe_cost_gamma(0), c); }
+            else {
+                if (a == c) emit(1.0, 1.0, a);
+                const int ja = m.bodyang_j[a], jb = m.bodyang_j[c];
+                if (ja >= 0 && jb >= 0)
+                    for (int e = 0; e < m.bodyang_legs_n[a]; e++) {
+                        const int r = m.bodyang_legs[a][e];
+                        if (m.rev_body_u[r][jb] == c) emit(cpe_cost_gamma(1 + ja), cpe_cost_gamma(1 + jb), m.rev_u[r]);
+                    }
+            }
+            double q = 0.0;
+            if (cnt == 1) q = term[0];
+            else for (int g = 0; g < cnt; g++) q += term[g];
+            m.mot_Q[a * nu + c] = q;
+        }
+    for (int k = 0; k < nu; k++) {
+        const int r = m.rev_of_u[k], ja = m.bodyang_j[k];
+        m.mot_gown[k] = r >= 0 ? cpe_cost_gamma(0) : 1.0;
+        m.mot_gn[k] = 0;
+        if (r < 0 && ja >= 0)
+            for (int e = 0; e < m.bodyang_legs_n[k]; e++) {
+                const int rr = m.bodyang_legs[k][e];
+                m.mot_gsrc[k][m.mot_gn[k]++] = m.rev_u[rr] | (cpe_cost_gamma(1 + ja) == 1.0 ? 1 << 8 : 0);
+            }
+    }
+}
+
 static cpe_status build_model(const cpe_skeleton* s, const cpe_camera* cams, int C, const cpe_options* o, DevModel& m) {
     memset(&m, 0, sizeof(m));
     if (s->n_links < 1 || s->n_links > CPE_MAX_LINKS || s->n_markers < 1 || s->n_markers > CPE_MAX_MARKERS ||
@@ -215,6 +255,7 @@
     if (m.nrev > LM_MAX_REV) return fail(CPE_BAD_ARG, "more than 12 leg links");
     for (int k = 0; k < nu; k++) if (m.bodyang_legs_n[k] > LM_MAX_LEGS) return fail(CPE_BAD_ARG, "more than 6 leg links on one body");
     for (int r = 0; r < m.nrev; r++) m.ucoord_src[m.rev_u[r]] = nq + r;
+    build_motion_constants(m);
     m.n_trunk = 0;
     for (int i = 0; i < nl; i++) { m.trunk_slot[i] = -1; if (rev_of_link[i] < 0) { m.trunk_slot[i] = m.n_trunk; m.trunk_link[m.n_trunk++] = i; } }
     int S = 0, mct = 0, ss = 0, sv = 0;
@@ -407,7 +448,7 @@
     size_t ov = CPE_MAX_SCOL * m.n_srow, hg = plain ? m.nu : m.nu * m.nu + m.nu;
     size_t camov = 6 * m.nl + 2 * m.nrev + 36 * m.n_trunk;
     if (camov < (size_t)22 * m.C) camov = (size_t)22 * m.C;
-    size_t n = m.ns + camov + 3 * m.L + 3 * m.sv_n + GAM_STRIDE * m.nrev + (ov > hg ? ov : hg) +
+    size_t n = m.ns + camov + 3 * m.L + 3 * m.sv_n + (ov > hg ? ov : hg) +
                9 * m.L + 3 * m.mc_total;
     if (gmm_k > 0) n += CPE_NX + gmm_k * gmm_dim + CPE_MAX_GMM + CPE_NX;
     if (shutter) n += 15 * m.C + 6 * m.L + 6;
@@ -426,7 +467,7 @@
 #define FRAME_TRACKED(gmm) ((gmm) ? k_frame_tracked<true> : k_frame_tracked<false>)
 #define FRAME_TRACKED_RAGGED(gmm) ((gmm) ? k_frame_tracked<true, true> : k_frame_tracked<false, true>)
 static size_t lds_tracked(const DevModel& m, int gmm_k, int gmm_dim) {
-    size_t n = m.ns + 6 * m.nl + 2 * m.nrev + 36 * m.n_trunk + GAM_STRIDE * m.nrev + m.nu + m.nu * m.nu + m.nu;
+    size_t n = m.ns + 6 * m.nl + 2 * m.nrev + 36 * m.n_trunk + m.nu + m.nu * m.nu + m.nu;
     if (gmm_k > 0) n += CPE_NX + gmm_k * gmm_dim + CPE_MAX_GMM + CPE_NX;
     return sizeof(double) * n;
 }
@@ -907,7 +948,6 @@
     const int nu = h->hm.nu;
     auto& w = h->ws_bufs;
     HIPCHK(ws_alloc(w, h->qbuf, 2 * F * h->hm.ns));
-    HIPCHK(ws_alloc(w, h->gambuf, 2 * F * (size_t)(GAM_STRIDE * (h->hm.nrev > 0 ? h->hm.nrev : 1))));
     HIPCHK(ws_alloc(w, h->gbuf, 2 * F * nu));
     HIPCHK(ws_alloc(w, h->Bbuf, 2 * F * nu * nu));
     HIPCHK(ws_alloc(w, h->costbuf, 2 * F * COST_STRIDE));
@@ -946,10 +986,10 @@
     if ((s = state_reset(h, B, N, q)) != CPE_OK) return s;
     const DevModel& m = h->hm;
     hipLaunchKernelGGL(FRAME_NORMAL(h->gmm_k == 0), dim3((unsigned)F), dim3(WAVE), lds_normal(m, h->gmm_k, h->gmm_dim), h->stream, h->dm, h->st, N, 1, F, h->qbuf, meas, weight,
-                       h->gbuf, h->Bbuf, h->costbuf, h->mu, h->gambuf, h->pri, nullptr, nullptr, ShutterArgs{nullptr, nullptr, nullptr}, RaggedArgs{});
+                       h->gbuf, h->Bbuf, h->costbuf, h->mu, h->pri, nullptr, nullptr, ShutterArgs{nullptr, nullptr, nullptr}, RaggedArgs{});
     HIPCHK(hipMemcpyAsync(g, h->gbuf, sizeof(double) * F * m.nu, hipMemcpyDeviceToDevice, h->stream));
     HIPCHK(hipMemcpyAsync(Bm, h->Bbuf, sizeof(double) * F * m.nu * m.nu, hipMemcpyDeviceToDevice, h->stream));
-    hipLaunchKernelGGL(k_gather_normal, dim3((unsigned)F), dim3(128), 0, h->stream, h->dm, F, h->qbuf, h->costbuf, h->gambuf, cost, gam, q_out);
+    hipLaunchKernelGGL(k_gather_normal, dim3((unsigned)F), dim3(128), 0, h->stream, h->dm, F, h->qbuf, h->costbuf, cost, gam, q_out);
     HIPCHK(hipGetLastError());
     return CPE_OK;
 }
@@ -1017,18 +1057,18 @@
     if (rg) {
         prof_begin(h, 0);
         hipLaunchKernelGGL(FRAME_NORMAL_RAGGED(h->gmm_k == 0), dim3(gf), dim3(WAVE), ldsn, h->stream, h->dm, h->st, N, first, Fw, h->qbuf, meas, weight,
-                           h->gbuf, h->Bbuf, h->costbuf, h->mu, h->gambuf, h->pri, act, n_act, ShutterArgs{nullptr, nullptr, nullptr}, *rg);
+                           h->gbuf, h->Bbuf, h->costbuf, h->mu, h->pri, act, n_act, ShutterArgs{nullptr, nullptr, nullptr}, *rg);
         prof_end(h);
         if (lr) {
             prof_begin(h, 1);
-            hipLaunchKernelGGL(k_lr_band<true>, dim3(gf), dim3(WAVE), 0, h->stream, h->dm, h->st, N, first, Fw, h->qbuf, h->gambuf, h->pri, h->pb, h->gbuf,
+            hipLaunchKernelGGL(k_lr_band<true>, dim3(gf), dim3(WAVE), 0, h->stream, h->dm, h->st, N, first, Fw, h->qbuf, h->pri, h->pb, h->gbuf,
                                h->Bbuf, h->Hlr, h->costbuf, act, n_act, *rg);
             prof_end(h);
         }
         prof_begin(h, 2);
         with_pb(h->pb, [&](auto pbc) {
             hipLaunchKernelGGL((k_lm_step<decltype(pbc)::value, 0, true>), dim3(slots), dim3(LM_THREADS), 0, h->stream, h->dm, h->st, prm, first, h->qbuf,
-                               h->gbuf, h->Bbuf, h->costbuf, h->Lbuf, h->zbuf, h->gtbuf, h->gambuf, h->Hlr, act, n_act, 2, nullptr, h->dgbuf, hiu, h->lr_window, *rg);
+                               h->gbuf, h->Bbuf, h->costbuf, h->Lbuf, h->zbuf, h->gtbuf, h->Hlr, act, n_act, 2, nullptr, h->dgbuf, hiu, h->lr_window, *rg);
         });
         prof_end(h);
         if (!back) return;
@@ -1042,18 +1082,18 @@
     }
     prof_begin(h, 0);
     hipLaunchKernelGGL(FRAME_NORMAL(h->gmm_k == 0 && sh.tau == nullptr), dim3(gf), dim3(WAVE), ldsn, h->stream, h->dm, h->st, N, first, Fw, h->qbuf, meas, weight, h->gbuf, h->Bbuf,
-                       h->costbuf, h->mu, h->gambuf, h->pri, act, n_act, sh, RaggedArgs{});
+                       h->costbuf, h->mu, h->pri, act, n_act, sh, RaggedArgs{});
     prof_end(h);
     if (lr) {
         prof_begin(h, 1);
-        hipLaunchKernelGGL(k_lr_band<>, dim3(gf), dim3(WAVE), 0, h->stream, h->dm, h->st, N, first, Fw, h->qbuf, h->gambuf, h->pri, h->pb, h->gbuf, h->Bbuf,
+        hipLaunchKernelGGL(k_lr_band<>, dim3(gf), dim3(WAVE), 0, h->stream, h->dm, h->st, N, first, Fw, h->qbuf, h->pri, h->pb, h->gbuf, h->Bbuf,
                            h->Hlr, h->costbuf, act, n_act);
         prof_end(h);
     }
     prof_begin(h, 2);
     with_pb(h->pb, [&](auto pbc) {
         hipLaunchKernelGGL((k_lm_step<decltype(pbc)::value, 0>), dim3(slots), dim3(LM_THREADS), 0, h->stream, h->dm, h->st, prm, first, h->qbuf, h->gbuf,
-                           h->Bbuf, h->costbuf, h->Lbuf, h->zbuf, h->gtbuf, h->gambuf, h->Hlr, act, n_act, 2, sh.gx, h->dgbuf, hiu, h->lr_window);
+                           h->Bbuf, h->costbuf, h->Lbuf, h->zbuf, h->gtbuf, h->Hlr, act, n_act, 2, sh.gx, h->dgbuf, hiu, h->lr_window);
     });
     prof_end(h);
     if (!back) return;
@@ -1482,14 +1522,14 @@
     const bool plain = h->gmm_k == 0;
     prof_begin(h, 0);
     if (xt) hipLaunchKernelGGL(RAGGED ? FRAME_TRACKED_RAGGED(!plain) : FRAME_TRACKED(!plain), dim3(gf), dim3(WAVE), ldsn, h->stream, h->dm, h->dtrack, h->st, N, first, Fw,
-                               h->qbuf, xt, h->gbuf, h->Bbuf, h->costbuf, h->mu, h->gambuf, h->pri, act, n_act, rg);
+                               h->qbuf, xt, h->gbuf, h->Bbuf, h->costbuf, h->mu, h->pri, act, n_act, rg);
     else hipLaunchKernelGGL(RAGGED ? FRAME_NORMAL_RAGGED(plain) : FRAME_NORMAL(plain), dim3(gf), dim3(WAVE), ldsn, h->stream, h->dm, h->st, N, first, Fw, h->qbuf, meas,
-                            weight, h->gbuf, h->Bbuf, h->costbuf, h->mu, h->gambuf, h->pri, act, n_act, ShutterArgs{nullptr, nullptr, nullptr}, rg);
+                            weight, h->gbuf, h->Bbuf, h->costbuf, h->mu, h->pri, act, n_act, ShutterArgs{nullptr, nullptr, nullptr}, rg);
     prof_end(h);
     launch_dyn_eval<RAGGED>(h, N, first, Fw, stance, act, n_act, slots, rg);
     prof_begin(h, 2);
     hipLaunchKernelGGL((k_lm_step<3, 1, RAGGED>), dim3(slots), dim3(LM_THREADS), 0, h->stream, h->dm, h->st, prm, first, h->qbuf, h->gbuf, h->Bbuf, h->costbuf,
-                       h->Lbuf, h->zbuf, h->gtbuf, h->gambuf, nullptr, act, n_act, 2, nullptr, h->dgbuf, nullptr, 0, rg);
+                       h->Lbuf, h->zbuf, h->gtbuf, nullptr, act, n_act, 2, nullptr, h->dgbuf, nullptr, 0, rg);
     prof_end(h);
     launch_dyn_pieces<RAGGED>(h, N, 0, Fw, act, n_act, slots, rg);
     prof_begin(h, 9);
@@ -1502,7 +1542,7 @@
     prof_end(h);
     prof_begin(h, 2);
     hipLaunchKernelGGL((k_lm_step<3, 2, RAGGED>), dim3(slots), dim3(LM_THREADS), 0, h->stream, h->dm, h->st, prm, first, h->qbuf, h->gk, h->Bk, h->costbuf,
-                       h->Lbuf, h->zbuf, h->gtbuf, h->gambuf, h->Hk, act, n_act, 1, nullptr, h->dgbuf, nullptr, 0, rg);
+                       h->Lbuf, h->zbuf, h->gtbuf, h->Hk, act, n_act, 1, nullptr, h->dgbuf, nullptr, 0, rg);
     prof_end(h);
     prof_begin(h, 7);
     hipLaunchKernelGGL((k_lm_back<3, RAGGED>), dim3(slots), dim3(2 * WAVE), 0, h->stream, h->dm, h->st, prm, h->qbuf, h->Lbuf, h->zbuf, h->gtbuf, h->dgbuf, act, n_act, rg);
@@ -1744,10 +1784,10 @@
     if ((s = state_reset(h, B, N, q)) != CPE_OK) return s;
     const DevModel& m = h->hm;
     hipLaunchKernelGGL(FRAME_TRACKED(h->gmm_k > 0), dim3((unsigned)F), dim3(WAVE), lds_tracked(m, h->gmm_k, h->gmm_dim), h->stream, h->dm, h->dtrack, h->st, N, 1, F,
-                       h->qbuf, h->xtgt, h->gbuf, h->Bbuf, h->costbuf, h->mu, h->gambuf, h->pri, nullptr, nullptr, RaggedArgs{});
+                       h->qbuf, h->xtgt, h->gbuf, h->Bbuf, h->costbuf, h->mu, h->pri, nullptr, nullptr, RaggedArgs{});
     HIPCHK(hipMemcpyAsync(g, h->gbuf, sizeof(double) * F * m.nu, hipMemcpyDeviceToDevice, h->stream));
     HIPCHK(hipMemcpyAsync(Bm, h->Bbuf, sizeof(double) * F * m.nu * m.nu, hipMemcpyDeviceToDevice, h->stream));
-    hipLaunchKernelGGL(k_gather_normal, dim3((unsigned)F), dim3(128), 0, h->stream, h->dm, F, h->qbuf, h->costbuf, h->gambuf, cost, gam, q_out);
+    hipLaunchKernelGGL(k_gather_normal, dim3((unsigned)F), dim3(128), 0, h->stream, h->dm, F, h->qbuf, h->costbuf, cost, gam, q_out);
     HIPCHK(hipGetLastError());
     return CPE_OK;
 }
@@ -1785,7 +1825,7 @@
     }
     const DevModel& m = h->hm;
     hipLaunchKernelGGL(FRAME_NORMAL(h->gmm_k == 0), dim3((unsigned)F), dim3(WAVE), lds_normal(m, h->gmm_k, h->gmm_dim), h->stream, h->dm, h->st, N, 1, F, h->qbuf, meas, weight,
-                       h->gbuf, h->Bbuf, h->costbuf, h->mu, h->gambuf, h->pri, nullptr, nullptr, ShutterArgs{nullptr, nullptr, nullptr}, RaggedArgs{});
+                       h->gbuf, h->Bbuf, h->costbuf, h->mu, h->pri, nullptr, nullptr, ShutterArgs{nullptr, nullptr, nullptr}, RaggedArgs{});
     launch_dyn_eval<>(h, N, 1, F, stance, nullptr, nullptr, B);
     launch_dyn_pieces<>(h, N, 1, F, nullptr, nullptr, B);
     if (band) {
diff --git a/cheetah_pose_estimation_amd/csrc/cpe_model.h b/cheetah_pose_estimation_amd/csrc/cpe_model.h
--- a/cheetah_pose_estimation_amd/csrc/cpe_model.h
+++ b/cheetah_pose_estimation_amd/csrc/cpe_model.h
@@ -13,6 +13,13 @@
 #define CPE_MAX_DEP 32
 #define CPE_MAX_SCOL 8
 #define CPE_MAX_SDYN 48
+#define CPE_MAX_BODY_LEGS 6
+#define CPE_GAM_STRIDE 4
+
+#if defined(__HIPCC__)
+__host__ __device__
+#endif
+static inline double cpe_cost_gamma(int i) { return (i == 0 || i == 2) ? 1.0 : 0.0; }
 
 struct DevModel {
     int32_t nl, L, C, nq, nu, S, nj, nb, ndep, curvature;
@@ -87,6 +94,10 @@
     int32_t bodyang_j[CPE_NX];
     int32_t bodyang_legs_n[CPE_NX];
     int32_t bodyang_legs[CPE_NX][CPE_MAX_JOINTS];
+    double mot_Q[CPE_NX * CPE_NX];
+    double mot_gown[CPE_NX];
+    int32_t mot_gn[CPE_NX];
+    int32_t mot_gsrc[CPE_NX][CPE_MAX_BODY_LEGS];
     int32_t trunk_link[CPE_MAX_LINKS];
     int32_t trunk_slot[CPE_MAX_LINKS];
     int32_t sv_kind[CPE_MAX_SDYN], sv_cnt[CPE_MAX_SDYN], sv_rev[CPE_MAX_SDYN][3];
diff --git a/cheetah_pose_estimation_amd/csrc/cpe_solver.hip.inc b/cheetah_pose_estimation_amd/csrc/cpe_solver.hip.inc
--- a/cheetah_pose_estimation_amd/csrc/cpe_solver.hip.inc
+++ b/cheetah_pose_estimation_amd/csrc/cpe_solver.hip.inc
@@ -25,9 +25,7 @@
 #define LM_DIAG_FLOOR(N) ((N) < 4 ? 0.1 : 1e-12)
 #define LM_NU0 8.0
 #define LM_MAX_REV 12
-#define LM_MAX_LEGS 6
-#define LM_MAX_TERMS 256
-#define LM_MAX_GROUP 7
+#define LM_MAX_LEGS CPE_MAX_BODY_LEGS
 
 struct LmParams {
     double tol_step, tol_cost, lambda0, bound_tol;
@@ -37,15 +35,14 @@
 
 #define COST_STRIDE 8
 
-#define GAM_STRIDE 4
+#define GAM_STRIDE CPE_GAM_STRIDE
 
 __device__ __forceinline__ double cost_coord(const DevModel* __restrict__ M, const double* __restrict__ state, int k) {
     const int w = M->ucost[k];
     return state[w & 255] + ((w >> 8) ? state[(w >> 8) - 1] : 0.0);
 }
 
-__device__ __forceinline__ void leg_euler(const double* RB, const double* scB, double sa, double ca, double psi_ref,
-                                          double* euler, double* gam) {
+__device__ __forceinline__ void leg_euler(const double* RB, double sa, double ca, double psi_ref, double* euler) {
     const double r00 = RB[0] * ca - RB[2] * sa, r10 = RB[3] * ca - RB[5] * sa, r20 = RB[6] * ca - RB[8] * sa;
     const double r21 = RB[7], r22 = RB[6] * sa + RB[8] * ca;
     double sth = -r20; sth = fmin(1.0, fmax(-1.0, sth));
@@ -53,14 +50,6 @@
     double psi = atan2(r10, r00);
     psi += 6.283185307179586476925286766559 * rint((psi_ref - psi) / 6.283185307179586476925286766559);
     euler[0] = phi; euler[1] = th; euler[2] = psi;
-    const double cth = sqrt(fmax(0.0, 1.0 - sth * sth));
-    const double icth = cth > 1e-300 ? 1.0 / cth : 0.0;
-    const double sphic = r21 * icth, cphic = r22 * icth;
-    const double sfB = scB[0], cfB = scB[1], stB = scB[2], ctB = scB[3];
-    gam[0] = cphic;
-    gam[1] = -sphic * sa;
-    gam[2] = cphic * cfB + sphic * ca * sfB;
-    gam[3] = cphic * sfB * ctB - sphic * (ca * cfB * ctB - sa * stB);
 }
 
 template <bool RAGGED = false>
@@ -93,7 +82,7 @@
                                                        double* __restrict__ qbuf, const double* __restrict__ meas,
                                                        const double* __restrict__ weight, double* __restrict__ gbuf,
                                                        double* __restrict__ Bbuf, double* __restrict__ costbuf,
-                                                       double* __restrict__ mu, double* __restrict__ gambuf,
+                                                       double* __restrict__ mu,
                                                        const DevPriors* __restrict__ pri, const int* __restrict__ act ,
                                                        const int* __restrict__ n_act ,
                                                        ShutterArgs sh = ShutterArgs{nullptr, nullptr, nullptr},
@@ -124,8 +113,7 @@
     double* spos = ssc + (n_camov > CAMW * C ? n_camov : CAMW * C);
     double* scam = ssc;
     double* sdyn = spos + 3 * L;
-    double* sgam = sdyn + 3 * svn;
-    double* sSv = sgam + GAM_STRIDE * nrev;
+    double* sSv = sdyn + 3 * svn;
     const int n_ov = CPE_MAX_SCOL * M->n_srow, n_hg = PLAIN ? nu : nu * nu + nu;
     double* sMv = sSv + (n_ov > n_hg ? n_ov : n_hg);
     double* sDp = sMv + 9 * L;
@@ -172,10 +160,8 @@
     if (lane < nrev) {
         const int Bk = fw.z & 255, c = (fw.z >> 8) & 255;
         double e[3];
-        double gtrue[GAM_STRIDE];
-        leg_euler(sR + 36 * (fw.z >> 16), ssc + 6 * Bk, ssa[2 * lane], ssa[2 * lane + 1], sq[3 + 3 * Bk + 2], e, gtrue);
+        leg_euler(sR + 36 * (fw.z >> 16), ssa[2 * lane], ssa[2 * lane + 1], sq[3 + 3 * Bk + 2], e);
         sq[3 + 3 * c] = e[0]; sq[3 + 3 * c + 1] = e[1]; sq[3 + 3 * c + 2] = e[2];
-        sgam[GAM_STRIDE * lane] = 1.0; sgam[GAM_STRIDE * lane + 1] = 0.0; sgam[GAM_STRIDE * lane + 2] = 1.0; sgam[GAM_STRIDE * lane + 3] = 0.0;
     }
     if (lane < svn) {
         double d0 = 0.0, d1 = 0.0, d2 = 0.0;
@@ -196,7 +182,6 @@
     }
     wave_lds_sync();
     if (lane < nq) stf[lane] = sq[lane];
-    if (lane < GAM_STRIDE * nrev) gambuf[((size_t)buf * n_frames + f) * (GAM_STRIDE * nrev) + lane] = sgam[lane];
 
     const int lm_ = lane < L ? lane : 0;
     int pco[CPE_MAX_CHAIN]; double pcv[CPE_MAX_CHAIN][3];
@@ -453,8 +438,8 @@
                 const int r = M->rev_of_u[k];
                 if (r < 0) { col[nz] = k; val[nz++] = sgn; }
                 else {
-                    col[nz] = k; val[nz++] = sgn * sgam[GAM_STRIDE * r];
-                    for (int a = 0; a < 3; a++) { col[nz] = M->rev_body_u[r][a]; val[nz++] = sgn * sgam[GAM_STRIDE * r + 1 + a]; }
+                    col[nz] = k; val[nz++] = sgn * cpe_cost_gamma(0);
+                    for (int a = 0; a < 3; a++) { col[nz] = M->rev_body_u[r][a]; val[nz++] = sgn * cpe_cost_gamma(1 + a); }
                 }
             }
             if (PLAIN) __builtin_amdgcn_s_waitcnt(0x0F70);
@@ -561,7 +546,7 @@
 
 template <bool RAGGED = false>
 __global__ __launch_bounds__(WAVE) void k_lr_band(const DevModel* __restrict__ M, const SeqState* __restrict__ st, int N, int which,
-                                                  size_t n_frames, const double* __restrict__ qbuf, const double* __restrict__ gambuf,
+                                                  size_t n_frames, const double* __restrict__ qbuf,
                                                   const DevPriors* __restrict__ pri, int nk, double* __restrict__ gbuf, double* __restrict__ Bbuf,
                                                   double* __restrict__ Hlr, double* __restrict__ costbuf, const int* __restrict__ act,
                                                   const int* __restrict__ n_act, RaggedArgs rg = RaggedArgs{}) {
@@ -584,7 +569,6 @@
     const int buf = (which || S.al_pending) ? S.cur : 1 - S.cur;
     const int nu = M->nu, ns = M->ns, W = pri->p.lr_window;
     const double* qs = qbuf + ((size_t)buf * n_frames + (size_t)b * N) * ns;
-    (void)gambuf;
     const size_t fo = (size_t)buf * n_frames + f;
 
     for (int t = lane; t < (2 * W + 1) * nu; t += WAVE) {
@@ -696,11 +680,11 @@
 }
 
 __global__ void k_gather_normal(const DevModel* __restrict__ M, size_t F, const double* __restrict__ qbuf, const double* __restrict__ costbuf,
-                                const double* __restrict__ gambuf, double* __restrict__ cost, double* __restrict__ gam, double* __restrict__ q_out) {
+                                double* __restrict__ cost, double* __restrict__ gam, double* __restrict__ q_out) {
     const size_t f = blockIdx.x;
     const int t = threadIdx.x, nq = M->nq, ns = M->ns, GS = GAM_STRIDE * M->nrev;
     if (t < 3) cost[3 * f + t] = costbuf[f * COST_STRIDE + t];
-    if (gam && t < GS) gam[f * GS + t] = gambuf[f * GS + t];
+    if (gam && t < GS) gam[f * GS + t] = cpe_cost_gamma(t % GAM_STRIDE);
     if (q_out && t < nq) q_out[f * nq + t] = qbuf[f * ns + t];
 }
 
@@ -862,7 +846,7 @@
                                                         const double* __restrict__ gbuf, const double* __restrict__ Bbuf,
                                                         const double* __restrict__ costbuf, double* __restrict__ Lbuf,
                                                         double* __restrict__ zbuf, double* __restrict__ gtbuf,
-                                                        const double* __restrict__ gambuf, const double* __restrict__ Hlr,
+                                                        const double* __restrict__ Hlr,
                                                         const int* __restrict__ act ,
                                                         const int* __restrict__ n_act , int hb = 2,
                                                         const double* __restrict__ gxbuf = nullptr ,
@@ -881,14 +865,9 @@
     __shared__ double Tm[BLK + 4 * LDB];
     __shared__ double smw[NU];
     __shared__ int sindep[NU];
-    constexpr int RG = RING + 1;
-    __shared__ double gamw[RG * LM_MAX_REV * GAM_STRIDE];
     __shared__ double marr[2 * NU];
     __shared__ double sgc[2 * NU];
     __shared__ int s_cnt[4];
-    __shared__ int mterm[LM_MAX_TERMS + LM_MAX_GROUP];
-    __shared__ int srev_of_u[NU], sja[NU], srev_u[LM_MAX_REV], srbu[LM_MAX_REV * 3], slegs_n[NU], slegs[NU * LM_MAX_LEGS];
-    __shared__ int scoord_of_state[CPE_MAX_NQ + CPE_MAX_JOINTS];
     __shared__ double rw[RING * NU];
     __shared__ double invd[NU];
     __shared__ double red[16];
@@ -903,7 +882,6 @@
     int N = NS;
     if constexpr (RAGGED) { const int2 rs = rg.seq[b]; M += rs.x; N = rs.y; }
     const int nq = M->ns;
-    const int nrev = M->nrev, GS = GAM_STRIDE * nrev;
     const size_t n_frames = (size_t)prm.B * NS;
     SeqState S = st[b];
     if (S.status != 0) return;
@@ -923,14 +901,31 @@
             const double* c = cb + (size_t)n * COST_STRIDE;
             acc[0] += c[0]; acc[2] += c[1]; acc[3] += c[2]; acc[4] += c[3]; acc[5] += c[5]; vmax = fmax(vmax, c[4]);
         }
-        for (int t = tid; t < N * NU; t += LM_THREADS) {
-            const int n = t / NU, k = t - n * NU;
-            const double wk = M->motion_w_u[k];
-            if (n >= 3 && wk != 0.0) {
-                const double* qf = qe + (size_t)n * nq;
-                const double e = (cost_coord(M, qf, k) - 3.0 * cost_coord(M, qf - nq, k) + 3.0 * cost_coord(M, qf - 2 * nq, k) - cost_coord(M, qf - 3 * nq, k)) * M->ih2;
-                acc[1] += wk * e * e;
-            }
+        constexpr int MU = 4;
+        const double ih2 = M->ih2;
+        for (int t0 = tid; t0 < N * NU; t0 += MU * LM_THREADS) {
+            double wk[MU], cv[MU][4];
+            bool on[MU];
+#pragma unroll
+            for (int u = 0; u < MU; u++) {
+                const int t = t0 + u * LM_THREADS, tc = t < N * NU ? t : tid;
+                const int n = tc / NU, k = tc - n * NU;
+                wk[u] = M->motion_w_u[k];
+                const int w = M->ucost[k], s0 = w & 255, s1 = (w >> 8) ? (w >> 8) - 1 : s0;
+                on[u] = t < N * NU && n >= 3 && wk[u] != 0.0;
+#pragma unroll
+                for (int i = 0; i < 4; i++) {
+                    const double* qf = qe + (size_t)(on[u] ? n - i : 0) * nq;
+                    const double a0 = qf[s0], a1 = qf[s1];
+                    cv[u][i] = a0 + ((w >> 8) ? a1 : 0.0);
+                }
+            }
+#pragma unroll
+            for (int u = 0; u < MU; u++)
+                if (on[u]) {
+                    const double e = (cv[u][0] - 3.0 * cv[u][1] + 3.0 * cv[u][2] - cv[u][3]) * ih2;
+                    acc[1] += wk[u] * e * e;
+                }
         }
         double tot[6];
         for (int v = 0; v < 6; v++) {
@@ -1004,38 +999,16 @@
     double* dgb = dgbuf + (size_t)b * NS * NU;
     const double mscale = 2.0 * M->ih2 * M->ih2;
 
-    if (tid < NU) {
-        smw[tid] = mscale * M->motion_w_u[tid]; sindep[tid] = M->ucost[tid];
-        srev_of_u[tid] = M->rev_of_u[tid]; sja[tid] = M->bodyang_j[tid]; slegs_n[tid] = M->bodyang_legs_n[tid];
-        for (int i = 0; i < M->bodyang_legs_n[tid]; i++) slegs[tid * LM_MAX_LEGS + i] = M->bodyang_legs[tid][i];
-    }
-    if (tid < nrev) { srev_u[tid] = M->rev_u[tid]; for (int a = 0; a < 3; a++) srbu[3 * tid + a] = M->rev_body_u[tid][a]; }
-    for (int t = tid; t < nq; t += LM_THREADS) scoord_of_state[t] = -1;
-    __syncthreads();
-    if (tid < NU) scoord_of_state[M->ucoord_src[tid]] = tid;
-    const double* gamc = gambuf + ((size_t)cur * n_frames + (size_t)b * NS) * GS;
+    if (tid < NU) { smw[tid] = mscale * M->motion_w_u[tid]; sindep[tid] = M->ucost[tid]; }
     const double* Hlc = Hlr ? Hlr + (hcur + (size_t)b * NS) * PB * (NU * NU) : nullptr;
     __syncthreads();
 
-    auto mot = [&](int i, int j, const double* Ga, const double* Gb) -> double {
-        const int ri = srev_of_u[i], rj = srev_of_u[j];
-        if (ri >= 0 && rj >= 0) return ri == rj ? Ga[GAM_STRIDE * ri] * smw[i] * Gb[GAM_STRIDE * ri] : 0.0;
-        if (ri >= 0) { const int jb = sja[j]; return (jb >= 0 && srbu[3 * ri + jb] == j) ? Ga[GAM_STRIDE * ri] * smw[i] * Gb[GAM_STRIDE * ri + 1 + jb] : 0.0; }
-        if (rj >= 0) { const int ja = sja[i]; return (ja >= 0 && srbu[3 * rj + ja] == i) ? Ga[GAM_STRIDE * rj + 1 + ja] * smw[j] * Gb[GAM_STRIDE * rj] : 0.0; }
-        double v = i == j ? smw[i] : 0.0;
-        const int ja = sja[i], jb = sja[j];
-        if (ja >= 0 && jb >= 0)
-            for (int e = 0; e < slegs_n[i]; e++) {
-                const int r = slegs[i * LM_MAX_LEGS + e];
-                if (srbu[3 * r + jb] == j) v += Ga[GAM_STRIDE * r + 1 + ja] * smw[srev_u[r]] * Gb[GAM_STRIDE * r + 1 + jb];
-            }
-        return v;
-    };
-
     constexpr int UT = LM_THREADS - WAVE, NPB = (NU * NU + UT - 1) / UT;
     const int ut = tid - WAVE;
-    double pb[NPB], pbh = 0.0;
-    int hcnt = 0, ht = 0;
+    double pb[NPB];
+    double qm[NPB];
+#pragma unroll
+    for (int j = 0; j < NPB; j++) { const int t = ut + UT * j; qm[j] = (ut >= 0 && t < NU * NU) ? M->mot_Q[t] : 0.0; }
 
     auto lds_release = [&]() {
         if constexpr (NSPILL > 0) __builtin_amdgcn_fence(__ATOMIC_RELEASE, "workgroup");
@@ -1053,96 +1026,22 @@
         sync_epoch += 3;
         wait_ge(3, sync_epoch);
     };
-    if (tid == 0) { s_int[0] = 0; s_int[1] = 0; }
-    __syncthreads();
-    constexpr int HEAVY_MAX = (LM_MAX_TERMS + LM_MAX_GROUP) / 8;
-    int* elist = reinterpret_cast<int*>(W);
-    if (tid == 0) { s_int[1] = 0; s_int[3] = 0; }
-    __syncthreads();
-#pragma unroll
-    for (int j = 0; j < NPB; j++) {
-        const int t = ut + UT * j;
-        if (ut >= 0 && t < NU * NU) {
-            const int a = t / NU, c = t - a * NU;
-            const int ri = srev_of_u[a], rj = srev_of_u[c];
-            int codes[LM_MAX_GROUP], cnt = 0;
-            auto emit = [&](int oa, int ob, int wi) { if (cnt < LM_MAX_GROUP) codes[cnt++] = (oa << 10) | (ob << 16) | (wi << 22); };
-            if (ri >= 0 && rj >= 0) { if (ri == rj) emit(GAM_STRIDE * ri, GAM_STRIDE * ri, a); }
-            else if (ri >= 0) { const int jb = sja[c]; if (jb >= 0 && srbu[3 * ri + jb] == c) emit(GAM_STRIDE * ri, GAM_STRIDE * ri + 1 + jb, a); }
-            else if (rj >= 0) { const int ja = sja[a]; if (ja >= 0 && srbu[3 * rj + ja] == a) emit(GAM_STRIDE * rj + 1 + ja, GAM_STRIDE * rj, c); }
-            else {
-                if (a == c) emit(63, 63, a);
-                const int ja = sja[a], jb = sja[c];
-                if (ja >= 0 && jb >= 0)
-                    for (int e = 0; e < slegs_n[a]; e++) {
-                        const int r = slegs[a * LM_MAX_LEGS + e];
-                        if (srbu[3 * r + jb] == c) emit(GAM_STRIDE * r + 1 + ja, GAM_STRIDE * r + 1 + jb, srev_u[r]);
-                    }
-            }
-            const int where = (a * LDB + c) | (a == c ? 1 << 30 : 0);
-            if (cnt == 0) elist[NU * NU - 1 - atomicAdd(&s_int[3], 1)] = where;
-            else if (cnt == 1) elist[atomicAdd(&s_int[1], 1)] = where | codes[0] | (1 << 28);
-            else {
-                const int h = atomicAdd(&s_int[0], 1);
-                if (h < HEAVY_MAX) {
-                    for (int g = 0; g < LM_MAX_GROUP; g++) mterm[8 * h + g] = g < cnt ? codes[g] : 0;
-                    mterm[8 * h + 7] = (cnt << 16) | t;
-                }
-            }
-        }
-    }
-    __syncthreads();
-    const int n_term = s_int[1], n_plain = s_int[3];
-    (void)n_plain;
-    const int npa = (n_term + UT - 1) / UT;
-    int my_code[NPB];
-    auto elem_of = [&](int code) -> int { const int off = code & 1023; return (off / LDB) * NU + off % LDB; };
-#pragma unroll
-    for (int j = 0; j < NPB; j++) {
-        const int i = ut + UT * j;
-        int code = 1 << 31;
-        if (ut >= 0) {
-            if (i < n_term) code = elist[i];
-            else if (i - n_term < n_plain) code = elist[NU * NU - 1 - (i - n_term)];
-        }
-        my_code[j] = code;
-    }
     auto fetch_B = [&](int m) {
 #pragma unroll
-        for (int j = 0; j < NPB; j++) if (my_code[j] >= 0) pb[j] = Bc[(size_t)m * (NU * NU) + elem_of(my_code[j])];
-        if (hcnt > 0) pbh = Bc[(size_t)m * (NU * NU) + ht];
+        for (int j = 0; j < NPB; j++) { const int t = ut + UT * j; if (t < NU * NU) pb[j] = Bc[(size_t)m * (NU * NU) + t]; }
     };
-    __syncthreads();
-    const int n_heavy = s_int[0];
-    const bool list_ok = n_heavy <= HEAVY_MAX && n_heavy <= WAVE;
-    const int hsel = ut - WAVE, gsel = ut - 2 * WAVE;
-    int hcode[LM_MAX_GROUP];
-#pragma unroll
-    for (int g = 0; g < LM_MAX_GROUP; g++) hcode[g] = 0;
-    if (list_ok && hsel >= 0 && hsel < n_heavy) {
-#pragma unroll
-        for (int g = 0; g < LM_MAX_GROUP; g++) hcode[g] = mterm[8 * hsel + g];
-        hcnt = mterm[8 * hsel + 7] >> 16; ht = mterm[8 * hsel + 7] & 0xffff;
-    }
-    int gl[LM_MAX_LEGS], gl_n = 0, gl_own = -1;
-#pragma unroll
-    for (int e = 0; e < LM_MAX_LEGS; e++) gl[e] = 0;
+    const int gsel = ut - 2 * WAVE;
+    double g_own = 0.0;
+    int g_n = 0, gsrc[LM_MAX_LEGS];
+#pragma unroll
+    for (int e = 0; e < LM_MAX_LEGS; e++) gsrc[e] = 0;
     if (gsel >= 0 && gsel < NU) {
-        const int r = srev_of_u[gsel];
-        if (r >= 0) gl_own = GAM_STRIDE * r;
-        else {
-            const int ja = sja[gsel];
-            if (ja >= 0) {
-                gl_n = slegs_n[gsel];
-#pragma unroll
-                for (int e = 0; e < LM_MAX_LEGS; e++)
-                    if (e < gl_n) { const int rr = slegs[gsel * LM_MAX_LEGS + e]; gl[e] = (GAM_STRIDE * rr + 1 + ja) | (srev_u[rr] << 8); }
-            }
-        }
-    }
-    double st_gam = 0.0, st_tu = 0.0, st_gv = 0.0;
+        g_own = M->mot_gown[gsel]; g_n = M->mot_gn[gsel];
+#pragma unroll
+        for (int e = 0; e < LM_MAX_LEGS; e++) gsrc[e] = M->mot_gsrc[gsel][e];
+    }
+    double st_tu = 0.0, st_gv = 0.0;
     auto stage_load = [&](int m) {
-        st_gam = lane < GS ? gamc[(size_t)m * GS + lane] : 0.0;
         if (lane < NU) {
             const int p = sindep[lane] & 255, p2 = (sindep[lane] >> 8) - 1;
             double tu = 0.0;
@@ -1164,100 +1063,51 @@
         }
     };
     auto stage_store = [&](int m) {
-        if (lane < GS) gamw[(m % RG) * GS + lane] = st_gam;
         if (lane < NU) { marr[(m & 1) * NU + lane] = smw[lane] * st_tu; sgc[(m & 1) * NU + lane] = st_gv; }
     };
     auto store_row = [&](int m) {
-        const double* Gm = gamw + (m % RG) * GS;
         double Tk[4];
         int base[PB + 1];
 #pragma unroll
         for (int k = 0; k <= 3; k++) Tk[k] = m - k >= 0 ? motion_T(m, k, N) : 0.0;
 #pragma unroll
         for (int k = 0; k <= PB; k++) base[k] = blk_slot<RING>(m, m - k >= 0 ? m - k : m) * BLK;
-        const double* Gk[4];
-#pragma unroll
-        for (int k = 0; k <= 3; k++) Gk[k] = gamw + ((m - k >= 0 ? m - k : m) % RG) * GS;
         const bool prior = Hlc != nullptr;
         const double* Hrow = prior ? ((HIu && m >= lrW && m <= N - lrW) ? HIu : Hlc + (size_t)m * PB * (NU * NU)) : nullptr;
         auto wput = [&](int bo, int off, double v) {
             if constexpr (NSPILL == 0) W[bo + off] = v;
             else { if (bo < NLDS * BLK) W[bo + off] = v; else Wg[bo - NLDS * BLK + off] = v; }
         };
-        auto put = [&](int t, int where, double bval, const double (&acc)[4]) {
-            const int off = where & 1023;
-            double v = bval + Tk[0] * acc[0];
-            if (where & (1 << 30)) { dgb[(size_t)m * NU + off / (LDB + 1)] = v; v += lam * fmax(v, LM_DIAG_FLOOR(N)); }
+        auto put = [&](int t, int a, int c, double bval, double q) {
+            const int off = a * LDB + c;
+            double v = bval + Tk[0] * q;
+            if (a == c) { dgb[(size_t)m * NU + a] = v; v += lam * fmax(v, LM_DIAG_FLOOR(N)); }
             W[base[0] + off] = v;
             if (prior) {
 #pragma unroll
                 for (int k = 1; k <= PB; k++)
-                    if (m - k >= 0) wput(base[k], off, Hrow[(k - 1) * (NU * NU) + t] + (k <= 3 ? Tk[k] * acc[k] : 0.0));
+                    if (m - k >= 0) wput(base[k], off, Hrow[(k - 1) * (NU * NU) + t] + (k <= 3 ? Tk[k] * q : 0.0));
             } else {
 #pragma unroll
                 for (int k = 1; k <= PB; k++)
-                    if (m - k >= 0) wput(base[k], off, k <= 3 ? Tk[k] * acc[k] : 0.0);
+                    if (m - k >= 0) wput(base[k], off, k <= 3 ? Tk[k] * q : 0.0);
             }
         };
 #pragma unroll
         for (int j = 0; j < NPB; j++) {
-            int code = my_code[j];
-            asm volatile("" : "+v"(code));
-            if (code >= 0) {
-                const int t = prior ? elem_of(code) : 0;
-                if (j < npa) {
-                    const int oa = (code >> 10) & 63, ob = (code >> 16) & 63, wi = (code >> 22) & 31;
-                    const int oac = oa == 63 ? 0 : oa, obc = ob == 63 ? 0 : ob;
-                    const double sw = smw[wi], ga = Gm[oac];
-                    double gb[4];
-#pragma unroll
-                    for (int k = 0; k <= 3; k++) gb[k] = Gk[k][obc];
-                    const double wa = (code & (1 << 28)) ? sw * (oa == 63 ? 1.0 : ga) : 0.0;
-                    double acc[4];
-#pragma unroll
-                    for (int k = 0; k <= 3; k++) acc[k] = wa * (ob == 63 ? 1.0 : gb[k]);
-                    put(t, code, pb[j], acc);
-                } else {
-                    const double acc[4] = {0.0, 0.0, 0.0, 0.0};
-                    put(t, code, pb[j], acc);
-                }
-            }
+            const int t = ut + UT * j;
+            if (t < NU * NU) { const int a = t / NU; put(t, a, t - a * NU, pb[j], qm[j]); }
         }
         RSTAMP(14);
-        if (hcnt > 0) {
-            double sw[LM_MAX_GROUP], ga[LM_MAX_GROUP], gb[LM_MAX_GROUP][4];
-            int hc[LM_MAX_GROUP];
-#pragma unroll
-            for (int g = 0; g < LM_MAX_GROUP; g++) { hc[g] = hcode[g]; asm volatile("" : "+v"(hc[g])); }
-#pragma unroll
-            for (int g = 0; g < LM_MAX_GROUP; g++) {
-                const int oa = (hc[g] >> 10) & 63, ob = (hc[g] >> 16) & 63, wi = (hc[g] >> 22) & 31;
-                sw[g] = smw[wi]; ga[g] = Gm[oa == 63 ? 0 : oa];
-#pragma unroll
-                for (int k = 0; k <= 3; k++) gb[g][k] = Gk[k][ob == 63 ? 0 : ob];
-            }
-            double acc[4] = {0.0, 0.0, 0.0, 0.0};
-#pragma unroll
-            for (int g = 0; g < LM_MAX_GROUP; g++) {
-                const int oa = (hc[g] >> 10) & 63, ob = (hc[g] >> 16) & 63;
-                const bool on = g < hcnt;
-                const double wa = on ? sw[g] * (oa == 63 ? 1.0 : ga[g]) : 0.0;
-#pragma unroll
-                for (int k = 0; k <= 3; k++) acc[k] += wa * (ob == 63 || !on ? 1.0 : gb[g][k]);
-            }
-            const int a = ht / NU, c = ht - a * NU;
-            put(ht, (a * LDB + c) | (a == c ? 1 << 30 : 0), pbh, acc);
-        }
-        RSTAMP(15);
         if (gsel >= 0 && gsel < NU) {
             const double* mar = marr + (m & 1) * NU;
-            const double own = mar[gsel], gown = Gm[gl_own >= 0 ? gl_own : 0];
-            double lg[LM_MAX_LEGS], lm[LM_MAX_LEGS];
-#pragma unroll
-            for (int e = 0; e < LM_MAX_LEGS; e++) { lg[e] = Gm[gl[e] & 255]; lm[e] = mar[gl[e] >> 8]; }
-            double gm = gl_own >= 0 ? gown * own : own;
-#pragma unroll
-            for (int e = 0; e < LM_MAX_LEGS; e++) gm += e < gl_n ? lg[e] * lm[e] : 0.0;
+            const double own = mar[gsel];
+            double lm[LM_MAX_LEGS];
+#pragma unroll
+            for (int e = 0; e < LM_MAX_LEGS; e++) lm[e] = mar[gsrc[e] & 255];
+            double gm = g_own * own;
+#pragma unroll
+            for (int e = 0; e < LM_MAX_LEGS; e++) gm += e < g_n ? ((gsrc[e] >> 8) ? 1.0 : 0.0) * lm[e] : 0.0;
             const double gt = sgc[(m & 1) * NU + gsel] + gm;
             gtb[(size_t)m * NU + gsel] = gt;
             rw[(m % RING) * NU + gsel] = -gt;
@@ -1265,13 +1115,12 @@
     };
 
     if (tid < 4) s_cnt[tid] = 0;
-    if (tid == 0) s_int[2] = list_ok ? 0 : 1;
+    if (tid == 0) s_int[2] = 0;
     for (int t = tid; t < BLK + 4 * LDB; t += LM_THREADS) Tm[t] = 0.0;
     __syncthreads();
     STAMP(1);
 
-    if (s_int[2]) {
-    } else if (wave == 0) {
+    if (wave == 0) {
         __builtin_amdgcn_s_setprio(3);
         for (int m = 0; m < RING && m < N; m++) {
             if (m >= 2) wait_ge(3, 3 * (m - 1));
diff --git a/cheetah_pose_estimation_amd/csrc/cpe_tracked.hip.inc b/cheetah_pose_estimation_amd/csrc/cpe_tracked.hip.inc
--- a/cheetah_pose_estimation_amd/csrc/cpe_tracked.hip.inc
+++ b/cheetah_pose_estimation_amd/csrc/cpe_tracked.hip.inc
@@ -38,7 +38,7 @@
 __global__ __launch_bounds__(WAVE) void k_frame_tracked(const DevModel* __restrict__ M, const DevTrack* __restrict__ T, const SeqState* __restrict__ st,
                                                         int N, int which, size_t n_frames, double* __restrict__ qbuf, const double* __restrict__ xt,
                                                         double* __restrict__ gbuf, double* __restrict__ Bbuf, double* __restrict__ costbuf,
-                                                        double* __restrict__ mu, double* __restrict__ gambuf, const DevPriors* __restrict__ pri,
+                                                        double* __restrict__ mu, const DevPriors* __restrict__ pri,
                                                         const int* __restrict__ act, const int* __restrict__ n_act, RaggedArgs rg = RaggedArgs{}) {
     extern __shared__ double smem[];
     const int lane = threadIdx.x;
@@ -61,8 +61,7 @@
     double* ssc = sq + ns;
     double* ssa = ssc + 6 * nl;
     double* sR = ssa + 2 * nrev;
-    double* sgam = sR + 36 * M->n_trunk;
-    double* sres = sgam + GAM_STRIDE * nrev;
+    double* sres = sR + 36 * M->n_trunk;
     double* sH = sres + nu;
     double* sg = sH + nu * nu;
     const int4 fw = *reinterpret_cast<const int4*>(M->fn_lane[lane]);
@@ -95,10 +94,9 @@
     wave_lds_sync();
     if (lane < nrev) {
         const int Bk = fw.z & 255, c = (fw.z >> 8) & 255;
-        double e[3], gtrue[GAM_STRIDE];
-        leg_euler(sR + 36 * (fw.z >> 16), ssc + 6 * Bk, ssa[2 * lane], ssa[2 * lane + 1], sq[3 + 3 * Bk + 2], e, gtrue);
+        double e[3];
+        leg_euler(sR + 36 * (fw.z >> 16), ssa[2 * lane], ssa[2 * lane + 1], sq[3 + 3 * Bk + 2], e);
         sq[3 + 3 * c] = e[0]; sq[3 + 3 * c + 1] = e[1]; sq[3 + 3 * c + 2] = e[2];
-        sgam[GAM_STRIDE * lane] = 1.0; sgam[GAM_STRIDE * lane + 1] = 0.0; sgam[GAM_STRIDE * lane + 2] = 1.0; sgam[GAM_STRIDE * lane + 3] = 0.0;
     }
     double ft = 0.0;
     if (lane < nu) {
@@ -111,7 +109,6 @@
     for (int t = lane; t < nu * nu; t += WAVE) sH[t] = T->H[t];
     wave_lds_sync();
     if (lane < nq) stf[lane] = sq[lane];
-    if (lane < GAM_STRIDE * nrev) gambuf[((size_t)buf * n_frames + f) * (GAM_STRIDE * nrev) + lane] = sgam[lane];
     if (lane < nu) {
         double a = 0.0;
         for (int k = 0; k < nu; k++) a += T->Xt[lane][k] * sres[k];
@@ -148,8 +145,8 @@
                 const int r = M->rev_of_u[k];
                 if (r < 0) { col[nz] = k; val[nz++] = sgn; }
                 else {
-                    col[nz] = k; val[nz++] = sgn * sgam[GAM_STRIDE * r];
-                    for (int a = 0; a < 3; a++) { col[nz] = M->rev_body_u[r][a]; val[nz++] = sgn * sgam[GAM_STRIDE * r + 1 + a]; }
+                    col[nz] = k; val[nz++] = sgn * cpe_cost_gamma(0);
+                    for (int a = 0; a < 3; a++) { col[nz] = M->rev_body_u[r][a]; val[nz++] = sgn * cpe_cost_gamma(1 + a); }
                 }
             }
             for (int i = 0; i < nz; i++) {
```

After: 148.2 million frames/s. About the same (-0.3%).
